# Daaohame/RAHT-3DGS-codec

Hardware: AMD Instinct MI355X
Metric: M-Gaussians/s fwd+inv RAHT, 59-ch SH3 3DGS (higher is better)
Workload: dtype f32 (xyz columns: f64); 1 GPU; cfg3: 2999072 Gaussians (3000000 draws/GPU, J=12, 59 channels), fwd RAHT + quantize/reorder + dequantize/un-reorder + inv RAHT (quantization fused into the transform kernels); the 3 xyz columns carried in float64 inside the same launches (raht_fwd_quant_mixed / raht_dequant_inv_mixed): the reference's integers on every column; rows_per_gpu=2999072, channels=59, depth_J=12, engine=tile, quantize=True, parallelism=1 GPU, world=1

## Files before the change

### include/raht.h

```cpp
#ifndef RAHT_H
#define RAHT_H

#include <stdint.h>

#ifdef __cplusplus
extern "C" {
#endif

#define RAHT_VERSION 300

enum raht_status {
    RAHT_OK = 0,
    RAHT_ERR_INVALID = -1,
    RAHT_ERR_UNSORTED = -2,
    RAHT_ERR_BOUNDS = -3,
    RAHT_ERR_HIP = -4,
    RAHT_ERR_NOMEM = -5,
    RAHT_ERR_UNSUPPORTED = -6
};

enum raht_dtype { RAHT_F32 = 0, RAHT_F64 = 1, RAHT_I32 = 2, RAHT_I64 = 3 };

enum raht_engine { RAHT_ENGINE_TILE = 0, RAHT_ENGINE_LEVEL = 1 };

typedef struct raht_plan raht_plan;
typedef void *raht_stream_t;

const char *raht_last_error(void);
int raht_version(void);

int raht_plan_create(const void *V, int v_dtype, int64_t N, const double minV[3], double width,
                     int depth, raht_stream_t stream, raht_plan **out);

int raht_plan_create_from_keys(const uint64_t *keys_sorted, int64_t N, int nbits,
                               const int64_t *leaf_weights, raht_stream_t stream, raht_plan **out);
int raht_plan_create_from_keys_borrowed(const uint64_t *keys_sorted, int64_t N, int nbits,
                                        const int64_t *leaf_weights, raht_stream_t stream, raht_plan **out);

int raht_plan_set_top_level(raht_plan *plan, int top_level, raht_stream_t stream);
int raht_plan_roots(const raht_plan *plan, int64_t *n_roots, int64_t *rows_dev, raht_stream_t stream);
int raht_plan_set_root_buffer(raht_plan *plan, void *buf_dev);
int raht_plan_set_root_buffer_wide(raht_plan *plan, double *buf_dev);

int raht_plan_set_row_map(raht_plan *plan, const int64_t *map_dev, int64_t n_matrix_rows, raht_stream_t stream);

int raht_plan_destroy(raht_plan *plan);
int64_t raht_plan_size(const raht_plan *plan);
int raht_plan_nbits(const raht_plan *plan);

int raht_plan_set_engine(raht_plan *plan, int engine, int tile_rows);
int raht_plan_set_tail_tile(raht_plan *plan, int tail_rows, int tail_channels, int final_rows);
int raht_plan_set_max_stages(raht_plan *plan, int max_stages);

int raht_release_cached_memory(void);
int raht_set_cached_memory_limit(int64_t bytes);

int raht_plan_levels(const raht_plan *plan);
int raht_plan_export_level(const raht_plan *plan, int level, int64_t *list, uint8_t *flags,
                           int64_t *weights, int64_t *n);
int raht_plan_order(const raht_plan *plan, int64_t *order_dev, raht_stream_t stream);
int raht_plan_arrays(const raht_plan *plan, const uint64_t **keys, const uint8_t **lvl,
                     const int32_t **wl, const int32_t **wr);
int raht_plan_copy_array(const raht_plan *plan, int which, void *dst_dev, raht_stream_t stream);
int raht_plan_stage_stats(raht_plan *plan, int elem_size, int D, int *n_stages, int64_t *rows_per_stage,
                          int max_stages, int *tile_rows);

int raht_fwd(const raht_plan *plan, const float *C, int64_t ldc, int D, float *T, int64_t ldt,
             float *w, raht_stream_t stream);
int raht_fwd_f64(const raht_plan *plan, const double *C, int64_t ldc, int D, double *T, int64_t ldt,
                 double *w, raht_stream_t stream);

int raht_inv(const raht_plan *plan, const float *T, int64_t ldt, int D, float *C, int64_t ldc,
             raht_stream_t stream);
int raht_inv_f64(const raht_plan *plan, const double *T, int64_t ldt, int D, double *C, int64_t ldc,
                 raht_stream_t stream);

int raht_fwd_quant(const raht_plan *plan, const float *C, int64_t ldc, int D, const float *steps,
                   int n_steps, int32_t *Q, int64_t ldq, raht_stream_t stream);
int raht_dequant_inv(const raht_plan *plan, const int32_t *Q, int64_t ldq, int D, const float *steps,
                     int n_steps, float *C, int64_t ldc, raht_stream_t stream);

int raht_fwd_quant_multi(const raht_plan *plan, const float *C, int64_t ldc, int D, const float *steps, int k,
                         int32_t *const *Q, int64_t ldq, raht_stream_t stream);

int raht_dequant_inv_sqdiff(const raht_plan *plan, const int32_t *Q, int64_t ldq, int D, const float *steps, int n_steps,
                            const float *C_ref, int64_t ld_ref, float *C_rec, int64_t ldc, double *sqdiff, raht_stream_t stream);

int raht_fwd_quant_f64(const raht_plan *plan, const double *C, int64_t ldc, int D, const double *steps,
                       int n_steps, int32_t *Q, int64_t ldq, raht_stream_t stream);
int raht_dequant_inv_f64(const raht_plan *plan, const int32_t *Q, int64_t ldq, int D, const double *steps,
                         int n_steps, double *C, int64_t ldc, raht_stream_t stream);

int raht_fwd_quant_mixed(const raht_plan *plan, const float *C, int64_t ldc, int D, const double *steps, int n_steps,
                         int n_wide, int32_t *Q, int64_t ldq, raht_stream_t stream);
int raht_dequant_inv_mixed(const raht_plan *plan, const int32_t *Q, int64_t ldq, int D, const double *steps, int n_steps,
                           int n_wide, float *C, int64_t ldc, raht_stream_t stream);
int raht_fwd_quant_mixed_multi(const raht_plan *plan, const float *C, int64_t ldc, int D, const double *steps, int k,
                               int n_wide, int32_t *const *Q, int64_t ldq, raht_stream_t stream);
int raht_dequant_inv_mixed_sqdiff(const raht_plan *plan, const int32_t *Q, int64_t ldq, int D, const double *steps, int n_steps,
                                  int n_wide, const float *C_ref, int64_t ld_ref, float *C_rec, int64_t ldc, double *sqdiff,
                                  raht_stream_t stream);
int raht_plan_mixed_stats(raht_plan *plan, int D, int n_wide, int *tile_rows, int *n_stages, int64_t *rows_per_stage,
                          int max_stages);

int raht_fwd_batch(int n, raht_plan *const *plans, const float *const *C, const int64_t *ldc, int D,
                   float *const *T, const int64_t *ldt, raht_stream_t stream);
int raht_inv_batch(int n, raht_plan *const *plans, const float *const *T, const int64_t *ldt, int D,
                   float *const *C, const int64_t *ldc, raht_stream_t stream);
int raht_fwd_quant_batch(int n, raht_plan *const *plans, const float *const *C, const int64_t *ldc, int D,
                         const float *steps, int n_steps, int32_t *const *Q, const int64_t *ldq, raht_stream_t stream);
int raht_dequant_inv_batch(int n, raht_plan *const *plans, const int32_t *const *Q, const int64_t *ldq, int D,
                           const float *steps, int n_steps, float *const *C, const int64_t *ldc, raht_stream_t stream);

int raht_fwd_quant_mixed_batch(int n, raht_plan *const *plans, const float *const *C, const int64_t *ldc, int D,
                               const double *steps, int n_steps, int n_wide,
                               int32_t *const *Q, const int64_t *ldq, raht_stream_t stream);
int raht_dequant_inv_mixed_batch(int n, raht_plan *const *plans, const int32_t *const *Q, const int64_t *ldq, int D,
                                 const double *steps, int n_steps, int n_wide,
                                 float *const *C, const int64_t *ldc, raht_stream_t stream);
int raht_mixed_batch_stats(int n, raht_plan *const *plans, int D, int n_wide, int inverse,
                           int *tile_launches, int *top_launches, int *single_scene_calls);

int raht_plan_prepare(raht_plan *plan, int elem_size, int D, raht_stream_t stream);

int raht_plan_set_concurrent_directions(raht_plan *plan, int on);

int raht_plan_set_stage0_events(raht_plan *plan, void *ev_before, void *ev_after);

int raht_debug_run_stage(const raht_plan *plan, int inverse, int stage, const float *mat, int64_t ld_mat,
                         int D, float *mat2, int64_t ld_mat2, int32_t *Q, int64_t ldq, float step,
                         int ablate, raht_stream_t stream);

int raht_quant_reorder(const raht_plan *plan, const float *T, int64_t ldt, int D, const float *steps,
                       int n_steps, int32_t *Q, int64_t ldq, raht_stream_t stream);
int raht_dequant_unreorder(const raht_plan *plan, const int32_t *Q, int64_t ldq, int D,
                           const float *steps, int n_steps, float *T, int64_t ldt,
                           raht_stream_t stream);
int raht_quant_reorder_f64(const raht_plan *plan, const double *T, int64_t ldt, int D, const double *steps,
                           int n_steps, int32_t *Q, int64_t ldq, raht_stream_t stream);
int raht_dequant_unreorder_f64(const raht_plan *plan, const int32_t *Q, int64_t ldq, int D,
                               const double *steps, int n_steps, double *T, int64_t ldt,
                               raht_stream_t stream);

int raht_voxelize(const float *PC, int64_t ldpc, int64_t N, int d, const float *vmin_in,
                  double width_in, int J, uint64_t *keys_sorted, int64_t *sort_idx,
                  int64_t *voxel_indices, float *PCvox, int64_t *Vvox, int64_t *n_vox,
                  float vmin_out[3], double *width_out, double *voxel_size_out,
                  raht_stream_t stream);

int raht_voxelize_all(const float *PC, int64_t ldpc, int64_t N, int d, const float *vmin_in, double width_in,
                      int J, uint64_t *keys_sorted, int64_t *sort_idx, int64_t *voxel_indices, float *PCvox,
                      int64_t *Vvox, float *PCsorted, float *DeltaPC, int64_t *n_vox, float vmin_out[3],
                      double *width_out, double *voxel_size_out, raht_stream_t stream);

int raht_voxelize_plan(const float *PC, int64_t ldpc, int64_t N, int d, const float *vmin_in, double width_in,
                       int J, uint64_t *voxel_keys, int64_t *voxel_indices, float *PCvox, int64_t *n_vox,
                       float vmin_out[3], double *width_out, double *voxel_size_out, raht_stream_t stream,
                       raht_plan **plan);

int raht_voxelize_residuals(const float *PC, int64_t ldpc, int64_t N, int d, const uint64_t *keys_sorted,
                            const int64_t *sort_idx, const float *PCvox, const float vmin[3], double voxel_size,
                            float *PCsorted, float *DeltaPC, raht_stream_t stream);

int raht_voxel_keys(const float *PC, int64_t ldpc, int64_t N, const float vmin[3], double width, int J,
                    uint64_t *keys, raht_stream_t stream);

int raht_morton(const int64_t *V, int64_t N, int J, uint64_t *keys, raht_stream_t stream);

int raht_sort_keys(const uint64_t *keys_in, int64_t N, int nbits, uint64_t *keys_out,
                   int64_t *idx_out, raht_stream_t stream);
int64_t raht_sort_fallbacks(void);

int raht_merge_clusters(const int32_t *cluster_indices, const int32_t *cluster_offsets, int64_t num_clusters,
                        const float *means, const float *quats, const float *scales, const float *opacities,
                        const float *colors, int color_dim, int weight_by_opacity, float *merged_means,
                        float *merged_quats, float *merged_scales, float *merged_opacities,
                        float *merged_colors, raht_stream_t stream);

int raht_voxelize_merge(const float *G, int64_t ldg, int64_t N, int color_dim, int weight_by_opacity, const float *vmin_in,
                        double width_in, int J, uint64_t *keys_sorted, int64_t *sort_idx, int64_t *voxel_indices, float *Gvox,
                        float *merged_means, int64_t *n_vox, float vmin_out[3], double *width_out, double *voxel_size_out,
                        raht_stream_t stream);

int raht_quant_rows(const float *X, int64_t ldx, int64_t n, int D, const float *steps, int n_steps,
                    const int64_t *pos, int32_t *Q, int64_t ldq, raht_stream_t stream);
int raht_dequant_rows(const int32_t *Q, int64_t ldq, const int64_t *pos, int64_t n, int D, const float *steps,
                      int n_steps, float *X, int64_t ldx, raht_stream_t stream);
int raht_quant_rows_f64(const double *X, int64_t ldx, int64_t n, int D, const double *steps, int n_steps,
                        const int64_t *pos, int32_t *Q, int64_t ldq, raht_stream_t stream);
int raht_dequant_rows_f64(const int32_t *Q, int64_t ldq, const int64_t *pos, int64_t n, int D, const double *steps,
                          int n_steps, double *X, int64_t ldx, raht_stream_t stream);

int raht_rows_gather(const void *src, int64_t ld_src, const int64_t *pos, int64_t n, int D, int elem_size, void *dst,
                     int64_t ld_dst, raht_stream_t stream);
int raht_rows_scatter(const void *src, int64_t ld_src, const int64_t *pos, int64_t n, int D, int elem_size, void *dst,
                      int64_t ld_dst, raht_stream_t stream);

int64_t raht_rlgr_bound(int64_t n);
int raht_rlgr_encode(const int32_t *seq, int64_t n, int64_t stride, int flag_signed, uint8_t *out,
                     int64_t cap, int64_t *nbytes);
int raht_rlgr_decode(const uint8_t *buf, int64_t nbytes, int64_t n, int flag_signed, int32_t *seq,
                     int64_t stride);
int raht_rlgr_encode_channels(const int32_t *Q, int64_t N, int D, int64_t sym_stride, int64_t chan_stride,
                              int flag_signed, uint8_t *out, int64_t cap_per_channel, int64_t *nbytes,
                              int nthreads);
int raht_rlgr_decode_channels(const uint8_t *bufs, int64_t cap_per_channel, const int64_t *nbytes,
                              int64_t N, int D, int flag_signed, int32_t *Q, int64_t sym_stride,
                              int64_t chan_stride, int nthreads);
int raht_transpose_i32(const int32_t *in, int64_t ld_in, int64_t rows, int64_t cols, int32_t *out,
                       int64_t ld_out, raht_stream_t stream);
int raht_xchg_bytes(int world, int64_t slot_bytes, int64_t *total);
int raht_xchg_alloc(int world, int64_t slot_bytes, void **base, void *handle64);
int raht_xchg_open(const void *handle64, void **base);
int raht_xchg_close(void *base);
int raht_xchg_free(void *base);
int raht_xchg_gather(const void *send, int64_t slot_bytes, void *const *peers, int rank, int world, uint32_t seq,
                     raht_stream_t stream);
int raht_xchg_buffer(void *base, int world, int64_t slot_bytes, uint32_t seq, void **buf);
int raht_xchg_status(void *base, int world, int64_t slot_bytes, raht_stream_t stream, int *status);

int raht_rlgr_seg_encode(const int32_t *Q, int64_t N, int D, int64_t chan_stride, int seg_len, int flag_signed,
                         uint32_t *seg_bytes, uint32_t *seg_off, uint8_t *out, int64_t cap, int64_t *total_bytes,
                         raht_stream_t stream);
int raht_rlgr_seg_decode(const uint8_t *in, int64_t in_bytes, const uint32_t *seg_off, const uint32_t *seg_bytes, int64_t N,
                         int D, int seg_len, int flag_signed, int32_t *Q, int64_t chan_stride, uint32_t *bad_dev,
                         raht_stream_t stream);

int raht_rlgr_seg_encode_strided(const int32_t *Q, int64_t N, int D, int64_t sym_stride, int64_t chan_stride, int seg_len,
                                 int flag_signed, uint32_t *seg_bytes, uint32_t *seg_off, uint8_t *out, int64_t cap,
                                 int64_t *total_bytes, raht_stream_t stream);
int raht_rlgr_seg_decode_strided(const uint8_t *in, int64_t in_bytes, const uint32_t *seg_off, const uint32_t *seg_bytes, int64_t N,
                                 int D, int seg_len, int flag_signed, int32_t *Q, int64_t sym_stride, int64_t chan_stride,
                                 uint32_t *bad_dev, raht_stream_t stream);

int raht_rlgr_seg_offsets_width(int64_t N, int D, int seg_len);
int raht_rlgr_seg_encode64(const int32_t *Q, int64_t N, int D, int64_t sym_stride, int64_t chan_stride, int seg_len,
                           int flag_signed, uint32_t *seg_bytes, uint64_t *seg_off, uint8_t *out, int64_t cap,
                           int64_t *total_bytes, raht_stream_t stream);
int raht_rlgr_seg_decode64(const uint8_t *in, int64_t in_bytes, const uint64_t *seg_off, const uint32_t *seg_bytes, int64_t N,
                           int D, int seg_len, int flag_signed, int32_t *Q, int64_t sym_stride, int64_t chan_stride,
                           uint32_t *bad_dev, raht_stream_t stream);

#define RAHT_RLGR_BATCH_MAX 12
int raht_rlgr_seg_encode_batch(int k, const int32_t *const *Q, int64_t N, int D, int64_t sym_stride, int64_t chan_stride, int seg_len,
                               int flag_signed, uint32_t *const *seg_bytes, uint32_t *const *seg_off, uint8_t *const *out,
                               const int64_t *cap, int64_t *total_bytes, raht_stream_t stream);
int raht_rlgr_seg_decode_batch(int k, const uint8_t *const *in, const int64_t *in_bytes, const uint32_t *const *seg_off,
                               const uint32_t *const *seg_bytes, int64_t N, int D, int seg_len, int flag_signed, int32_t *const *Q,
                               int64_t sym_stride, int64_t chan_stride, uint32_t *bad_dev, raht_stream_t stream);
int raht_rlgr_seg_decode_batch_check(int k, const uint8_t *const *in, const int64_t *in_bytes, const uint32_t *const *seg_off,
                                     const uint32_t *const *seg_bytes, int64_t N, int D, int seg_len, int flag_signed,
                                     int32_t *const *Q, const int32_t *const *expect, int64_t sym_stride, int64_t chan_stride,
                                     uint32_t *bad_dev, raht_stream_t stream);

int raht_rlgr_seg_encode_batch64(int k, const int32_t *const *Q, int64_t N, int D, int64_t sym_stride, int64_t chan_stride,
                                 int seg_len, int flag_signed, uint32_t *const *seg_bytes, uint64_t *const *seg_off,
// ... 80 lines not shown
```

### raht-3dgs-codec_amd/_lib.py

```python
import contextlib
import ctypes as C
import os
import subprocess

_PKG = os.path.dirname(os.path.abspath(__file__))
_CSRC = os.path.join(_PKG, "csrc")
SO_PATH = os.path.join(_PKG, "libraht_hip.so")

RAHT_OK = 0
ERRORS = {-1: "RAHT_ERR_INVALID", -2: "RAHT_ERR_UNSORTED", -3: "RAHT_ERR_BOUNDS", -4: "RAHT_ERR_HIP",
          -5: "RAHT_ERR_NOMEM", -6: "RAHT_ERR_UNSUPPORTED"}
RAHT_F32, RAHT_F64, RAHT_I32, RAHT_I64 = 0, 1, 2, 3
ENGINE_TILE, ENGINE_LEVEL = 0, 1

EXPORTS = [
    "raht_last_error", "raht_version", "raht_plan_create", "raht_plan_create_from_keys", "raht_plan_create_from_keys_borrowed",
    "raht_plan_destroy", "raht_plan_set_top_level", "raht_plan_roots", "raht_plan_set_root_buffer", "raht_plan_set_root_buffer_wide", "raht_plan_size", "raht_plan_nbits", "raht_plan_set_engine", "raht_plan_set_tail_tile", "raht_release_cached_memory", "raht_set_cached_memory_limit", "raht_quant_rows", "raht_dequant_rows", "raht_quant_rows_f64", "raht_dequant_rows_f64",
    "raht_plan_levels", "raht_plan_export_level", "raht_plan_order", "raht_plan_arrays",
    "raht_plan_copy_array", "raht_plan_stage_stats", "raht_fwd", "raht_fwd_f64", "raht_inv", "raht_inv_f64", "raht_debug_run_stage", "raht_plan_set_stage0_events", "raht_fwd_quant", "raht_dequant_inv", "raht_plan_prepare",
    "raht_quant_reorder", "raht_dequant_unreorder", "raht_voxelize", "raht_voxelize_all", "raht_voxelize_plan", "raht_morton", "raht_sort_keys",
    "raht_voxel_keys", "raht_sort_fallbacks", "raht_voxelize_residuals", "raht_plan_set_row_map", "raht_rows_gather", "raht_rows_scatter",
    "raht_plan_set_max_stages", "raht_plan_set_concurrent_directions", "raht_quant_reorder_f64", "raht_dequant_unreorder_f64", "raht_fwd_quant_f64", "raht_dequant_inv_f64",
    "raht_fwd_quant_mixed", "raht_dequant_inv_mixed", "raht_dequant_inv_sqdiff", "raht_fwd_quant_multi", "raht_plan_mixed_stats",
    "raht_fwd_quant_mixed_multi", "raht_dequant_inv_mixed_sqdiff",
    "raht_fwd_batch", "raht_inv_batch", "raht_fwd_quant_batch", "raht_dequant_inv_batch",
    "raht_fwd_quant_mixed_batch", "raht_dequant_inv_mixed_batch", "raht_mixed_batch_stats",
    "raht_rlgr_bound", "raht_rlgr_encode", "raht_rlgr_decode", "raht_rlgr_encode_channels", "raht_rlgr_decode_channels", "raht_transpose_i32", "raht_i32_equal", "raht_sqdiff_columns", "raht_merge_clusters", "raht_voxelize_merge", "raht_rlgr_seg_encode", "raht_rlgr_seg_decode", "raht_rlgr_seg_encode_strided", "raht_rlgr_seg_decode_strided", "raht_rlgr_seg_encode_batch", "raht_rlgr_seg_decode_batch", "raht_rlgr_seg_decode_batch_check", "raht_rlgr_seg_offsets_width", "raht_rlgr_seg_encode64", "raht_rlgr_seg_decode64", "raht_rlgr_seg_encode_batch64", "raht_rlgr_seg_decode_batch64", "raht_rlgr_seg_encode_ragged", "raht_rlgr_seg_decode_ragged", "raht_debug_rlgr_decode_out", "raht_debug_rlgr_encode_out", "raht_rlgr_seg_rate", "raht_debug_height_stages_per_launch", "raht_debug_live_blocks", "raht_debug_cached_blocks", "raht_debug_sort_form", "raht_debug_motion_tile",
    "raht_xchg_bytes", "raht_xchg_alloc", "raht_xchg_open", "raht_xchg_close", "raht_xchg_free", "raht_xchg_gather", "raht_xchg_buffer", "raht_xchg_status",
    "raht_octree_counts", "raht_octree_encode", "raht_octree_decode", "raht_octree_symbols", "raht_octree_bytes", "raht_demorton",
    "raht_octree_encode_inter", "raht_octree_decode_inter", "raht_octree_bytes_used",
    "raht_region_layout", "raht_region_cells", "raht_region_assemble",
    "raht_region_layout_set", "raht_region_assemble_set", "raht_region_needs",
    "raht_predict", "raht_motion_search", "raht_predict_mc",
]


class RahtError(RuntimeError):
    def __init__(self, code, msg):
        super().__init__(f"{ERRORS.get(code, code)}: {msg}")
        self.code = code


def build(verbose=False):
    r = subprocess.run(["make", "-C", _CSRC, "-j4"], capture_output=True, text=True)
    if verbose or r.returncode != 0:
        print(r.stdout)
        print(r.stderr)
    if r.returncode != 0:
        raise RuntimeError("building libraht_hip.so failed")
    return SO_PATH


_lib = None


def lib():
    global _lib
    if _lib is not None:
        return _lib
    if not os.path.exists(SO_PATH):
        raise RuntimeError(
            f"raht-3dgs-codec_amd: HIP library {SO_PATH} is missing. Build it with "
            f"`python -c 'import __graft_entry__ as g; g.build()'` (or `make -C {_CSRC}`). "
            "There is no CPU fallback for the RAHT hot path.")
    try:
        import torch
    except Exception:
        pass
    L = C.CDLL(SO_PATH)
    vp, i64, i32, dbl = C.c_void_p, C.c_int64, C.c_int, C.c_double
    L.raht_last_error.restype = C.c_char_p
    L.raht_plan_create.argtypes = [vp, i32, i64, C.POINTER(dbl), dbl, i32, vp, C.POINTER(vp)]
    L.raht_plan_create_from_keys.argtypes = [vp, i64, i32, vp, vp, C.POINTER(vp)]
    L.raht_plan_create_from_keys_borrowed.argtypes = [vp, i64, i32, vp, vp, C.POINTER(vp)]
    L.raht_plan_destroy.argtypes = [vp]
    L.raht_plan_set_top_level.argtypes = [vp, i32, vp]
    L.raht_plan_roots.argtypes = [vp, C.POINTER(i64), vp, vp]
    L.raht_plan_set_root_buffer.argtypes = [vp, vp]
    L.raht_plan_set_root_buffer_wide.argtypes = [vp, vp]
    L.raht_plan_size.argtypes = [vp]
    L.raht_plan_size.restype = i64
    L.raht_plan_nbits.argtypes = [vp]
    L.raht_plan_set_engine.argtypes = [vp, i32, i32]
    L.raht_plan_set_tail_tile.argtypes = [vp, i32, i32, i32]
    L.raht_plan_levels.argtypes = [vp]
    L.raht_plan_export_level.argtypes = [vp, i32, vp, vp, vp, C.POINTER(i64)]
    L.raht_plan_order.argtypes = [vp, vp, vp]
    L.raht_plan_arrays.argtypes = [vp, C.POINTER(vp), C.POINTER(vp), C.POINTER(vp), C.POINTER(vp)]
    L.raht_plan_copy_array.argtypes = [vp, i32, vp, vp]
    L.raht_plan_stage_stats.argtypes = [vp, i32, i32, C.POINTER(i32), C.POINTER(i64), i32, C.POINTER(i32)]
    for f in (L.raht_fwd, L.raht_fwd_f64):
        f.argtypes = [vp, vp, i64, i32, vp, i64, vp, vp]
    for f in (L.raht_inv, L.raht_inv_f64):
        f.argtypes = [vp, vp, i64, i32, vp, i64, vp]
    L.raht_plan_set_stage0_events.argtypes = [vp, vp, vp]
    L.raht_debug_run_stage.argtypes = [vp, i32, i32, vp, i64, i32, vp, i64, vp, i64, C.c_float, i32, vp]
    L.raht_fwd_quant.argtypes = [vp, vp, i64, i32, C.POINTER(C.c_float), i32, vp, i64, vp]
    L.raht_dequant_inv.argtypes = [vp, vp, i64, i32, C.POINTER(C.c_float), i32, vp, i64, vp]
    L.raht_plan_prepare.argtypes = [vp, i32, i32, vp]
    L.raht_fwd_quant_mixed.argtypes = [vp, vp, i64, i32, C.POINTER(dbl), i32, i32, vp, i64, vp]
    L.raht_dequant_inv_mixed.argtypes = [vp, vp, i64, i32, C.POINTER(dbl), i32, i32, vp, i64, vp]
    L.raht_dequant_inv_sqdiff.argtypes = [vp, vp, i64, i32, C.POINTER(C.c_float), i32, vp, i64, vp, i64, vp, vp]
    L.raht_fwd_quant_multi.argtypes = [vp, vp, i64, i32, C.POINTER(C.c_float), i32, C.POINTER(vp), i64, vp]
    L.raht_fwd_quant_mixed_multi.argtypes = [vp, vp, i64, i32, C.POINTER(dbl), i32, i32, C.POINTER(vp), i64, vp]
    L.raht_dequant_inv_mixed_sqdiff.argtypes = [vp, vp, i64, i32, C.POINTER(dbl), i32, i32, vp, i64, vp, i64, vp, vp]
    L.raht_plan_mixed_stats.argtypes = [vp, i32, i32, C.POINTER(i32), C.POINTER(i32), C.POINTER(i64), i32]
    pp, pi64 = C.POINTER(vp), C.POINTER(i64)
    L.raht_fwd_batch.argtypes = [i32, pp, pp, pi64, i32, pp, pi64, vp]
    L.raht_inv_batch.argtypes = [i32, pp, pp, pi64, i32, pp, pi64, vp]
    L.raht_fwd_quant_batch.argtypes = [i32, pp, pp, pi64, i32, C.POINTER(C.c_float), i32, pp, pi64, vp]
    L.raht_dequant_inv_batch.argtypes = [i32, pp, pp, pi64, i32, C.POINTER(C.c_float), i32, pp, pi64, vp]
    L.raht_fwd_quant_mixed_batch.argtypes = [i32, pp, pp, pi64, i32, C.POINTER(dbl), i32, i32, pp, pi64, vp]
    L.raht_dequant_inv_mixed_batch.argtypes = [i32, pp, pp, pi64, i32, C.POINTER(dbl), i32, i32, pp, pi64, vp]
    L.raht_mixed_batch_stats.argtypes = [i32, pp, i32, i32, i32, C.POINTER(i32), C.POINTER(i32), C.POINTER(i32)]
    L.raht_plan_set_max_stages.argtypes = [vp, i32]
    L.raht_plan_set_concurrent_directions.argtypes = [vp, i32]
    L.raht_plan_set_row_map.argtypes = [vp, vp, i64, vp]
    for f in (L.raht_rows_gather, L.raht_rows_scatter):
        f.argtypes = [vp, i64, vp, i64, i32, i32, vp, i64, vp]
    for f in (L.raht_quant_reorder_f64, L.raht_dequant_unreorder_f64, L.raht_fwd_quant_f64, L.raht_dequant_inv_f64):
        f.argtypes = [vp, vp, i64, i32, C.POINTER(dbl), i32, vp, i64, vp]
    L.raht_quant_reorder.argtypes = [vp, vp, i64, i32, C.POINTER(C.c_float), i32, vp, i64, vp]
    L.raht_dequant_unreorder.argtypes = [vp, vp, i64, i32, C.POINTER(C.c_float), i32, vp, i64, vp]
    L.raht_quant_rows.argtypes = [vp, i64, i64, i32, C.POINTER(C.c_float), i32, vp, vp, i64, vp]
    L.raht_dequant_rows.argtypes = [vp, i64, vp, i64, i32, C.POINTER(C.c_float), i32, vp, i64, vp]
    L.raht_quant_rows_f64.argtypes = [vp, i64, i64, i32, C.POINTER(dbl), i32, vp, vp, i64, vp]
    L.raht_dequant_rows_f64.argtypes = [vp, i64, vp, i64, i32, C.POINTER(dbl), i32, vp, i64, vp]
    L.raht_voxelize.argtypes = [vp, i64, i64, i32, C.POINTER(C.c_float), dbl, i32, vp, vp, vp, vp, vp,
                                C.POINTER(i64), C.POINTER(C.c_float), C.POINTER(dbl), C.POINTER(dbl), vp]
    L.raht_sqdiff_columns.argtypes = [vp, i64, vp, i64, i64, i32, i32, vp, vp]
    L.raht_voxelize_all.argtypes = [vp, i64, i64, i32, C.POINTER(C.c_float), dbl, i32, vp, vp, vp, vp, vp, vp, vp,
                                    C.POINTER(i64), C.POINTER(C.c_float), C.POINTER(dbl), C.POINTER(dbl), vp]
    L.raht_voxelize_plan.argtypes = [vp, i64, i64, i32, C.POINTER(C.c_float), dbl, i32, vp, vp, vp, C.POINTER(i64),
                                     C.POINTER(C.c_float), C.POINTER(dbl), C.POINTER(dbl), vp, C.POINTER(vp)]
    L.raht_voxelize_merge.argtypes = [vp, i64, i64, i32, i32, C.POINTER(C.c_float), dbl, i32, vp, vp, vp, vp, vp, C.POINTER(i64),
                                      C.POINTER(C.c_float), C.POINTER(dbl), C.POINTER(dbl), vp]
    L.raht_morton.argtypes = [vp, i64, i32, vp, vp]
    L.raht_voxel_keys.argtypes = [vp, i64, i64, C.POINTER(C.c_float), dbl, i32, vp, vp]
    L.raht_voxelize_residuals.argtypes = [vp, i64, i64, i32, vp, vp, vp, C.POINTER(C.c_float), dbl, vp, vp, vp]
    L.raht_sort_keys.argtypes = [vp, i64, i32, vp, vp, vp]
    L.raht_sort_fallbacks.argtypes = []
    L.raht_sort_fallbacks.restype = i64
    L.raht_rlgr_bound.argtypes = [i64]
    L.raht_rlgr_bound.restype = i64
    L.raht_rlgr_encode.argtypes = [vp, i64, i64, i32, vp, i64, C.POINTER(i64)]
    L.raht_rlgr_decode.argtypes = [vp, i64, i64, i32, vp, i64]
    L.raht_rlgr_encode_channels.argtypes = [vp, i64, i32, i64, i64, i32, vp, i64, vp, i32]
    L.raht_rlgr_decode_channels.argtypes = [vp, i64, vp, i64, i32, i32, vp, i64, i64, i32]
    L.raht_merge_clusters.argtypes = [vp, vp, i64, vp, vp, vp, vp, vp, i32, i32, vp, vp, vp, vp, vp, vp]
    L.raht_transpose_i32.argtypes = [vp, i64, i64, i64, vp, i64, vp]
    L.raht_i32_equal.argtypes = [vp, vp, i64, i32, C.POINTER(i64)]
    L.raht_rlgr_seg_encode.argtypes = [vp, i64, i32, i64, i32, i32, vp, vp, vp, i64, C.POINTER(i64), vp]
    L.raht_rlgr_seg_decode.argtypes = [vp, i64, vp, vp, i64, i32, i32, i32, vp, i64, vp, vp]
    L.raht_rlgr_seg_encode_strided.argtypes = [vp, i64, i32, i64, i64, i32, i32, vp, vp, vp, i64, C.POINTER(i64), vp]
    L.raht_rlgr_seg_decode_strided.argtypes = [vp, i64, vp, vp, i64, i32, i32, i32, vp, i64, i64, vp, vp]
    L.raht_debug_rlgr_decode_out.argtypes = [i32]
    L.raht_debug_rlgr_encode_out.argtypes = [i32]
    L.raht_debug_height_stages_per_launch.argtypes = [i32]
    L.raht_debug_live_blocks.argtypes = []
    L.raht_debug_live_blocks.restype = i64
    L.raht_debug_cached_blocks.argtypes = []
    L.raht_debug_cached_blocks.restype = i64
    L.raht_set_cached_memory_limit.argtypes = [i64]
    L.raht_debug_sort_form.argtypes = [i32, i32, i64]
    L.raht_debug_motion_tile.argtypes = [i32]
    L.raht_rlgr_seg_encode_batch.argtypes = [i32, C.POINTER(vp), i64, i32, i64, i64, i32, i32, C.POINTER(vp), C.POINTER(vp), C.POINTER(vp), C.POINTER(i64), C.POINTER(i64), vp]
    L.raht_rlgr_seg_decode_batch.argtypes = [i32, C.POINTER(vp), C.POINTER(i64), C.POINTER(vp), C.POINTER(vp), i64, i32, i32, i32, C.POINTER(vp), i64, i64, vp, vp]
    L.raht_rlgr_seg_decode_batch_check.argtypes = [i32, C.POINTER(vp), C.POINTER(i64), C.POINTER(vp), C.POINTER(vp), i64, i32, i32, i32, C.POINTER(vp), C.POINTER(vp), i64, i64, vp, vp]
    L.raht_rlgr_seg_offsets_width.argtypes = [i64, i32, i32]
    L.raht_rlgr_seg_encode64.argtypes = L.raht_rlgr_seg_encode_strided.argtypes
    L.raht_rlgr_seg_decode64.argtypes = L.raht_rlgr_seg_decode_strided.argtypes
    L.raht_rlgr_seg_encode_batch64.argtypes = L.raht_rlgr_seg_encode_batch.argtypes
    L.raht_rlgr_seg_decode_batch64.argtypes = L.raht_rlgr_seg_decode_batch_check.argtypes
    L.raht_rlgr_seg_encode_ragged.argtypes = [i32, C.POINTER(vp), C.POINTER(i64), i32, C.POINTER(i64), C.POINTER(i64), i32, i32, C.POINTER(vp), C.POINTER(vp), C.POINTER(vp), C.POINTER(i64), C.POINTER(i64), vp]
    L.raht_rlgr_seg_decode_ragged.argtypes = [i32, C.POINTER(vp), C.POINTER(i64), C.POINTER(vp), C.POINTER(vp), C.POINTER(i64), i32, i32, i32, C.POINTER(vp), C.POINTER(vp), C.POINTER(i64), C.POINTER(i64), vp, vp]
    L.raht_rlgr_seg_rate.argtypes = [vp, i32, i64, i64, i32, vp, i32, i32, i32, i32, vp, vp, vp]
    L.raht_xchg_bytes.argtypes = [i32, i64, C.POINTER(i64)]
    L.raht_xchg_alloc.argtypes = [i32, i64, C.POINTER(vp), vp]
    L.raht_xchg_open.argtypes = [vp, C.POINTER(vp)]
    L.raht_xchg_close.argtypes = [vp]
    L.raht_xchg_free.argtypes = [vp]
    L.raht_xchg_gather.argtypes = [vp, i64, C.POINTER(vp), i32, i32, C.c_uint32, vp]
    L.raht_xchg_buffer.argtypes = [vp, i32, i64, C.c_uint32, C.POINTER(vp)]
    L.raht_xchg_status.argtypes = [vp, i32, i64, vp, C.POINTER(i32)]
    L.raht_octree_counts.argtypes = [vp, i64, i32, C.POINTER(i64), vp]
    L.raht_octree_encode.argtypes = [vp, i64, i32, C.POINTER(i64), vp, vp]
    L.raht_octree_decode.argtypes = [vp, C.POINTER(i64), i32, vp, vp, vp]
    L.raht_octree_symbols.argtypes = [vp, i64, vp, vp, vp]
    L.raht_octree_bytes.argtypes = [vp, i64, vp, vp, vp, vp]
    L.raht_demorton.argtypes = [vp, i64, i32, vp, vp]
    L.raht_octree_encode_inter.argtypes = [vp, i64, i32, C.POINTER(i64), vp, i64, vp, vp]
    L.raht_octree_decode_inter.argtypes = [vp, C.POINTER(i64), i32, vp, i64, vp, vp, vp]
    L.raht_octree_bytes_used.argtypes = [vp, i64, vp, i32, vp, vp, vp]
    L.raht_region_layout.argtypes = [vp, i64, i32, i64, i64, vp, vp]
    L.raht_region_cells.argtypes = [vp, i64, i32, i32, i64, vp, vp, vp]
    L.raht_region_assemble.argtypes = [vp, i64, i64, vp, i64, i64, i32, C.POINTER(i64), i32, vp]
    L.raht_region_layout_set.argtypes = [vp, i64, i32, vp, i32, vp, vp]
    L.raht_region_assemble_set.argtypes = [vp, i64, i64, vp, i64, i64, i32, vp, C.POINTER(i64), i32, vp]
    L.raht_region_needs.argtypes = [vp, i64, i32, i32, i32, vp, i64, vp, i32, vp, i64, C.POINTER(i64), vp]
    L.raht_predict.argtypes = [vp, i64, vp, i64, i32, vp, i64, vp, i64, i32, i32, vp, i64, vp, vp]
    L.raht_motion_search.argtypes = [vp, i64, i32, i32, vp, i64, vp, i64, i32, vp, i64, vp, i64, i32, vp, vp, i32, vp, vp, vp, vp]
    L.raht_predict_mc.argtypes = [vp, i64, i32, i32, vp, i64, vp, vp, i64, i32, vp, i64, vp, i64, i32, i32, vp, i64, vp, vp]
    _lib = L
    return L


def check(rc):
    if rc != RAHT_OK:
        raise RahtError(rc, lib().raht_last_error().decode("utf-8", "replace"))


@contextlib.contextmanager
def sort_form(onesweep=1, rounds=0, fail_tile=-1):
    prev = lib().raht_debug_sort_form(onesweep, rounds, fail_tile)
    check(min(prev, 0))
    try:
        yield
    finally:
        lib().raht_debug_sort_form(prev & 1, (prev >> 1) & 31, (prev >> 6) - 1)
```

### raht-3dgs-codec_amd/csrc/raht_common.h

```cpp
#pragma once

#include <hip/hip_runtime.h>
#include <stdint.h>

#include <cstdarg>
#include <cstdio>
#include <deque>
#include <exception>
#include <functional>
#include <new>
#include <type_traits>
#include <utility>
#include <vector>

#include "raht.h"

#define RAHT_WAVE 64
#define RAHT_MAX_LEVELS 64

namespace raht {

void set_error(const char *fmt, ...);

#define RAHT_HIP_CHECK(expr)                                                              \
// ... 45 lines not shown
    return RAHT_OK;
}

constexpr int RAHT_MAX_DEVICES = 64;
static inline int current_device()
{
    int d = 0;
    if (hipGetDevice(&d) != hipSuccess || d < 0 || d >= RAHT_MAX_DEVICES) d = 0;
    return d;
}
class DeviceGuard {
public:
    explicit DeviceGuard(int device) : prev_(current_device()), dev_(device)
    {
        if (prev_ != dev_) (void)hipSetDevice(dev_);
    }
    ~DeviceGuard() { if (prev_ != dev_) (void)hipSetDevice(prev_); }
    DeviceGuard(const DeviceGuard &) = delete;
    DeviceGuard &operator=(const DeviceGuard &) = delete;
private:
    int prev_, dev_;
};
struct PerDeviceOnce {
    bool done[RAHT_MAX_DEVICES] = {};
    bool first(int device) { if (done[device]) return false; done[device] = true; return true; }
};

class Scratch {
public:
    Scratch(size_t bytes, hipStream_t stream);
    ~Scratch();
    Scratch(const Scratch &) = delete;
    Scratch &operator=(const Scratch &) = delete;
    void *ptr() const { return p_; }
    template <typename T> T *as() const { return (T *)p_; }
    bool ok() const { return p_ != nullptr; }
private:
    void *p_ = nullptr;
    int slot_ = -1;
};

hipError_t dev_malloc(void **p, size_t bytes);
template <typename T> inline hipError_t dev_malloc(T **p, size_t bytes) { return dev_malloc((void **)p, bytes); }
void dev_free(void *p);

template <typename T>
class DevBuf {
public:
    DevBuf() = default;
    DevBuf(DevBuf &&o) noexcept : p_(o.p_), owned_(o.owned_) { o.p_ = nullptr; }
    DevBuf &operator=(DevBuf &&o) noexcept { if (this != &o) { reset(); p_ = o.p_; owned_ = o.owned_; o.p_ = nullptr; } return *this; }
    ~DevBuf() { reset(); }
    hipError_t alloc(size_t count)
    {
        reset();
        owned_ = true;
        return dev_malloc((void **)&p_, count * sizeof(typename std::conditional<std::is_void<T>::value, char, T>::type));
    }
    void borrow(T *p) { reset(); p_ = p; owned_ = false; }
    T *get() const { return p_; }
    operator T *() const { return p_; }
    void reset() { if (p_ && owned_) dev_free(p_); p_ = nullptr; }
    T *release() { T *q = p_; p_ = nullptr; return q; }
private:
    T *p_ = nullptr;
    bool owned_ = true;
};
struct OwnedEvent {
    hipEvent_t ev = nullptr;
    OwnedEvent() = default;
    OwnedEvent(OwnedEvent &&o) noexcept : ev(o.ev) { o.ev = nullptr; }
    OwnedEvent &operator=(OwnedEvent &&o) noexcept { std::swap(ev, o.ev); return *this; }
    ~OwnedEvent() { if (ev) (void)hipEventDestroy(ev); }
    operator hipEvent_t() const { return ev; }
};

int read_back_u32(uint32_t *dst_a, const uint32_t *dev_a, int na, uint32_t *dst_b, const uint32_t *dev_b, int nb,
                  hipStream_t s, const std::function<void()> &behind = std::function<void()>());

int exclusive_scan_u32(const uint32_t *in, uint32_t *out, int64_t n, uint32_t *total, hipStream_t s);
int exclusive_scan_u32_u64(const uint32_t *in, uint64_t *out, int64_t n, uint64_t *total, hipStream_t s);

struct VoxGrid;
int sort_keys_u32idx(const uint64_t *keys_in, int64_t N, int nbits, uint64_t *keys_out, uint32_t *idx_out, hipStream_t s,
                     uint32_t *sort_err = nullptr, int64_t *idx64_out = nullptr, const VoxGrid *grid = nullptr, bool onesweep = true);
void note_sort_fallback();
int vox_keys(const VoxGrid &grid, int64_t N, uint64_t *keys, hipStream_t s);
int bucket_sort_u8(const uint8_t *bucket, uint32_t *perm_out, int64_t n, int bits,
                   uint32_t *bucket_off, hipStream_t s);

int compact_u32(const uint32_t *in, const uint32_t *flag, uint32_t *out, int64_t n,
                int64_t *count_host, hipStream_t s, const uint32_t *extra_dev = nullptr, uint32_t *extra_host = nullptr);

int run_starts_u64(const uint64_t *keys_sorted, int64_t n, uint32_t *starts, int64_t *starts64, uint64_t *run_keys,
                   uint32_t *count_dev, hipStream_t s);

#ifdef RAHT_PHASE_CLOCKS
constexpr int PL_CLK_BLOCKS = 4096, PL_CLK_SLOTS = 12;
static __device__ unsigned long long g_phase_clk_plan[3][PL_CLK_BLOCKS][PL_CLK_SLOTS];
#define PL_STAMP(which, blk, k) do { if (threadIdx.x == 0 && (blk) < PL_CLK_BLOCKS) g_phase_clk_plan[which][blk][k] = __builtin_readcyclecounter(); } while (0)
#define PL_NOTE_LEVELS(blk, n) do { if (threadIdx.x == 0 && (blk) < PL_CLK_BLOCKS) g_phase_clk_plan[1][blk][PL_CLK_SLOTS - 1] = (unsigned long long)(n); } while (0)
#define PL_SLOT_DECL int pl_slot = 0
#define PL_STAMP_NEXT() do { if (pl_slot < 8) { PL_STAMP(2, 0, pl_slot); ++pl_slot; } } while (0)
int read_phase_clocks_sched(unsigned long long *dst, int which, int n_blocks);
#else
#define PL_STAMP(which, blk, k) do { } while (0)
#define PL_NOTE_LEVELS(blk, n) do { } while (0)
#define PL_SLOT_DECL do { } while (0)
#define PL_STAMP_NEXT() do { } while (0)
#endif

constexpr int RAHT_TOP_MAX_ROWS = 8192;

struct Stage {
    int64_t n_entries = 0;
    int64_t n_tiles = 0;
    DevBuf<uint32_t> rows;
    DevBuf<uint32_t> surv_off;
    DevBuf<void> ws;
    size_t ws_inv_off = 0;
    int tile_rows = 0;
    DevBuf<int32_t> e_wl, e_wr;
    DevBuf<uint8_t> e_lvl;
    DevBuf<uint32_t> e_pos;
    DevBuf<uint8_t> e_ht;
    bool is_top = false;
    uint32_t n_merges = 0;
    DevBuf<uint32_t> t_pj;
    DevBuf<float> t_ab32;
    DevBuf<double> t_ab64;
    DevBuf<uint32_t> t_root;
    uint32_t t_loff[65] = {0};
    uint32_t t_lev_host[2 * 64] = {0};
    DevBuf<uint32_t> t_lev;
    int t_nlev = 0;
    int t_nbig = 0;
    uint32_t t_small_start = 0;
    DevBuf<uint32_t> prog;
    uint32_t prog_stride = 0;
    uint32_t prog_ab = 0;
    bool prog_compact = false;
};

struct Schedule {
    int tile_rows = 0;
    int tail_rows = 0;
    int final_rows = 0;
    bool valid = false;
    std::vector<Stage> stages;
    size_t ws_row_bytes = 0;
    bool ws_split = false;
    OwnedEvent ready;
    hipStream_t ready_on = nullptr;
};
static_assert(!std::is_copy_constructible<Stage>::value && !std::is_copy_constructible<Schedule>::value, "stages and schedules own device memory: moved, never copied");

}

struct raht_plan {
    int device = 0;
    int64_t N = 0;
    int nbits = 0;
    int max_level = -1;
    raht::DevBuf<uint64_t> keys;
    raht::DevBuf<uint8_t> lvl;
    raht::DevBuf<int32_t> wl, wr;
    raht::DevBuf<int64_t> wsum;
    raht::DevBuf<uint32_t> order;
    raht::DevBuf<uint32_t> inv_order;
    raht::DevBuf<uint32_t> level_rows;
    uint32_t level_off[RAHT_MAX_LEVELS + 1];
    int top_level = 64;
    int64_t n_roots = 1;
    raht::DevBuf<uint32_t> root_rows;
    void *root_buf = nullptr;
    double *root_buf_w = nullptr;
    raht::DevBuf<uint32_t> row_map;
    int64_t map_rows = 0;
    int engine = RAHT_ENGINE_TILE;
    int tile_rows_override = 0;
    int tail_rows_override = 0;
    int tail_chunk_override = 0;
    int final_rows_override = 0;
    const uint32_t *pend_dev = nullptr; uint32_t *pend_host = nullptr; int pend_n = 0;
    hipEvent_t ev_before = nullptr, ev_after = nullptr;
    int max_stages = 24;
    bool split_ws = false;
    std::deque<raht::Schedule> schedules;
    std::vector<uint8_t> lvl_host;
};

namespace raht {
int check_plan_device(const raht_plan *plan, const char *what);
__device__ __forceinline__ void pair_weights(int64_t i, int l, int r, const int64_t *wsum, double &w0, double &w1)
{
    if (wsum) {
        w0 = (double)(wsum[i] - wsum[i - l]);
        w1 = (double)(wsum[i + r] - wsum[i]);
    } else {
        w0 = (double)l;
        w1 = (double)r;
    }
}

int ensure_level_rows(raht_plan *plan, hipStream_t s);
int get_schedule(raht_plan *plan, int tile_rows, int tail_rows, int final_rows, hipStream_t s, Schedule **out);
void pick_tail_geometry(const raht_plan *plan, int elem_size, int D, int stage0_rows, int *tail_rows, int *tail_chunk,
                        int *final_rows);
int build_tile_programs(raht_plan *plan, Schedule *sc, hipStream_t s);
int ensure_workspace(Schedule *sc, size_t row_bytes, bool split = false);
static inline void *stage_ws(const Stage &st, bool inverse) { return st.ws ? (void *)((char *)st.ws.get() + (inverse ? st.ws_inv_off : 0)) : nullptr; }
void free_schedule(Schedule &sc);
struct StageArrays { const uint32_t *rows; const int32_t *wl, *wr; const uint8_t *lvl; const uint32_t *pos; uint8_t *ht; };
static inline StageArrays stage_arrays(const raht_plan *p, const Stage &st)
{
    if (st.rows) return {st.rows, st.e_wl, st.e_wr, st.e_lvl, st.e_pos, st.e_ht};
    return {nullptr, p->wl, p->wr, p->lvl, p->inv_order, st.e_ht};
}
int pick_tile_rows(const raht_plan *plan, int elem_size, int chunk_channels);
int pick_chunk_channels(int elem_size, int D);

size_t tile_lds_bytes(int R, int elem_size, int Dc, bool ident, bool qm);
int launch_sq_final(const double *part, int64_t n_tiles, int D, int ncv, double *out, hipStream_t s);
}
```

### raht-3dgs-codec_amd/csrc/schedule.hip

```cpp
#include "raht_common.h"

#include <algorithm>
#include <atomic>

namespace raht {

__global__ void compact_scatter_kernel(const uint32_t *in, const uint32_t *flag, const uint32_t *pos, uint32_t *out, int64_t n);

__global__ void stage_survivor_kernel(const uint32_t *__restrict__ rows, int64_t n, int R, int64_t N,
                                      const int32_t *__restrict__ wl, const int32_t *__restrict__ wr,
                                      const uint8_t *__restrict__ lvl, int top_level,
                                      uint32_t *__restrict__ survivor)
{
    const int64_t j = (int64_t)blockIdx.x * blockDim.x + threadIdx.x;
    if (j >= n) return;
    const int64_t r = rows ? rows[j] : j;
    const int64_t t = j / R;
    const int64_t j0 = t * R, j1 = j0 + R;
    const int64_t start = rows ? rows[j0] : j0;
    const int64_t end = (j1 < n) ? (rows ? (int64_t)rows[j1] : j1) : N;
    const bool merged = (r > 0) && ((int)lvl[r] < top_level) && (r - wl[r] >= start) && (r + wr[r] <= end);
    survivor[j] = merged ? 0u : 1u;
}

static int fit_chunk_channels(int elem_size, int D, int max_dc)
{
    const int vn = 16 / elem_size;
    const int hi = std::max(std::min(max_dc, 64), vn);
    if (D <= hi) return D;
    for (int Dc = hi; Dc >= vn; --Dc) {
        const int r = D % Dc;
        if (r == 0 || r >= vn) return Dc;
    }
    for (int Dc = hi + 1; Dc <= 64; ++Dc) {
        const int r = D % Dc;
        if (r == 0 || r >= vn) return Dc;
    }
    return std::min(D, 64);
}

int pick_chunk_channels(int elem_size, int D)
{
    return fit_chunk_channels(elem_size, D, 64);
}

size_t tile_lds_bytes(int R, int elem_size, int Dc, bool ident, bool qm)
{
    const int vn = 16 / elem_size;
    const size_t Dp = (size_t)((Dc + vn - 1) / vn) * vn;
    size_t data = (size_t)R * Dp * elem_size;
    size_t meta = (size_t)R * ((elem_size == 4 ? 16 : 24) + (ident ? 0 : 4) + (qm ? 4 : 0) + 1);
    size_t surv = ((size_t)R * 2 + 15) & ~(size_t)15;
    return data + ((meta + 15) & ~(size_t)15) + 1024 + surv + (size_t)12 * Dp * elem_size;
}

int pick_tile_rows(const raht_plan *plan, int elem_size, int Dc)
{
    if (plan->tile_rows_override > 0) return plan->tile_rows_override;
    const size_t budget = (size_t)42 * 1280;
    for (int R = 512; R >= 64; R -= 8)
        if (tile_lds_bytes(R, elem_size, Dc, true, true) <= budget) return R;
    return 0;
}

void pick_tail_geometry(const raht_plan *plan, int elem_size, int D, int stage0_rows, int *tail_rows, int *tail_chunk,
                        int *final_rows)
{
    int Dc = std::min(D, 64), R = stage0_rows;
    if (D > 64) Dc = pick_chunk_channels(elem_size, D);
    if (plan->tail_chunk_override > 0) Dc = fit_chunk_channels(elem_size, D, std::min(plan->tail_chunk_override, std::min(D, 64)));
    if (plan->tail_rows_override > 0) {
        R = plan->tail_rows_override;
        while (R > 64 && tile_lds_bytes(R, elem_size, Dc, false, true) > (size_t)128 * 1280) R -= 64;
    } else {
        while (R > 64 && tile_lds_bytes(R, elem_size, Dc, false, true) > (size_t)42 * 1280) R -= 8;
    }
    *tail_rows = R;
    *tail_chunk = Dc;
    int Rf = 1536;
    if (plan->final_rows_override > 0) Rf = std::min(plan->final_rows_override, RAHT_TOP_MAX_ROWS);
    *final_rows = Rf;
}

void free_schedule(Schedule &sc)
{
    if (!sc.stages.empty()) (void)hipDeviceSynchronize();
    sc.stages.clear();
    sc.ready = OwnedEvent();
}

int ensure_workspace(Schedule *sc, size_t row_bytes, bool split)
{
    if (row_bytes <= sc->ws_row_bytes && split == sc->ws_split) return RAHT_OK;
    row_bytes = std::max(row_bytes, sc->ws_row_bytes);
    for (size_t k = 1; k < sc->stages.size(); ++k) {
        Stage &st = sc->stages[k];
        if (st.ws) { (void)hipDeviceSynchronize(); st.ws.reset(); }
        const size_t one = (row_bytes * (size_t)st.n_entries + 255) & ~(size_t)255;
        if (st.ws.alloc(split ? 2 * one : one) != hipSuccess) {
            set_error("workspace allocation failed (%zu bytes)", split ? 2 * one : one);
            sc->ws_row_bytes = 0;
            return RAHT_ERR_NOMEM;
        }
        st.ws_inv_off = split ? one : 0;
    }
    sc->ws_row_bytes = row_bytes;
    sc->ws_split = split;
    return RAHT_OK;
}

__global__ void tile_start_kernel(const uint32_t *__restrict__ pos, int64_t n, int R, int64_t n_tiles,
                                  uint32_t total, uint32_t *__restrict__ surv_off)
{
    const int64_t t = (int64_t)blockIdx.x * blockDim.x + threadIdx.x;
    if (t > n_tiles) return;
    surv_off[t] = (t < n_tiles) ? pos[t * R] : total;
    (void)n;
}

__global__ void gather_meta_kernel(const uint32_t *__restrict__ rows, int64_t n, const int32_t *__restrict__ wl,
                                   const int32_t *__restrict__ wr, const uint8_t *__restrict__ lvl,
                                   const uint32_t *__restrict__ inv_order, int32_t *__restrict__ e_wl,
                                   int32_t *__restrict__ e_wr, uint8_t *__restrict__ e_lvl, uint32_t *__restrict__ e_pos)
{
    const int64_t j = (int64_t)blockIdx.x * blockDim.x + threadIdx.x;
    if (j >= n) return;
    const uint32_t r = rows[j];
    e_wl[j] = wl[r]; e_wr[j] = wr[r]; e_lvl[j] = lvl[r]; e_pos[j] = inv_order[r];
}

constexpr int HT_MAX_ROWS = 1024, HT_MAX_STAGES = 8;
struct HeightStage {
    const uint32_t *rows; const int32_t *wl, *wr; const uint8_t *lvl; uint8_t *ht;
    int64_t n; int R; uint32_t first_tile;
    const uint32_t *n_dev, *kind_dev; uint32_t kind_tile;
};
struct HeightArgs { HeightStage st[HT_MAX_STAGES]; int n_stages; uint32_t n_tiles; int64_t N; int top_level; };

template <int SPL>
__global__ __launch_bounds__(64) void tile_heights_kernel(const HeightArgs H)
{
    extern __shared__ __align__(16) unsigned char ht_smem[];
    int k = 0;
#pragma unroll
    for (int q = 1; q < HT_MAX_STAGES; ++q) k += (q < H.n_stages && blockIdx.x >= H.st[q].first_tile) ? 1 : 0;
    PL_STAMP(1, blockIdx.x, 0);
    const HeightStage &S = H.st[k];
    const int R = S.R;
    const int lane = threadIdx.x;
    const int64_t e0 = (int64_t)(blockIdx.x - S.first_tile) * R;
    if (S.kind_dev && *S.kind_dev != S.kind_tile) return;
    const int64_t Sn = S.n_dev ? (int64_t)*S.n_dev : S.n;
    if (e0 >= Sn) return;
    const uint32_t *__restrict__ rows = S.rows;
    const int nt = (int)min((int64_t)R, Sn - e0);
    uint8_t *s_cur = ht_smem;
    uint32_t *s_row = (uint32_t *)(ht_smem + ((R + 15) & ~15));
    const int64_t start_row = rows ? (int64_t)rows[e0] : e0;
    const int64_t end_row = (e0 + R < Sn) ? (rows ? (int64_t)rows[e0 + R] : e0 + R) : H.N;
    int lv[SPL], part[SPL];
    int32_t wlv[SPL], wrv[SPL];
    int64_t r[SPL];
#pragma unroll
    for (int s = 0; s < SPL; ++s) {
        const int j = lane + s * 64;
        lv[s] = 255; wlv[s] = 0; wrv[s] = 0; r[s] = 0;
        if (j < nt) {
            r[s] = rows ? (int64_t)rows[e0 + j] : e0 + j;
            lv[s] = (int)S.lvl[e0 + j]; wlv[s] = S.wl[e0 + j]; wrv[s] = S.wr[e0 + j];
        }
    }
    if (rows) {
#pragma unroll
        for (int s = 0; s < SPL; ++s) { const int j = lane + s * 64; if (j < nt) s_row[j] = (uint32_t)r[s]; }
    }
#pragma unroll
    for (int s = 0; s < SPL; ++s) { const int j = lane + s * 64; if (j < nt) s_cur[j] = 0; }
    __syncthreads();
    PL_STAMP(1, blockIdx.x, 1);
    uint64_t mask = 0;
#pragma unroll
    for (int s = 0; s < SPL; ++s) {
        const int j = lane + s * 64;
        const bool merged = (j < nt) && (r[s] > 0) && (lv[s] < H.top_level) && (r[s] - wlv[s] >= start_row) && (r[s] + wrv[s] <= end_row);
        part[s] = 0;
        if (merged) {
            if (!rows) part[s] = j - wlv[s];
            else {
                const uint32_t want = (uint32_t)(r[s] - wlv[s]);
                int lo = 0, hi = j - 1;
                while (lo < hi) { const int mid = (lo + hi) >> 1; if (s_row[mid] < want) lo = mid + 1; else hi = mid; }
                part[s] = lo;
            }
            mask |= (uint64_t)1 << lv[s];
        } else {
            lv[s] = 255;
        }
    }
#pragma unroll
    for (int d = 32; d >= 1; d >>= 1) {
        const uint32_t lo = (uint32_t)__shfl_xor((int)(uint32_t)mask, d, 64), hi = (uint32_t)__shfl_xor((int)(uint32_t)(mask >> 32), d, 64);
        mask |= (uint64_t)lo | ((uint64_t)hi << 32);
    }
    int ht[SPL];
#pragma unroll
    for (int s = 0; s < SPL; ++s) ht[s] = 0;
    PL_STAMP(1, blockIdx.x, 2);
    PL_NOTE_LEVELS(blockIdx.x, __popcll(mask));
    mask = (uint64_t)(uint32_t)__builtin_amdgcn_readfirstlane((int)(uint32_t)mask) |
           ((uint64_t)(uint32_t)__builtin_amdgcn_readfirstlane((int)(uint32_t)(mask >> 32)) << 32);
    while (mask) {
        const int l = __ffsll((unsigned long long)mask) - 1;
        mask &= mask - 1;
        int h[SPL];
#pragma unroll
        for (int s = 0; s < SPL; ++s) {
            h[s] = 0;
            if (lv[s] == l) h[s] = 1 + max((int)s_cur[part[s]], (int)s_cur[lane + s * 64]);
        }
#pragma unroll
        for (int s = 0; s < SPL; ++s)
            if (lv[s] == l) { ht[s] = h[s]; s_cur[part[s]] = (uint8_t)h[s]; }
        __syncthreads();
    }
    PL_STAMP(1, blockIdx.x, 3);
#pragma unroll
    for (int s = 0; s < SPL; ++s) { const int j = lane + s * 64; if (j < nt) S.ht[e0 + j] = (uint8_t)ht[s]; }
    PL_STAMP(1, blockIdx.x, 4);
}

template <typename F>
static void by_lane_slots(int R, F &&f)
{
    const int spl = (R + 63) / 64;
    if (spl <= 3) f(std::integral_constant<int, 3>{});
    else if (spl <= 4) f(std::integral_constant<int, 4>{});
    else if (spl <= 8) f(std::integral_constant<int, 8>{});
    else f(std::integral_constant<int, 16>{});
}

// ... 24 lines not shown
        for (int q = H.n_stages; q < HT_MAX_STAGES; ++q) H.st[q] = H.st[0];
        launch_heights_kernel(H, maxR, any_rows, s);
        RAHT_HIP_CHECK(hipGetLastError());
        reset();
        return RAHT_OK;
    };
    reset();
    const int group = g_height_group.load();
    for (size_t k = 0; k < sc.stages.size(); ++k) {
        Stage &st = sc.stages[k];
        if (st.is_top || st.n_entries < 1) continue;
        if (st.tile_rows > HT_MAX_ROWS) { set_error("tile heights: %d rows per tile not supported", st.tile_rows); return RAHT_ERR_UNSUPPORTED; }
        if (!st.e_ht) RAHT_HIP_CHECK(st.e_ht.alloc((size_t)st.n_entries));
        HeightStage &h = H.st[H.n_stages++];
        h = height_stage(stage_arrays(plan, st), st.tile_rows, H.n_tiles);
        h.n = st.n_entries;
        H.n_tiles += (uint32_t)st.n_tiles;
        maxR = std::max(maxR, st.tile_rows);
        any_rows = any_rows || st.rows != nullptr;
        if (H.n_stages == group) RAHT_RET(flush());
    }
    return flush();
}

struct ProgStage {
    const uint32_t *rows; const int32_t *wl, *wr; const uint8_t *lvl, *ht; const uint32_t *pos;
    uint32_t *prog; int64_t n; int R; uint32_t stride, ab; int compact;
};

template <int SPL>
__global__ __launch_bounds__(64) void tile_program_kernel(const ProgStage S, int64_t N, int top_level, const int64_t *__restrict__ wsum)
{
    extern __shared__ __align__(16) unsigned char pg_smem[];
    __shared__ uint32_t s_hist[64], s_cur[64];
    uint32_t *s_row = (uint32_t *)pg_smem;
    const int R = S.R;
    const int lane = threadIdx.x;
    const int64_t e0 = (int64_t)blockIdx.x * R;
    if (e0 >= S.n) return;
    const uint32_t *__restrict__ rows = S.rows;
    const int nt = (int)min((int64_t)R, S.n - e0);
    const int64_t start_row = rows ? (int64_t)rows[e0] : e0;
    const int64_t end_row = (e0 + R < S.n) ? (rows ? (int64_t)rows[e0 + R] : e0 + R) : N;
    uint32_t *pg = S.prog + (size_t)blockIdx.x * S.stride;
    uint32_t *rw = pg + 32, *rec = pg + 32 + R;
    double *ab = (double *)(pg + S.ab);
    int lv[SPL], ht[SPL];
    int32_t wlv[SPL], wrv[SPL];
    uint32_t pos[SPL];
    int64_t r[SPL];
#pragma unroll
    for (int s = 0; s < SPL; ++s) {
        const int j = lane + s * 64;
        lv[s] = 255; wlv[s] = 0; wrv[s] = 0; r[s] = 0; ht[s] = 0; pos[s] = 0;
        if (j < nt) {
            r[s] = rows ? (int64_t)rows[e0 + j] : e0 + j;
            lv[s] = (int)S.lvl[e0 + j]; wlv[s] = S.wl[e0 + j]; wrv[s] = S.wr[e0 + j];
            ht[s] = S.ht[e0 + j] & 63; pos[s] = S.pos[e0 + j];
        }
    }
    s_hist[lane] = 0;
    if (rows) {
#pragma unroll
        for (int s = 0; s < SPL; ++s) { const int j = lane + s * 64; if (j < nt) s_row[j] = (uint32_t)r[s]; }
    }
    __syncthreads();
    bool merged[SPL];
    int part[SPL];
#pragma unroll
    for (int s = 0; s < SPL; ++s) {
        const int j = lane + s * 64;
        merged[s] = (j < nt) && (r[s] > 0) && (lv[s] < top_level) && (r[s] - wlv[s] >= start_row) && (r[s] + wrv[s] <= end_row);
        part[s] = 0;
        if (merged[s]) {
            if (!rows) part[s] = j - wlv[s];
            else {
                const uint32_t want = (uint32_t)(r[s] - wlv[s]);
                int lo = 0, hi = j - 1;
                while (lo < hi) { const int mid = (lo + hi) >> 1; if (s_row[mid] < want) lo = mid + 1; else hi = mid; }
                part[s] = lo;
            }
            atomicAdd(&s_hist[ht[s]], 1u);
        }
        if (j < nt) rw[j] = pos[s] | (merged[s] ? 0x80000000u : 0u);
    }
    __syncthreads();
    const uint32_t c = s_hist[lane];
    uint32_t inc = c;
#pragma unroll
    for (int d = 1; d < 64; d <<= 1) {
        const uint32_t t = __shfl_up(inc, d, 64);
        if (lane >= d) inc += t;
    }
    ((uint16_t *)pg)[lane] = (uint16_t)inc;
    s_cur[lane] = inc - c;
    const uint32_t n_merged = (uint32_t)__shfl((int)inc, 63, 64);
    __syncthreads();
    const uint64_t lt = (lane == 0) ? 0ull : (~0ull >> (64 - lane));
    uint32_t n_surv = 0;
#pragma unroll
    for (int s = 0; s < SPL; ++s) {
        const int j = lane + s * 64;
        const bool surv = j < nt && !merged[s];
        const uint64_t bal = __ballot(surv);
        if (surv) rec[n_merged + n_surv + (uint32_t)__popcll(bal & lt)] = (uint32_t)j;
        n_surv += (uint32_t)__popcll(bal);
        if (merged[s]) {
            const uint32_t k = atomicAdd(&s_cur[ht[s]], 1u);
            if (S.compact) {
                rec[k] = (uint32_t)j | ((uint32_t)wlv[s] << 10) | ((uint32_t)wrv[s] << 20);
            } else {
                double w0, w1;
                pair_weights(r[s], wlv[s], wrv[s], wsum, w0, w1);
                const double den = w0 + w1;
                rec[k] = (uint32_t)part[s] | ((uint32_t)j << 16);
                ab[2 * k] = sqrt(w0 / den);
                ab[2 * k + 1] = sqrt(w1 / den);
            }
        }
    }
}

int build_tile_programs(raht_plan *plan, Schedule *sc, hipStream_t s)
{
    bool built = false;
    for (auto &st : sc->stages) {
        if (st.is_top || st.n_entries < 1 || st.prog) continue;
        const int R = st.tile_rows;
        if (R > HT_MAX_ROWS || !st.e_ht) { set_error("tile programs: %d rows per tile not supported", R); return RAHT_ERR_UNSUPPORTED; }
        ProgStage P;
        const StageArrays a = stage_arrays(plan, st);
        P.rows = a.rows; P.wl = a.wl; P.wr = a.wr; P.lvl = a.lvl; P.pos = a.pos; P.ht = a.ht;
        P.n = st.n_entries; P.R = R;
        P.compact = (st.rows == nullptr && plan->wsum == nullptr) ? 1 : 0;
        P.ab = (uint32_t)(32 + 2 * R + 3) & ~3u;
        P.stride = P.compact ? P.ab : P.ab + 4 * (uint32_t)R;
        if (!P.wl || !P.wr || !P.lvl || !P.pos) { set_error("tile programs: missing plan arrays"); return RAHT_ERR_INVALID; }
        RAHT_HIP_CHECK(st.prog.alloc((size_t)P.stride * (size_t)st.n_tiles));
        P.prog = st.prog;
        const size_t lds = st.rows ? (size_t)R * 4 : 0;
        const unsigned grid = (unsigned)st.n_tiles;
        by_lane_slots(R, [&](auto spl) {
            hipLaunchKernelGGL(tile_program_kernel<decltype(spl)::value>, dim3(grid), dim3(64), lds, s, P, plan->N, plan->top_level, plan->wsum);
        });
        RAHT_HIP_CHECK(hipGetLastError());
        st.prog_stride = P.stride; st.prog_ab = P.ab; st.prog_compact = P.compact != 0;
        built = true;
    }
    if (built) {
        if (!sc->ready) RAHT_HIP_CHECK(hipEventCreateWithFlags(&sc->ready.ev, hipEventDisableTiming));
        RAHT_HIP_CHECK(hipEventRecord(sc->ready, s));
        sc->ready_on = s;
    }
    return RAHT_OK;
}

__global__ void top_resolve_kernel(const uint32_t *__restrict__ rows, int64_t n, const int32_t *__restrict__ wl,
                                   const int32_t *__restrict__ wr, const uint8_t *__restrict__ lvl,
                                   const int64_t *__restrict__ wsum, int top_level, uint32_t *__restrict__ pj,
                                   double *__restrict__ ab, uint8_t *__restrict__ bucket, uint32_t *__restrict__ is_root)
{
    const int64_t e = (int64_t)blockIdx.x * blockDim.x + threadIdx.x;
    if (e >= n) return;
    const int64_t r = rows ? (int64_t)rows[e] : e;
    const int l = (int)lvl[r];
    const bool merged = (r > 0) && (l < top_level);
    is_root[e] = merged ? 0u : 1u;
    bucket[e] = merged ? (uint8_t)l : (uint8_t)63;
    uint32_t rec = 0;
    double a = 0.0, b = 0.0;
    if (merged) {
        const int64_t want = r - wl[r];
        int64_t p = want;
        if (rows) {
            int64_t lo = 0, hi = e - 1;
            while (lo < hi) {
                const int64_t mid = (lo + hi) >> 1;
                if ((int64_t)rows[mid] < want) lo = mid + 1; else hi = mid;
            }
            p = lo;
        }
        double w0, w1;
        pair_weights(r, wl[r], wr[r], wsum, w0, w1);
        const double den = w0 + w1;
        a = sqrt(w0 / den);
        b = sqrt(w1 / den);
        rec = (uint32_t)p | ((uint32_t)e << 16);
    }
    pj[e] = rec; ab[2 * e] = a; ab[2 * e + 1] = b;
}

__global__ void top_gather_kernel(const uint32_t *__restrict__ perm, uint32_t n_merges, const uint32_t *__restrict__ pj,
                                  const double *__restrict__ ab, uint32_t *__restrict__ t_pj,
                                  float *__restrict__ t_ab32, double *__restrict__ t_ab64)
{
    const uint32_t k = blockIdx.x * blockDim.x + threadIdx.x;
    if (k >= n_merges) return;
    const uint32_t e = perm[k];
    t_pj[k] = pj[e];
    const double a = ab[2 * e], b = ab[2 * e + 1];
    t_ab64[2 * k] = a; t_ab64[2 * k + 1] = b;
    t_ab32[2 * k] = (float)a; t_ab32[2 * k + 1] = (float)b;
}

__global__ void top_root_rank_kernel(const uint32_t *__restrict__ is_root, const uint32_t *__restrict__ pos, int64_t n,
                                     uint32_t *__restrict__ t_root)
{
    const int64_t e = (int64_t)blockIdx.x * blockDim.x + threadIdx.x;
    if (e < n) t_root[e] = is_root[e] ? pos[e] : 0xffffffffu;
}

static hipError_t gather_stage_meta(const raht_plan *plan, Stage &st, hipStream_t s)
{
    const size_t n = (size_t)st.n_entries;
    hipError_t e = hipSuccess;
    if ((e = st.e_wl.alloc(n)) != hipSuccess || (e = st.e_wr.alloc(n)) != hipSuccess || (e = st.e_lvl.alloc(n)) != hipSuccess ||
        (e = st.e_pos.alloc(n)) != hipSuccess) return e;
    hipLaunchKernelGGL(gather_meta_kernel, dim3((unsigned)ceil_div((int64_t)n, 256)), dim3(256), 0, s, st.rows, (int64_t)n, plan->wl,
                       plan->wr, plan->lvl, plan->inv_order, st.e_wl, st.e_wr, st.e_lvl, st.e_pos);
    return hipSuccess;
}

static int build_top_stage(raht_plan *plan, int64_t n, hipStream_t s, Stage &st)
{
    st.is_top = true;
    st.n_entries = n;
    st.n_tiles = 1;
    st.tile_rows = (int)n;
    const uint32_t *rows = st.rows;
    const unsigned gb = (unsigned)ceil_div(n, 256);
    if (rows) RAHT_HIP_CHECK(gather_stage_meta(plan, st, s));
    Scratch buf(sizeof(double) * 2 * (size_t)n + sizeof(uint32_t) * (4 * (size_t)n + 66) + (size_t)n, s);
    if (!buf.ok()) return RAHT_ERR_NOMEM;
    double *ab = buf.as<double>();
    uint32_t *pj = (uint32_t *)(ab + 2 * n), *is_root = pj + n, *pos = is_root + n, *perm = pos + n, *boff = perm + n,
             *total = boff + 65;
    uint8_t *bucket = (uint8_t *)(total + 1);
    hipLaunchKernelGGL(top_resolve_kernel, dim3(gb), dim3(256), 0, s, rows, n, plan->wl, plan->wr, plan->lvl, plan->wsum,
                       plan->top_level, pj, ab, bucket, is_root);
    RAHT_RET(exclusive_scan_u32(is_root, pos, n, total, s));
    RAHT_HIP_CHECK(st.t_root.alloc((size_t)n));
    hipLaunchKernelGGL(top_root_rank_kernel, dim3(gb), dim3(256), 0, s, is_root, pos, n, st.t_root);
    RAHT_RET(bucket_sort_u8(bucket, perm, n, 6, boff, s));
    RAHT_RET(read_back_u32(st.t_loff, boff, 65, nullptr, nullptr, 0, s));
    st.n_merges = st.t_loff[63];
    {
        uint32_t *lev = st.t_lev_host;
        int nlev = 0;
        for (int l = 0; l < 63; ++l)
            if (st.t_loff[l + 1] > st.t_loff[l]) { lev[2 * nlev] = st.t_loff[l]; lev[2 * nlev + 1] = st.t_loff[l + 1]; ++nlev; }
        int nbig = nlev;
        while (nbig > 0 && lev[2 * (nbig - 1) + 1] - lev[2 * (nbig - 1)] <= 64) --nbig;
        const size_t lds_budget = 160 * 1024 - 1024;
        while (nbig < nlev && (size_t)n * 16 + (size_t)(st.n_merges - lev[2 * nbig]) * 20 > lds_budget) ++nbig;
        st.t_nlev = nlev; st.t_nbig = nbig;
        st.t_small_start = (nbig < nlev) ? lev[2 * nbig] : st.n_merges;
        RAHT_HIP_CHECK(st.t_lev.alloc(2 * 64));
        RAHT_HIP_CHECK(hipMemcpyAsync(st.t_lev, lev, sizeof(uint32_t) * 2 * (size_t)std::max(nlev, 1), hipMemcpyHostToDevice, s));
    }
    const size_t nm = std::max<size_t>(st.n_merges, 1);
    RAHT_HIP_CHECK(st.t_pj.alloc(nm));
    RAHT_HIP_CHECK(st.t_ab32.alloc(2 * nm));
    RAHT_HIP_CHECK(st.t_ab64.alloc(2 * nm));
    if (st.n_merges)
        hipLaunchKernelGGL(top_gather_kernel, dim3((unsigned)ceil_div(st.n_merges, 256)), dim3(256), 0, s, perm, st.n_merges,
                           pj, ab, st.t_pj, st.t_ab32, st.t_ab64);
    return RAHT_OK;
}

constexpr int SB_THREADS = 256, SB_ITEMS = 8, SB_BLOCK = SB_THREADS * SB_ITEMS;
constexpr int SCHED_SPEC_MAX = 8;
enum { SK_NONE = 0, SK_TILE = 1, SK_TOP = 2 };

struct SchedState {
    uint32_t n[SCHED_SPEC_MAX + 2];
    uint32_t kind[SCHED_SPEC_MAX + 2];
    uint32_t finished;
    uint32_t last_stage, last_is_top;
    uint32_t trouble;
    uint32_t top[4];
};
constexpr int SCHED_STATE_WORDS = sizeof(SchedState) / 4;

__device__ __forceinline__ uint32_t block_sum_256(uint32_t v, uint32_t *red )
{
#pragma unroll
    for (int d = 32; d >= 1; d >>= 1) v += __shfl_xor(v, d, 64);
    if ((threadIdx.x & 63) == 0) red[threadIdx.x >> 6] = v;
    __syncthreads();
    const uint32_t t = red[0] + red[1] + red[2] + red[3];
    __syncthreads();
    return t;
}

__device__ __forceinline__ void sched_state_init(SchedState *S, uint32_t n0, uint32_t kind0)
{
    uint32_t *w = (uint32_t *)S;
    for (int i = threadIdx.x; i < SCHED_STATE_WORDS; i += blockDim.x) w[i] = 0;
    __syncthreads();
    if (threadIdx.x == 0) { S->n[0] = n0; S->kind[0] = kind0; }
}

__global__ __launch_bounds__(SB_THREADS) void sched_count_kernel(SchedState *__restrict__ S, int k, const uint32_t *__restrict__ rows,
                                                                 const int32_t *__restrict__ wl, const int32_t *__restrict__ wr,
                                                                 const uint8_t *__restrict__ lvl, int R, int64_t N, int top_level,
                                                                 uint8_t *__restrict__ flags, uint32_t *__restrict__ blk_cnt, int64_t n_first)
// ... 583 lines not shown
```

### raht-3dgs-codec_amd/csrc/transform_mx.hip

```cpp
#include "raht_common.h"
#include "raht_device.h"
#include "tile_engine.h"
#include "tile_host.h"

#include <algorithm>
#include <cstdlib>
#include <string>
#include <type_traits>
#include <vector>

namespace raht {

#ifdef RAHT_PHASE_CLOCKS
constexpr int MX_CLK_TILES = 4096, MX_CLK_SLOTS = 12;
__device__ unsigned long long g_phase_clk_mx[MX_CLK_TILES][MX_CLK_SLOTS];
#define MX_STAMP(k) do { if (IDENT && threadIdx.x == 0 && tile_id < MX_CLK_TILES) g_phase_clk_mx[tile_id][k] = __builtin_readcyclecounter(); } while (0)
#else
#define MX_STAMP(k) do { } while (0)
#endif

constexpr int MX_MAX_WIDE = 4;
constexpr int MX_THREADS = 512;
constexpr int MX_TOP_THREADS = 1024;
constexpr int MX_TOP_SLOTS = RAHT_TOP_MAX_ROWS / MX_TOP_THREADS;

struct StepTableMX {
    StepTable f;
    double w[MX_MAX_WIDE];
};

static size_t tile_lds_bytes_mx(int R, int NF, int nwide)
{
    const size_t data = (size_t)R * NF * 16 + (((size_t)R * nwide * 8 + 15) & ~(size_t)15);
    const size_t meta = (size_t)R * (16 + 4 + 4);
    const size_t surv = ((size_t)R * 2 + 15) & ~(size_t)15;
    return data + meta + surv;
}

struct MxPtrs {
    const double *in_w;
    double *out_w;
    double *wsn_w;
    double *root_w;
    const uint32_t *prog;
    uint32_t prog_stride, prog_ab;
    int prog_compact;
};

struct MxMultiQ {
    int k;
    uint32_t fast_div;
    double step[MULTI_Q_MAX];
    int32_t *Q[MULTI_Q_MAX];
};

template <bool INV, bool IDENT, int SLOTS, bool ROOTS, bool MULTI = false, bool SQ = false>
__device__ __forceinline__ void tile_body_mx(const TileArgs<float> &A, const MxPtrs &P, const StepTableMX &ST, const int64_t tile_id,
                                             const MxMultiQ *MQ = nullptr)
{
    extern __shared__ __align__(16) unsigned char smem[];
    typedef RegChunk<float> V16;
    typedef RegChunk<double> W16;
    typedef RegChunk<int32_t> I16;
    const int R = A.R;
    const int tid0 = threadIdx.x;
    const int nthreads = blockDim.x, nwv = nthreads >> 6;
    const int nwide = A.nwide;
    const int lgw = nwide > 2 ? 2 : nwide - 1;
    const int Df = A.D;
    const int Fp = A.Dp, NF = Fp >> 2;
    const int lg = A.lg, lr = 6 - A.lg;
    const uint32_t NFm = ((1u << 20) + (uint32_t)NF - 1) / (uint32_t)NF;
    auto sync_lds = [&]() { asm volatile("s_waitcnt lgkmcnt(0)\n\ts_barrier" ::: "memory"); };
    auto wait_landed = [&]() { asm volatile("s_waitcnt vmcnt(0)" ::: "memory"); };

    size_t off = 0;
    float *ftile = (float *)smem; off += (size_t)R * Fp * 4;
    double *wd = (double *)(smem + off); off += ((size_t)R * nwide * 8 + 15) & ~(size_t)15;
    W16 *rec_ab = (W16 *)(smem + off); off += (size_t)R * 16;
    uint32_t *rec_pj = (uint32_t *)(smem + off); off += (size_t)R * 4;
    int32_t *sdst = (int32_t *)(smem + off); off += (size_t)R * 4;
    uint16_t *ssurv = (uint16_t *)(smem + off);

    auto lane_geom = [&](int tid, int &lane, int &wid, int &g, int &c4, int &fl, int &sp, int &goff, bool &head) {
        lane = tid & 63;
        wid = __builtin_amdgcn_readfirstlane(tid >> 6);
        g = lane >> lg;
        c4 = lane & ((1 << lg) - 1);
        fl = min(c4, NF - 1);
        head = c4 == 0;
        sp = fl;
        goff = min(fl * 4, Df - 4);
    };
    float my_step[4], my_rcp[4], tab_step[4];
    auto fetch_steps = [&](int place) {
        const int g0 = ST.f.n == 1 ? 0 : min(place * 4, Df - 4);
#pragma unroll
        for (int i = 0; i < 4; ++i) tab_step[i] = ST.f.v[g0 + i];
    };
    auto use_steps = [&]() {
#pragma unroll
        for (int i = 0; i < 4; ++i) {
            my_step[i] = ST.f.n == 1 ? ST.f.v[0] : tab_step[i];
            my_rcp[i] = refined_rcp(my_step[i]);
        }
    };

    int tid = tid0;
    asm volatile("" : "+v"(tid));
    int lane, wid, g, c4, fl, sp, goff; bool head;
    lane_geom(tid, lane, wid, g, c4, fl, sp, goff, head);
    const int64_t e0 = tile_id * R;
    const int nt = (int)min((int64_t)R, A.n_entries - e0);
    MX_STAMP(0);
    if constexpr (!MULTI) fetch_steps(fl);

    const uint32_t *pg = P.prog + (uint64_t)tile_id * P.prog_stride;
    const int end_v = ((const uint16_t *)pg)[lane];
    const int endm_v = lane ? ((const uint16_t *)pg)[lane - 1] : 0;
    uint32_t surv_raw = A.surv_off ? A.surv_off[tile_id + (tid0 & 1)] : 0u;
    uint32_t m_rw[SLOTS], m_rec[SLOTS];
    W16 m_ab[SLOTS];
#pragma unroll
    for (int s = 0; s < SLOTS; ++s) {
        const int j = tid0 + s * nthreads;
        m_rw[s] = 0; m_rec[s] = 0; m_ab[s].v[0] = 0.0; m_ab[s].v[1] = 0.0;
        if (j < nt) {
            m_rw[s] = pg[32 + j];
            m_rec[s] = pg[32 + R + j];
            if (!P.prog_compact) m_ab[s] = ((const W16 *)(pg + P.prog_ab))[j];
        }
    }
    auto early_loads_landed = [&]() {
        asm volatile("" : "+v"(surv_raw));
        if constexpr (!MULTI) asm volatile("" : "+v"(tab_step[0]), "+v"(tab_step[1]), "+v"(tab_step[2]), "+v"(tab_step[3]));
    };
    auto fin_of = [&](uint32_t rw) { return (rw >> 31) != 0 || (A.last_stage && !ROOTS); };
    auto write_dst = [&]() {
#pragma unroll
        for (int s = 0; s < SLOTS; ++s) {
            const int j = tid0 + s * nthreads;
            if (j < nt) sdst[j] = (int32_t)((m_rw[s] & 0x7fffffffu) | (fin_of(m_rw[s]) ? 0x80000000u : 0u));
        }
    };
    auto write_survivors = [&](uint32_t n_merged) {
#pragma unroll
        for (int s = 0; s < SLOTS; ++s) {
            const uint32_t k = (uint32_t)(tid0 + s * nthreads);
            if (k >= n_merged && k < (uint32_t)nt) ssurv[k - n_merged] = (uint16_t)m_rec[s];
        }
    };
    auto write_records = [&](uint32_t n_merged) {
#pragma unroll
        for (int s = 0; s < SLOTS; ++s) {
            const uint32_t k = (uint32_t)(tid0 + s * nthreads);
            if (k < n_merged) {
                uint32_t pj = m_rec[s];
                W16 ab = m_ab[s];
                if (P.prog_compact) {
                    const uint32_t j = pj & 1023u, l = (pj >> 10) & 1023u, r = (pj >> 20) & 1023u;
                    const double w0 = (double)(int)l, w1 = (double)(int)r;
                    const double den = w0 + w1;
                    ab.v[0] = sqrt(w0 / den);
                    ab.v[1] = sqrt(w1 / den);
                    pj = (j - l) | (j << 16);
                }
                rec_ab[k] = ab;
                rec_pj[k] = pj;
            }
        }
    };

    auto load_linear = [&](const float *dst, int chunks, const float *src) {
        const uint32_t lds0 = (uint32_t)(uintptr_t)(__attribute__((address_space(3))) const void *)dst;
        for (int it = wid; (it << 6) < chunks; it += nwv) {
            const int c = (it << 6) + lane;
            if (c < chunks) glds16<0>(src + (uint32_t)c * 4u, lds0 + ((uint32_t)it << 10));
        }
    };
    auto load_caller_rows = [&](int rows, auto src) {
        const uint32_t lds0 = (uint32_t)(uintptr_t)(__attribute__((address_space(3))) const void *)ftile;
        const int total = rows * NF;
        for (int it = wid; (it << 6) < total; it += nwv) {
            const int c = (it << 6) + lane;
            const int jr = (int)(((uint32_t)c * NFm) >> 20), ch = c - jr * NF;
            if (c < total) { const void *a = src(jr, (uint32_t)min(ch * 4, Df - 4)); if (a) glds16<1>(a, lds0 + ((uint32_t)it << 10)); }
        }
    };
    auto widen_row = [&](int j) {
        double *row = wd + __mul24(j, nwide);
        const V16 raw = *(const V16 *)(ftile + __mul24(j, Fp));
        double d[4];
#pragma unroll
        for (int i = 0; i < 4; ++i) d[i] = i < nwide ? (double)raw.v[i] : 0.0;
#pragma unroll
        for (int i = 0; i < 4; ++i) if (i < nwide) row[i] = d[i];
    };

    if constexpr (!INV) {
        if constexpr (IDENT) {
            const uint32_t ldc = (uint32_t)A.ld_in;
            const float *src = A.in + e0 * (int64_t)ldc;
            load_caller_rows(nt, [&](int jr, uint32_t go) { return row_at(src, (uint32_t)jr, ldc, go); });
        } else {
            load_linear(ftile, nt * NF, A.in + e0 * (int64_t)Fp);
            load_linear((const float *)wd, (nt * nwide + 1) >> 1, (const float *)(P.in_w + e0 * (int64_t)nwide));
        }
        MX_STAMP(9);
        const uint32_t n_merged = (uint32_t)__builtin_amdgcn_readlane(end_v, 63);
        write_dst();
        write_survivors(n_merged);
        write_records(n_merged);
        MX_STAMP(1);
        wait_landed();
        early_loads_landed();
        sync_lds();
        MX_STAMP(2);
        if constexpr (IDENT) {
#pragma unroll
            for (int s = 0; s < SLOTS; ++s) {
                const int j = tid + s * nthreads;
                if (j < nt) widen_row(j);
            }
            sync_lds();
        }
        MX_STAMP(3);
        MX_STAMP(4);
    } else {
        const uint32_t n_merged = (uint32_t)__builtin_amdgcn_readlane(end_v, 63);
        write_dst();
        write_survivors(n_merged);
        MX_STAMP(1);
        sync_lds();
        MX_STAMP(2);
        load_caller_rows(nt, [&](int jr, uint32_t go) -> const void * {
            const uint32_t d = (uint32_t)sdst[jr];
            return (d >> 31) ? (const void *)row_far((const int32_t *)A.Q, d & 0x7fffffffu, (uint32_t)A.ldq, go) : nullptr; });
        write_records(n_merged);
        const uint32_t surv_base = (uint32_t)__builtin_amdgcn_readlane((int)surv_raw, 0);
        const uint32_t surv_cnt = (uint32_t)__builtin_amdgcn_readlane((int)surv_raw, 1) - surv_base;
        if (!A.last_stage) {
            if (c4 < NF) for (uint32_t it = wid; (it << lr) < surv_cnt; it += nwv) {
                const uint32_t qc = min((it << lr) + g, surv_cnt - 1);
                const V16 x = ld_chunk<float>(row_at((const float *)A.wsn + (int64_t)surv_base * Fp, qc, (uint32_t)Fp, (uint32_t)(fl * 4)));
                *(V16 *)&ftile[__mul24((int)ssurv[qc], Fp) + fl * 4] = x;
            }
            for (uint32_t c = (uint32_t)tid; c < surv_cnt * (uint32_t)nwide; c += (uint32_t)nthreads) {
                const uint32_t qc = c / (uint32_t)nwide, i = c - qc * (uint32_t)nwide;
                wd[__mul24((int)ssurv[qc], nwide) + i] = P.wsn_w[(int64_t)surv_base * nwide + c];
            }
        } else if (ROOTS) {
            if (c4 < NF) for (uint32_t it = wid; (it << lr) < surv_cnt; it += nwv) {
                const uint32_t qc = min((it << lr) + g, surv_cnt - 1);
                const V16 x = ld_chunk<float>(A.root_buf + (int64_t)(surv_base + qc) * Df + goff);
                *(V16 *)&ftile[__mul24((int)ssurv[qc], Fp) + fl * 4] = x;
            }
            for (uint32_t c = (uint32_t)tid; c < surv_cnt * (uint32_t)nwide; c += (uint32_t)nthreads) {
                const uint32_t qc = c / (uint32_t)nwide, i = c - qc * (uint32_t)nwide;
                wd[__mul24((int)ssurv[qc], nwide) + i] = P.root_w[(int64_t)surv_base * nwide + c];
            }
        }
        MX_STAMP(3);
        wait_landed();
        early_loads_landed();
        sync_lds();
        MX_STAMP(4);
        use_steps();
#pragma unroll
        for (int s = 0; s < SLOTS; ++s) {
            const int j = tid0 + s * nthreads;
            if (j < nt && fin_of(m_rw[s])) {
                double *row = wd + __mul24(j, nwide);
                const I16 raw = *(const I16 *)(ftile + __mul24(j, Fp));
#pragma unroll
                for (int i = 0; i < 4; ++i) if (i < nwide) row[i] = (double)raw.v[i] * ST.w[i];
            }
        }
        if (A.last_stage && !ROOTS) {
            const uint32_t n_fin = (uint32_t)nt - n_merged;
            if (c4 < NF) for (uint32_t it = wid; (it << lr) < n_fin; it += nwv) {
                const uint32_t qc = (it << lr) + g;
                if (qc < n_fin) {
                    V16 *pr = (V16 *)&ftile[__mul24((int)ssurv[qc], Fp) + fl * 4];
                    const I16 raw = *(const I16 *)pr;
                    V16 x;
#pragma unroll
                    for (int i = 0; i < 4; ++i)
                        x.v[i] = (head && i < nwide) ? __int_as_float(raw.v[i]) : (float)raw.v[i] * my_step[i];
                    *pr = x;
                }
            }
        }
        sync_lds();
    }
    MX_STAMP(5);
    {
        const uint32_t stride = (uint32_t)(nwv << lr);
        const uint32_t gw = (uint32_t)lane >> lgw, cw = (uint32_t)min(lane & ((1 << lgw) - 1), nwide - 1);
        const uint32_t bw = 64u >> lgw;
        const uint32_t cf = (uint32_t)fl * 4u;
        bool chained = false;
        const int loff_v = endm_v, hist_v = end_v - endm_v;
        uint64_t mask = __ballot(hist_v > 0);
        while (mask) {
            const int l = INV ? (63 - __clzll((long long)mask)) : (__ffsll((long long)mask) - 1);
            mask &= ~(1ull << l);
            const uint32_t base = (uint32_t)__builtin_amdgcn_readlane(loff_v, l), cnt = (uint32_t)__builtin_amdgcn_readlane(hist_v, l);
            auto apply_f = [&](auto UC, uint32_t mb) {
                constexpr int U = decltype(UC)::value;
                W16 ab[U];
                uint32_t pj[U];
#pragma unroll
                for (int u = 0; u < U; ++u) { const uint32_t m = base + min(mb + u * stride + g, cnt - 1); pj[u] = rec_pj[m]; ab[u] = rec_ab[m]; }
                uint32_t ip[U], ij[U];
                V16 x0[U], x1[U];
#pragma unroll
                for (int u = 0; u < U; ++u) { ip[u] = __umul24(pj[u] & 0xffffu, (uint32_t)Fp) + cf; ij[u] = __umul24(pj[u] >> 16, (uint32_t)Fp) + cf; }
#pragma unroll
                for (int u = 0; u < U; ++u) { x0[u] = *(const V16 *)&ftile[ip[u]]; x1[u] = *(const V16 *)&ftile[ij[u]]; }
                if constexpr (INV) {
#pragma unroll
                    for (int u = 0; u < U; ++u) {
#pragma unroll
                        for (int i = 0; i < 4; ++i) x1[u].v[i] = (float)__float_as_int(x1[u].v[i]) * my_step[i];
                    }
                }
#pragma unroll
                for (int u = 0; u < U; ++u) {
                    const float ca = (float)ab[u].v[0], cb = (float)ab[u].v[1];
                    V16 lo, hi;
#pragma unroll
                    for (int i = 0; i < 4; ++i) {
                        if (!INV) {
                            lo.v[i] = ca * x0[u].v[i] + cb * x1[u].v[i];
                            hi.v[i] = ca * x1[u].v[i] - cb * x0[u].v[i];
                        } else {
                            lo.v[i] = ca * x0[u].v[i] - cb * x1[u].v[i];
                            hi.v[i] = cb * x0[u].v[i] + ca * x1[u].v[i];
                        }
                    }
                    if (u == 0 || mb + u * stride < cnt) { *(V16 *)&ftile[ip[u]] = lo; *(V16 *)&ftile[ij[u]] = hi; }
                }
            };
            auto pass_f = [&](auto UC) {
                constexpr int U = decltype(UC)::value;
                for (uint32_t mb = (uint32_t)(wid << lr); mb < cnt; mb += stride * U) apply_f(UC, mb);
            };
            auto apply_w = [&](uint32_t m0) {
                const uint32_t m = base + min(m0 + gw, cnt - 1);
                const uint32_t pj = rec_pj[m];
                const W16 ab = rec_ab[m];
                const uint32_t ip = __umul24(pj & 0xffffu, (uint32_t)nwide) + cw, ij = __umul24(pj >> 16, (uint32_t)nwide) + cw;
                const double d0 = wd[ip], d1 = wd[ij];
                const double ca = ab.v[0], cb = ab.v[1];
                double lo, hi;
                if (!INV) {
                    lo = ca * d0 + cb * d1;
                    hi = ca * d1 - cb * d0;
                } else {
                    lo = ca * d0 - cb * d1;
                    hi = cb * d0 + ca * d1;
                }
                wd[ip] = lo; wd[ij] = hi;
            };
            if (cnt <= (1u << lr)) {
                if (wid == 0) pass_f(std::integral_constant<int, 1>());
                else if (wid == 1) { for (uint32_t m0 = 0; m0 < cnt; m0 += bw) apply_w(m0); }
                chained = true;
            } else {
                if (chained) { __syncthreads(); chained = false; }
                if (cnt <= stride) pass_f(std::integral_constant<int, 1>());
                else pass_f(std::integral_constant<int, TILE_ROUND_U>());
                for (uint32_t m0 = (uint32_t)(nwv - 1 - wid) * bw; m0 < cnt; m0 += (uint32_t)nwv * bw) apply_w(m0);
                __syncthreads();
            }
        }
        if (chained) __syncthreads();
    }

    MX_STAMP(6);
    {
        int tid5 = tid0;
        asm volatile("" : "+v"(tid5));
        lane_geom(tid5, lane, wid, g, c4, fl, sp, goff, head);
    }
    const bool rowlane = c4 < NF;
    if constexpr (INV) {
        if constexpr (IDENT) {
            float *base = A.out + e0 * A.ld_out;
            double acc[4] = {0.0, 0.0, 0.0, 0.0};
            const float *rbase = SQ ? A.ref + e0 * A.ld_ref : nullptr;
            if (rowlane) for (int it = wid; (it << lr) < nt; it += 2 * nwv) {
                int j[2]; V16 x[2]; double w[2][4] = {};
                V16 c[2];
                if constexpr (SQ) {
#pragma unroll
                    for (int u = 0; u < 2; ++u)
                        c[u] = ld_chunk<float, true>(row_at(rbase, (uint32_t)min(((it + u * nwv) << lr) + g, nt - 1), (uint32_t)A.ld_ref, (uint32_t)goff));
                }
#pragma unroll
                for (int u = 0; u < 2; ++u) {
                    j[u] = min(((it + u * nwv) << lr) + g, nt - 1);
                    x[u] = *(const V16 *)&ftile[__mul24(j[u], Fp) + sp * 4];
                }
                if (head) {
#pragma unroll
                    for (int u = 0; u < 2; ++u) {
#pragma unroll
                        for (int i = 0; i < 4; ++i) w[u][i] = wd[__mul24(j[u], nwide) + min(i, nwide - 1)];
                    }
                }
                asm volatile("" : "+v"(w[0][0]), "+v"(w[0][1]), "+v"(w[0][2]), "+v"(w[0][3]), "+v"(w[1][0]), "+v"(w[1][1]), "+v"(w[1][2]), "+v"(w[1][3]));
#pragma unroll
                for (int u = 0; u < 2; ++u) {
#pragma unroll
                    for (int i = 0; i < 4; ++i) { const float f = (float)w[u][i]; x[u].v[i] = (head && i < nwide) ? f : x[u].v[i]; }
                    asm volatile("" : "+v"(x[u].v[0]), "+v"(x[u].v[1]), "+v"(x[u].v[2]), "+v"(x[u].v[3]));
                    if constexpr (SQ) {
                        if (u == 0 || ((it + nwv) << lr) < nt) {
                            if (A.out) st_chunk<float, true>(row_at(base, (uint32_t)j[u], (uint32_t)A.ld_out, (uint32_t)goff), x[u]);
                            if (((it + u * nwv) << lr) + g < nt) {
#pragma unroll
                                for (int i = 0; i < 4; ++i) { const float d = x[u].v[i] - c[u].v[i]; acc[i] += (double)d * (double)d; }
                            }
                        }
                    } else if (u == 0 || ((it + nwv) << lr) < nt) {
                        st_chunk<float, true>(row_at(base, (uint32_t)j[u], (uint32_t)A.ld_out, (uint32_t)goff), x[u]);
                    }
                }
            }
            if constexpr (SQ) {
#pragma unroll
                for (int i = 0; i < 4; ++i) {
                    for (int sh = 1 << lg; sh < 64; sh <<= 1) acc[i] += __shfl_xor(acc[i], sh, 64);
                }
                __syncthreads();
                double *sacc = (double *)smem;
                if (g == 0 && rowlane) {
#pragma unroll
                    for (int i = 0; i < 4; ++i) sacc[(wid * NF + c4) * 4 + i] = acc[i];
                }
                __syncthreads();
                if (tid0 < NF * 4) {
                    double t = 0.0;
                    for (int w = 0; w < nwv; ++w) t += sacc[w * NF * 4 + tid0];
                    A.sq_part[tile_id * (NF * 4) + tid0] = t;
                }
            }
        } else {
            float *bf = A.out + e0 * (int64_t)Fp;
            double *bw_ = P.out_w + e0 * (int64_t)nwide;
            for (int c = tid; c < nt * NF; c += nthreads) st_chunk<float>(bf + c * 4, *(const V16 *)&ftile[c * 4]);
            for (int c = tid; c < nt * nwide; c += nthreads) bw_[c] = wd[c];
        }
    } else {
        if (!A.last_stage || ROOTS) {
            const uint32_t surv_base = (uint32_t)__builtin_amdgcn_readlane((int)surv_raw, 0);
            const uint32_t surv_cnt = (uint32_t)__builtin_amdgcn_readlane((int)surv_raw, 1) - surv_base;
            constexpr bool to_roots = ROOTS;
            float *bf = to_roots ? A.root_buf + (int64_t)surv_base * Df : A.wsn + (int64_t)surv_base * Fp;
            double *bw_ = (to_roots ? P.root_w : P.wsn_w) + (int64_t)surv_base * nwide;
            const uint32_t ldb = (uint32_t)(to_roots ? Df : Fp), cb = (uint32_t)(to_roots ? goff : fl * 4);
            if (c4 < NF) for (uint32_t it = wid; (it << lr) < surv_cnt; it += nwv) {
                const uint32_t q = min((it << lr) + g, surv_cnt - 1);
                const V16 x = *(const V16 *)&ftile[__mul24((int)ssurv[q], Fp) + fl * 4];
                st_chunk<float>(row_at(bf, q, ldb, cb), x);
            }
            for (uint32_t c = (uint32_t)tid; c < surv_cnt * (uint32_t)nwide; c += (uint32_t)nthreads) {
                const uint32_t q = c / (uint32_t)nwide, i = c - q * (uint32_t)nwide;
                bw_[c] = wd[__mul24((int)ssurv[q], nwide) + i];
            }
        }
        if constexpr (MULTI) {
            int32_t *qa = (int32_t *)rec_ab;
            auto store_step = [&](auto fast_div, int32_t *Qd) {
                if (rowlane) for (int it = wid; (it << lr) < nt; it += 2 * nwv) {
                    int jc[2]; V16 x[2]; I16 qi[2] = {}; uint32_t dv[2];
#pragma unroll
                    for (int u = 0; u < 2; ++u) {
                        jc[u] = min(((it + u * nwv) << lr) + g, nt - 1);
                        x[u] = *(const V16 *)&ftile[__mul24(jc[u], Fp) + sp * 4];
                        dv[u] = (uint32_t)sdst[jc[u]];
                    }
                    if (head) {
#pragma unroll
                        for (int u = 0; u < 2; ++u) {
#pragma unroll
                            for (int i = 0; i < 4; ++i) qi[u].v[i] = qa[__mul24(jc[u], nwide) + min(i, nwide - 1)];
                        }
                    }
                    asm volatile("" : "+v"(x[0].v[0]), "+v"(x[1].v[0]), "+v"(qi[0].v[0]), "+v"(qi[0].v[1]), "+v"(qi[0].v[2]), "+v"(qi[0].v[3]),
                                 "+v"(qi[1].v[0]), "+v"(qi[1].v[1]), "+v"(qi[1].v[2]), "+v"(qi[1].v[3]));
#pragma unroll
                    for (int u = 0; u < 2; ++u) {
                        I16 qv;
#pragma unroll
                        for (int i = 0; i < 4; ++i) {
                            const int32_t q = quantize_one(x[u].v[i], my_step[i], my_rcp[i], decltype(fast_div)::value);
                            qv.v[i] = (head && i < nwide) ? qi[u].v[i] : q;
                        }
                        asm volatile("" : "+v"(qv.v[0]), "+v"(qv.v[1]), "+v"(qv.v[2]), "+v"(qv.v[3]));
                        if ((dv[u] >> 31) && (u == 0 || ((it + nwv) << lr) < nt))
                            st_chunk<int32_t, true>(row_far(Qd, dv[u] & 0x7fffffffu, (uint32_t)A.ldq, (uint32_t)goff), qv);
                    }
                }
            };
            for (int kk = 0; kk < MQ->k; ++kk) {
                const double sw = MQ->step[kk];
#pragma unroll
                for (int s = 0; s < SLOTS; ++s) {
                    const int j = tid0 + s * nthreads;
                    if (j < nt && ((uint32_t)sdst[j] >> 31)) {
                        const double *row = &wd[__mul24(j, nwide)];
                        int32_t *qrow = &qa[__mul24(j, nwide)];
#pragma unroll
                        for (int i = 0; i < 4; ++i) if (i < nwide) qrow[i] = quantize_one_f64(row[i], sw);
                    }
                }
                sync_lds();
                const float sf = (float)sw, rf = refined_rcp(sf);
#pragma unroll
                for (int i = 0; i < 4; ++i) { my_step[i] = sf; my_rcp[i] = rf; }
                if ((MQ->fast_div >> kk) & 1u) store_step(std::true_type(), MQ->Q[kk]);
                else store_step(std::false_type(), MQ->Q[kk]);
                sync_lds();
            }
        } else {
            MX_STAMP(10);
#pragma unroll
            for (int s = 0; s < SLOTS; ++s) {
                const int j = tid0 + s * nthreads;
                if (j < nt && ((uint32_t)sdst[j] >> 31)) {
                    double *row = &wd[__mul24(j, nwide)];
                    double d[4] = {0.0, 0.0, 0.0, 0.0};
#pragma unroll
                    for (int i = 0; i < 4; ++i) if (i < nwide) d[i] = row[i];
                    asm volatile("" ::: "memory");
                    int32_t *qrow = (int32_t *)row;
#pragma unroll
                    for (int i = 0; i < 4; ++i) if (i < nwide) qrow[i] = quantize_one_f64(d[i], ST.w[i]);
                }
            }
            sync_lds();
            MX_STAMP(7);
            use_steps();
#ifdef RAHT_PHASE_CLOCKS
            asm volatile("" :: "v"(my_step[0]), "v"(my_rcp[3]));
#endif
            MX_STAMP(11);
            auto store_final = [&](auto fast_div) {
                if (rowlane) for (int it = wid; (it << lr) < nt; it += 2 * nwv) {
                    int jc[2]; V16 x[2]; I16 qi[2] = {}; uint32_t dv[2];
#pragma unroll
                    for (int u = 0; u < 2; ++u) {
                        jc[u] = min(((it + u * nwv) << lr) + g, nt - 1);
                        x[u] = *(const V16 *)&ftile[__mul24(jc[u], Fp) + sp * 4];
                        dv[u] = (uint32_t)sdst[jc[u]];
                    }
                    if (head) {
#pragma unroll
                        for (int u = 0; u < 2; ++u) {
                            const int32_t *qrow = (const int32_t *)&wd[__mul24(jc[u], nwide)];
#pragma unroll
                            for (int i = 0; i < 4; ++i) qi[u].v[i] = qrow[min(i, nwide - 1)];
                        }
                    }
                    asm volatile("" : "+v"(x[0].v[0]), "+v"(x[1].v[0]), "+v"(qi[0].v[0]), "+v"(qi[0].v[1]), "+v"(qi[0].v[2]), "+v"(qi[0].v[3]),
                                 "+v"(qi[1].v[0]), "+v"(qi[1].v[1]), "+v"(qi[1].v[2]), "+v"(qi[1].v[3]));
#pragma unroll
                    for (int u = 0; u < 2; ++u) {
                        I16 qv;
#pragma unroll
                        for (int i = 0; i < 4; ++i) {
                            const int32_t q = quantize_one(x[u].v[i], my_step[i], my_rcp[i], decltype(fast_div)::value);
                            qv.v[i] = (head && i < nwide) ? qi[u].v[i] : q;
                        }
                        asm volatile("" : "+v"(qv.v[0]), "+v"(qv.v[1]), "+v"(qv.v[2]), "+v"(qv.v[3]));
                        if ((dv[u] >> 31) && (u == 0 || ((it + nwv) << lr) < nt))
                            st_chunk<int32_t, true>(row_far(A.Q, dv[u] & 0x7fffffffu, (uint32_t)A.ldq, (uint32_t)goff), qv);
                    }
                }
            };
            if (ST.f.fast_div) store_final(std::true_type()); else store_final(std::false_type());
        }
    }
    MX_STAMP(8);
}

template <bool INV, bool IDENT, int SLOTS>
__global__ __launch_bounds__(MX_THREADS, 6) void tile_kernel_mx(const TileArgs<float> A, const MxPtrs P, const StepTableMX ST)
{
    tile_body_mx<INV, IDENT, SLOTS, false>(A, P, ST, (int64_t)blockIdx.x);
}
template <bool INV, bool IDENT, int SLOTS>
__global__ __launch_bounds__(MX_THREADS, 6) void tile_kernel_mx_roots(const TileArgs<float> A, const MxPtrs P, const StepTableMX ST)
{
    tile_body_mx<INV, IDENT, SLOTS, true>(A, P, ST, (int64_t)blockIdx.x);
}
template <bool IDENT, int SLOTS>
__global__ __launch_bounds__(MX_THREADS, 6) void tile_kernel_mx_multi(const TileArgs<float> A, const MxPtrs P, const StepTableMX ST, const MxMultiQ M)
{
    tile_body_mx<false, IDENT, SLOTS, false, true, false>(A, P, ST, (int64_t)blockIdx.x, &M);
}
template <int SLOTS>
__global__ __launch_bounds__(MX_THREADS, 6) void tile_kernel_mx_sq(const TileArgs<float> A, const MxPtrs P, const StepTableMX ST)
{
    tile_body_mx<true, true, SLOTS, false, false, true>(A, P, ST, (int64_t)blockIdx.x);
}

struct TileBatchMX {
    TileArgs<float> a[BATCH_MAX];
    MxPtrs p[BATCH_MAX];
    uint32_t first_tile[BATCH_MAX + 1];
    int n;
};
static_assert(sizeof(TileBatchMX) + sizeof(StepTableMX) <= 4096, "tile_kernel_mx_batch: arguments exceed the 4 KB kernarg segment");

template <bool INV, bool IDENT, int SLOTS>
__global__ __launch_bounds__(MX_THREADS, 6) void tile_kernel_mx_batch(const TileBatchMX B, const StepTableMX ST)
{
    int s = 0;
#pragma unroll
    for (int q = 1; q < BATCH_MAX; ++q) s += (q < B.n && blockIdx.x >= B.first_tile[q]) ? 1 : 0;
    tile_body_mx<INV, IDENT, SLOTS, false>(B.a[s], B.p[s], ST, (int64_t)(blockIdx.x - B.first_tile[s]));
}

struct TopArgsMX {
    const float *in_rows;  int64_t ld_in;
    const float *in_img; const double *in_img_w;
    float *out_rows;       int64_t ld_out;
    float *out_img; double *out_img_w;
    int32_t *Q;            int64_t ldq;
    const uint32_t *e_pos;
    const uint32_t *pj;
    const float *ab32;  const double *ab64;
    int n, n_merges, D, nwide, Fp;
    const uint32_t *lev;
    int nlev, nbig;
    uint32_t small_start;
    const uint32_t *root_rank;
    float *root_f; double *root_w;
};

template <bool WIDE, bool INV, bool ROOTS, bool MULTI = false>
__device__ __forceinline__ void top_body_mx(const TopArgsMX &A, const StepTableMX &ST, const int chunk, const MxMultiQ *MQ = nullptr)
{
    typedef typename std::conditional<WIDE, double, float>::type T;
    constexpr int VN = WIDE ? 2 : 4;
    typedef RegChunk<T> V16;
    extern __shared__ __align__(16) unsigned char smem[];
    V16 *tile = (V16 *)smem;
    __shared__ uint32_t s_lev[2 * 64];
    const int tid = threadIdx.x;
    const int nwide = A.nwide;
    const int goff = WIDE ? 2 * chunk : min(chunk * 4, A.D - 4);
    const int ioff = chunk * 4;
    const int n = A.n, nm = A.n_merges;
    if (tid < 2 * A.nlev) s_lev[tid] = A.lev[tid];
    const T *ab = WIDE ? (const T *)A.ab64 : (const T *)A.ab32;
    const int n_small = nm - (int)A.small_start;
    uint32_t *s_pj = (uint32_t *)(smem + (size_t)n * 16);
    T *s_ab = (T *)(s_pj + ((n_small + 3) & ~3));
    for (int i = tid; i < n_small; i += MX_TOP_THREADS) {
        s_pj[i] = A.pj[A.small_start + i];
        s_ab[2 * i] = ab[2 * (A.small_start + i)];
        s_ab[2 * i + 1] = ab[2 * (A.small_start + i) + 1];
    }
    T my_step[VN];
    float my_rcp[VN];
    bool live[VN];
#pragma unroll
    for (int i = 0; i < VN; ++i) {
        if constexpr (WIDE) { live[i] = goff + i < nwide; my_step[i] = live[i] ? ST.w[goff + i] : 1.0; my_rcp[i] = 1.0f; }
        else { live[i] = !(chunk == 0 && i < nwide); my_step[i] = ST.f.v[ST.f.n == 1 ? 0 : goff + i]; my_rcp[i] = refined_rcp(my_step[i]); }
    }
    uint32_t pj[MX_TOP_SLOTS];
    T ra[MX_TOP_SLOTS], rb[MX_TOP_SLOTS];
#pragma unroll
    for (int k = 0; k < MX_TOP_SLOTS; ++k) {
        const int idx = min(k * MX_TOP_THREADS + tid, max(nm - 1, 0));
        pj[k] = A.pj[idx]; ra[k] = ab[2 * idx]; rb[k] = ab[2 * idx + 1];
    }
    uint32_t m_dst[MX_TOP_SLOTS], m_rr[MX_TOP_SLOTS];
#pragma unroll
    for (int k = 0; k < MX_TOP_SLOTS; ++k) {
        m_dst[k] = A.e_pos[min(k * MX_TOP_THREADS + tid, n - 1)];
        m_rr[k] = ROOTS ? A.root_rank[min(k * MX_TOP_THREADS + tid, n - 1)] : 0xffffffffu;
    }
#pragma unroll
    for (int k = 0; k < MX_TOP_SLOTS; ++k) {
        const int e = k * MX_TOP_THREADS + tid;
        if (e >= n) continue;
        V16 v;
        if constexpr (!INV) {
            if (A.in_img) {
                if constexpr (WIDE) {
#pragma unroll
                    for (int i = 0; i < VN; ++i) v.v[i] = live[i] ? A.in_img_w[(int64_t)e * nwide + goff + i] : 0.0;
                } else {
                    v = *(const V16 *)(A.in_img + (int64_t)e * A.Fp + ioff);
                }
            } else if constexpr (WIDE) {
#pragma unroll
                for (int i = 0; i < VN; ++i) v.v[i] = live[i] ? (double)A.in_rows[(int64_t)e * A.ld_in + goff + i] : 0.0;
            } else {
                v = ld_chunk<float>(A.in_rows + (int64_t)e * A.ld_in + goff);
            }
        } else if (m_rr[k] != 0xffffffffu) {
            if constexpr (WIDE) {
#pragma unroll
                for (int i = 0; i < VN; ++i) v.v[i] = live[i] ? A.root_w[(int64_t)m_rr[k] * nwide + goff + i] : 0.0;
            } else {
                v = ld_chunk<float>(A.root_f + (int64_t)m_rr[k] * A.D + goff);
            }
        } else {
            const int32_t *q = A.Q + (int64_t)m_dst[k] * A.ldq + goff;
            if constexpr (WIDE) {
#pragma unroll
                for (int i = 0; i < VN; ++i) v.v[i] = live[i] ? (double)q[i] * my_step[i] : 0.0;
            } else {
                const RegChunk<int32_t> raw = ld_chunk<int32_t>(q);
#pragma unroll
                for (int i = 0; i < VN; ++i) v.v[i] = (float)raw.v[i] * my_step[i];
            }
        }
        tile[e] = v;
    }
    __syncthreads();

    auto butterfly = [&](uint32_t rec, T a, T b) {
        const uint32_t ip = rec & 0xffffu, ij = rec >> 16;
        const V16 x0 = tile[ip], x1 = tile[ij];
        V16 vlo, vhi;
#pragma unroll
        for (int i = 0; i < VN; ++i) {
            if (!INV) {
                vlo.v[i] = a * x0.v[i] + b * x1.v[i];
                vhi.v[i] = a * x1.v[i] - b * x0.v[i];
            } else {
                vlo.v[i] = a * x0.v[i] - b * x1.v[i];
                vhi.v[i] = b * x0.v[i] + a * x1.v[i];
            }
        }
        tile[ip] = vlo; tile[ij] = vhi;
    };
    auto big_levels = [&]() {
#pragma unroll 1
        for (int q = 0; q < A.nbig; ++q) {
            const int li = INV ? A.nbig - 1 - q : q;
            const uint32_t lo = s_lev[2 * li], hi = s_lev[2 * li + 1];
#pragma unroll
            for (int k = 0; k < MX_TOP_SLOTS; ++k) {
                const uint32_t idx = (uint32_t)(k * MX_TOP_THREADS + tid);
                if ((uint32_t)(k * MX_TOP_THREADS) < hi && (uint32_t)((k + 1) * MX_TOP_THREADS) > lo && idx >= lo && idx < hi)
                    butterfly(pj[k], ra[k], rb[k]);
            }
            __syncthreads();
        }
    };
    auto small_levels = [&]() {
        if (tid < 64) {
#pragma unroll 1
            for (int q = A.nbig; q < A.nlev; ++q) {
                const int li = INV ? A.nlev - 1 - (q - A.nbig) : q;
                const uint32_t lo = s_lev[2 * li], hi = s_lev[2 * li + 1];
                const uint32_t i = lo - A.small_start + (uint32_t)tid;
                if (lo + (uint32_t)tid < hi) butterfly(s_pj[i], s_ab[2 * i], s_ab[2 * i + 1]);
            }
        }
        __syncthreads();
    };
    if (!INV) { big_levels(); small_levels(); }
    else { small_levels(); big_levels(); }

#pragma unroll
    for (int k = 0; k < MX_TOP_SLOTS; ++k) {
        const int e = k * MX_TOP_THREADS + tid;
        if (e >= n) continue;
        const V16 v = tile[e];
        if constexpr (INV) {
            if (A.out_img) {
                if constexpr (WIDE) {
#pragma unroll
                    for (int i = 0; i < VN; ++i) if (live[i]) A.out_img_w[(int64_t)e * nwide + goff + i] = v.v[i];
                } else {
                    *(V16 *)(A.out_img + (int64_t)e * A.Fp + ioff) = v;
                }
            } else if constexpr (WIDE) {
#pragma unroll
                for (int i = 0; i < VN; ++i) if (live[i]) A.out_rows[(int64_t)e * A.ld_out + goff + i] = (float)v.v[i];
            } else if (chunk == 0) {
#pragma unroll
                for (int i = 0; i < VN; ++i) if (live[i]) A.out_rows[(int64_t)e * A.ld_out + goff + i] = v.v[i];
            } else {
                st_chunk<float>(A.out_rows + (int64_t)e * A.ld_out + goff, v);
            }
        } else if (m_rr[k] != 0xffffffffu) {
            if constexpr (WIDE) {
#pragma unroll
                for (int i = 0; i < VN; ++i) if (live[i]) A.root_w[(int64_t)m_rr[k] * nwide + goff + i] = v.v[i];
            } else {
                st_chunk<float>(A.root_f + (int64_t)m_rr[k] * A.D + goff, v);
            }
        } else if constexpr (MULTI) {
            for (int kk = 0; kk < MQ->k; ++kk) {
                int32_t *q = MQ->Q[kk] + (int64_t)m_dst[k] * A.ldq + goff;
                if constexpr (WIDE) {
#pragma unroll
                    for (int i = 0; i < VN; ++i) if (live[i]) q[i] = quantize_one_f64(v.v[i], MQ->step[kk]);
                } else {
                    const float sf = (float)MQ->step[kk], rf = refined_rcp(sf);
                    const int fd = (int)((MQ->fast_div >> kk) & 1u);
                    RegChunk<int32_t> qv;
#pragma unroll
                    for (int i = 0; i < VN; ++i) qv.v[i] = quantize_one(v.v[i], sf, rf, fd);
                    if (chunk == 0) {
#pragma unroll
                        for (int i = 0; i < VN; ++i) if (live[i]) q[i] = qv.v[i];
                    } else {
                        st_chunk<int32_t>(q, qv);
                    }
                }
            }
        } else {
            int32_t *q = A.Q + (int64_t)m_dst[k] * A.ldq + goff;
            if constexpr (WIDE) {
#pragma unroll
                for (int i = 0; i < VN; ++i) if (live[i]) q[i] = quantize_one_f64(v.v[i], my_step[i]);
            } else {
                RegChunk<int32_t> qv;
#pragma unroll
                for (int i = 0; i < VN; ++i) qv.v[i] = quantize_one(v.v[i], my_step[i], my_rcp[i], ST.f.fast_div);
                if (chunk == 0) {
#pragma unroll
                    for (int i = 0; i < VN; ++i) if (live[i]) q[i] = qv.v[i];
                } else {
                    st_chunk<int32_t>(q, qv);
                }
            }
        }
    }
}

template <bool INV>
__global__ __launch_bounds__(MX_TOP_THREADS) void top_kernel_mx(const TopArgsMX A, const StepTableMX ST)
{
    const int NW2 = (A.nwide + 1) >> 1;
    if ((int)blockIdx.x < NW2) top_body_mx<true, INV, false>(A, ST, (int)blockIdx.x);
    else top_body_mx<false, INV, false>(A, ST, (int)blockIdx.x - NW2);
}
template <bool INV>
__global__ __launch_bounds__(MX_TOP_THREADS) void top_kernel_mx_roots(const TopArgsMX A, const StepTableMX ST)
{
    const int NW2 = (A.nwide + 1) >> 1;
    if ((int)blockIdx.x < NW2) top_body_mx<true, INV, true>(A, ST, (int)blockIdx.x);
    else top_body_mx<false, INV, true>(A, ST, (int)blockIdx.x - NW2);
}

struct TopBatchMX { TopArgsMX a[BATCH_MAX]; };
static_assert(sizeof(TopBatchMX) + sizeof(StepTableMX) <= 4096, "top_kernel_mx_batch: arguments exceed the 4 KB kernarg segment");

template <bool INV>
__global__ __launch_bounds__(MX_TOP_THREADS) void top_kernel_mx_batch(const TopBatchMX B, const StepTableMX ST)
{
    const TopArgsMX &A = B.a[blockIdx.y];
    const int NW2 = (A.nwide + 1) >> 1;
    if ((int)blockIdx.x < NW2) top_body_mx<true, INV, false>(A, ST, (int)blockIdx.x);
    else top_body_mx<false, INV, false>(A, ST, (int)blockIdx.x - NW2);
}

__global__ __launch_bounds__(MX_TOP_THREADS) void top_kernel_mx_multi(const TopArgsMX A, const StepTableMX ST, const MxMultiQ M)
{
    const int NW2 = (A.nwide + 1) >> 1;
    if ((int)blockIdx.x < NW2) top_body_mx<true, false, false, true>(A, ST, (int)blockIdx.x, &M);
    else top_body_mx<false, false, false, true>(A, ST, (int)blockIdx.x - NW2, &M);
}

__global__ void mx_cols_to_f64_kernel(const float *__restrict__ C, int64_t ldc, int64_t N, int nwide, double *__restrict__ W)
{
    const int64_t e = (int64_t)blockIdx.x * blockDim.x + threadIdx.x;
    if (e >= N * nwide) return;
    const int64_t i = e / nwide;
    W[e] = (double)C[i * ldc + (e - i * nwide)];
}
__global__ void mx_cols_from_f64_kernel(const double *__restrict__ W, int64_t N, int nwide, float *__restrict__ C, int64_t ldc)
{
    const int64_t e = (int64_t)blockIdx.x * blockDim.x + threadIdx.x;
    if (e >= N * nwide) return;
    const int64_t i = e / nwide;
    C[i * ldc + (e - i * nwide)] = (float)W[e];
}

struct MxGeom {
    int nwide = 0, NCp = 0, Dp = 0, lg = 0;
    int R0 = 0, R1 = 0, Rf = 0;
};
// ... 104 lines not shown
        L.n_tiles = 0;
        return RAHT_OK;
    }
    TileArgs<float> &A = L.A;
    A.rows = st.rows; A.surv_off = st.surv_off; A.n_entries = st.n_entries; A.N = p->N; A.R = st.tile_rows;
    A.D = D; A.Dc = D; A.Dp = g.Dp; A.lg = g.lg; A.nwide = g.nwide;
    A.last_stage = (k == K - 1) ? 1 : 0;
    A.wsum = p->wsum;
    const StageArrays a = stage_arrays(p, st);
    A.lvl = a.lvl; A.wl = a.wl; A.wr = a.wr; A.inv_order = a.pos; A.ht = a.ht;
    A.Q = io.Q; A.ldq = io.ldq;
    A.top_level = p->top_level; A.root_buf = A.last_stage ? (float *)p->root_buf : nullptr; A.dbg = 0; A.ref = nullptr; A.ld_ref = 0; A.sq_part = nullptr;
    A.ld_ws = g.Dp; A.wsn = ws_n;
    A.fin = nullptr; A.ld_fin = 0;
    if (!INV) { A.in = (k == 0) ? io.C_in : ws_k; A.ld_in = (k == 0) ? io.ldc : g.Dp; A.out = nullptr; A.ld_out = 0; }
    else { A.in = nullptr; A.ld_in = 0; A.out = (k == 0) ? io.C_out : ws_k; A.ld_out = (k == 0) ? io.ldc : g.Dp; }
    {
        const char *bad = nullptr;
        if (!A.lvl || !A.wl || !A.wr || !A.ht) bad = "plan arrays";
        else if (!A.last_stage && (!A.wsn || !A.surv_off)) bad = "survivor workspace of a non-final stage";
        else if (!A.Q || !A.inv_order) bad = "Q / inv_order";
        else if (!INV && !A.in) bad = "forward input";
        else if (INV && !A.out && !(k == 0 && io.sq_part)) bad = "inverse output";
        else if (k == 0 && io.sq_part && (!INV || !io.ref || A.root_buf || (int64_t)st.tile_rows * io.ld_ref * 4 >= ((int64_t)1 << 31))) bad = "sqdiff reference rows";
        else if (!INV && io.multi && A.root_buf) bad = "multi-step write-back without root buffers";
        else if ((st.rows == nullptr) != (k == 0)) bad = "stage order";
        else if (st.tile_rows < 1 || st.tile_rows > TILE_MAX_SLOTS * MX_THREADS ||
                 (int64_t)st.tile_rows * std::max<int64_t>(io.ldc, g.Dp) * 4 >= ((int64_t)1 << 31)) bad = "tile geometry (32-bit row offsets)";
        if (bad) { set_error("mixed tile stage %d (%s): missing %s", k, INV ? "inverse" : "forward", bad); return RAHT_ERR_INVALID; }
    }
    MxPtrs &P = L.P;
    P.in_w = (!INV && k >= 1) ? ws_k_w : nullptr;
    P.out_w = (INV && k >= 1) ? ws_k_w : nullptr;
    P.wsn_w = ws_n_w;
    P.root_w = A.last_stage ? p->root_buf_w : nullptr;
    P.prog = st.prog; P.prog_stride = st.prog_stride; P.prog_ab = st.prog_ab; P.prog_compact = st.prog_compact ? 1 : 0;
    if (!P.prog) { set_error("mixed tile stage %d: missing tile programs", k); return RAHT_ERR_INVALID; }
    L.lds = tile_lds_bytes_mx(st.tile_rows, g.Dp / 4, g.nwide);
    L.n_tiles = (unsigned)st.n_tiles;
    if (INV && k == 0 && io.sq_part) {
        A.out = io.C_out; A.ld_out = io.C_out ? io.ldc : 0;
        A.ref = io.ref; A.ld_ref = io.ld_ref; A.sq_part = io.sq_part;
    }
    return RAHT_OK;
}

template <bool INV>
static int launch_prepared_mx(const raht_plan *p, int k, const MxIO &io, const MxStageLaunch &L, const MxGeom &g,
                              const StepTableMX &stp, hipStream_t s)
{
    auto launch = [&]() -> int {
        if (L.is_top) {
            const dim3 grid((unsigned)g.NCp), block(MX_TOP_THREADS);
            if constexpr (!INV) { if (io.multi) return launch_lds<top_kernel_mx_multi>(grid, block, L.lds, TOP_LDS_LIMIT, s, L.T, stp, *io.multi); }
            if (L.T.root_f) return launch_lds<top_kernel_mx_roots<INV>>(grid, block, L.lds, TOP_LDS_LIMIT, s, L.T, stp);
            return launch_lds<top_kernel_mx<INV>>(grid, block, L.lds, TOP_LDS_LIMIT, s, L.T, stp);
        }
        if constexpr (!INV) { if (io.multi) return launch_tile_mx<false, false, MX_MULTI>(k == 0, L.A, L.P, stp, io.multi, L.n_tiles, L.lds, s); }
        if constexpr (INV) { if (k == 0 && io.sq_part) return launch_tile_mx<true, false, MX_SQ>(true, L.A, L.P, stp, nullptr, L.n_tiles, L.lds, s); }
        return L.A.root_buf ? launch_tile_mx<INV, true, MX_PLAIN>(k == 0, L.A, L.P, stp, nullptr, L.n_tiles, L.lds, s)
                            : launch_tile_mx<INV, false, MX_PLAIN>(k == 0, L.A, L.P, stp, nullptr, L.n_tiles, L.lds, s);
    };
    if (!(k == 0 && p->ev_before)) return launch();
    RAHT_HIP_CHECK(hipEventRecord(p->ev_before, s));
    const int rc = launch();
    RAHT_HIP_CHECK(hipEventRecord(p->ev_after, s));
    return rc;
}

template <bool INV>
static int launch_stage_mx(const raht_plan *p, const Schedule &sc, int k, const MxIO &io, int D, const MxGeom &g,
                           const StepTableMX &stp, hipStream_t s)
{
    MxStageLaunch L;
    RAHT_RET((prepare_stage_mx<INV>(p, sc, k, io, D, g, L)));
    return launch_prepared_mx<INV>(p, k, io, L, g, stp, s);
}

static int mx_check_args(const raht_plan *p, const void *a, const void *b, int D, int64_t lda, int64_t ldb, const double *steps,
                         int n_steps, int n_wide, const char *what)
{
    if (!p || !a || !b || D < 1 || lda < D || ldb < D) { set_error("%s: bad argument", what); return RAHT_ERR_INVALID; }
    RAHT_RET(check_plan_device(p, what));
    if (n_wide < 1 || n_wide > MX_MAX_WIDE || n_wide > D) { set_error("%s: n_wide must be 1..%d (and <= D)", what, MX_MAX_WIDE); return RAHT_ERR_INVALID; }
    RAHT_RET(check_quant_steps(what, steps, n_steps, D, true));
    if (p->row_map) { set_error("%s: not available for row-mapped plans", what); return RAHT_ERR_UNSUPPORTED; }
    if ((p->root_buf == nullptr) != (p->root_buf_w == nullptr)) {
        set_error("%s: set both root buffers (raht_plan_set_root_buffer and raht_plan_set_root_buffer_wide) or neither", what);
        return RAHT_ERR_UNSUPPORTED;
    }
    if (p->top_level < 64 && !p->root_buf) {
        set_error("%s: a truncated plan needs both root buffers (raht_plan_set_root_buffer, raht_plan_set_root_buffer_wide)", what);
        return RAHT_ERR_UNSUPPORTED;
    }
    return RAHT_OK;
}

template <typename F>
static int with_wide_roots(raht_plan *p, F &&call)
{
    void *const saved = p->root_buf;
    if (saved) p->root_buf = p->root_buf_w;
    const int rc = call();
    p->root_buf = saved;
    return rc;
}

static int mx_setup(raht_plan *p, int D, int n_wide, int64_t max_ld, hipStream_t s, Schedule **sc_out, MxGeom &g)
{
    *sc_out = nullptr;
    if (p->engine == RAHT_ENGINE_LEVEL || max_ld > ((int64_t)1 << 18)) return RAHT_OK;
    if (!mx_geometry(p, D, n_wide, g)) return RAHT_OK;
    Schedule *sc = nullptr;
    RAHT_RET(get_schedule(p, g.R0, g.R1, g.Rf, s, &sc));
    if (!sc->valid) return RAHT_OK;
    RAHT_RET(build_tile_programs(p, sc, s));
    RAHT_RET(ensure_workspace(sc, (size_t)g.Dp * 4 + (size_t)g.nwide * 8 + 8, p->split_ws));
    *sc_out = sc;
    return RAHT_OK;
}

static int fwd_quant_mixed_impl(const raht_plan *cp, const float *C, int64_t ldc, int D, const double *steps, int n_steps, int n_wide,
                                int32_t *Q, int64_t ldq, raht_stream_t stream)
{
    raht_plan *p = const_cast<raht_plan *>(cp);
    hipStream_t s = (hipStream_t)stream;
    RAHT_RET(mx_check_args(p, C, Q, D, ldc, ldq, steps, n_steps, n_wide, "raht_fwd_quant_mixed"));
    Schedule *sc = nullptr;
    MxGeom g;
    RAHT_RET(mx_setup(p, D, n_wide, std::max(ldc, ldq), s, &sc, g));
    if (!sc) {
        float f[MAX_STEP_CH];
        for (int c = 0; c < n_steps; ++c) f[c] = (float)steps[c];
        RAHT_RET(raht_fwd_quant(p, C, ldc, D, f, n_steps, Q, ldq, stream));
        Scratch tmp(sizeof(double) * 2 * (size_t)p->N * (size_t)n_wide, s);
        if (!tmp.ok()) return RAHT_ERR_NOMEM;
        double *W = tmp.as<double>(), *TW = W + (size_t)p->N * n_wide;
        hipLaunchKernelGGL(mx_cols_to_f64_kernel, dim3((unsigned)ceil_div(p->N * n_wide, 256)), dim3(256), 0, s, C, ldc, p->N, n_wide, W);
        RAHT_HIP_CHECK(hipGetLastError());
        RAHT_RET(with_wide_roots(p, [&]() { return raht_fwd_f64(p, W, n_wide, n_wide, TW, n_wide, nullptr, stream); }));
        double ws[MX_MAX_WIDE];
        for (int i = 0; i < n_wide; ++i) ws[i] = steps[n_steps == 1 ? 0 : i];
        return raht_quant_reorder_f64(p, TW, n_wide, n_wide, ws, n_wide, Q, ldq, stream);
    }
    StepTableMX stp;
    fill_steps_mx(stp, steps, n_steps, n_wide);
    MxIO io;
    io.C_in = C; io.ldc = ldc; io.Q = Q; io.ldq = ldq;
    const int K = (int)sc->stages.size();
    for (int k = 0; k < K; ++k) RAHT_RET((launch_stage_mx<false>(p, *sc, k, io, D, g, stp, s)));
    return RAHT_OK;
}

static int dequant_inv_mixed_impl(const raht_plan *cp, const int32_t *Q, int64_t ldq, int D, const double *steps, int n_steps, int n_wide,
                                  float *C, int64_t ldc, raht_stream_t stream)
{
    raht_plan *p = const_cast<raht_plan *>(cp);
    hipStream_t s = (hipStream_t)stream;
    RAHT_RET(mx_check_args(p, Q, C, D, ldq, ldc, steps, n_steps, n_wide, "raht_dequant_inv_mixed"));
    Schedule *sc = nullptr;
    MxGeom g;
    RAHT_RET(mx_setup(p, D, n_wide, std::max(ldc, ldq), s, &sc, g));
    if (!sc) {
        float f[MAX_STEP_CH];
        for (int c = 0; c < n_steps; ++c) f[c] = (float)steps[c];
        RAHT_RET(raht_dequant_inv(p, Q, ldq, D, f, n_steps, C, ldc, stream));
        Scratch tmp(sizeof(double) * 2 * (size_t)p->N * (size_t)n_wide, s);
        if (!tmp.ok()) return RAHT_ERR_NOMEM;
        double *W = tmp.as<double>(), *TW = W + (size_t)p->N * n_wide;
        double ws[MX_MAX_WIDE];
        for (int i = 0; i < n_wide; ++i) ws[i] = steps[n_steps == 1 ? 0 : i];
        RAHT_RET(raht_dequant_unreorder_f64(p, Q, ldq, n_wide, ws, n_wide, TW, n_wide, stream));
        RAHT_RET(with_wide_roots(p, [&]() { return raht_inv_f64(p, TW, n_wide, n_wide, W, n_wide, stream); }));
        hipLaunchKernelGGL(mx_cols_from_f64_kernel, dim3((unsigned)ceil_div(p->N * n_wide, 256)), dim3(256), 0, s, W, p->N, n_wide, C, ldc);
        RAHT_HIP_CHECK(hipGetLastError());
        return RAHT_OK;
    }
    StepTableMX stp;
    fill_steps_mx(stp, steps, n_steps, n_wide);
    MxIO io;
    io.C_out = C; io.ldc = ldc; io.Q = const_cast<int32_t *>(Q); io.ldq = ldq;
    const int K = (int)sc->stages.size();
    for (int k = K - 1; k >= 0; --k) RAHT_RET((launch_stage_mx<true>(p, *sc, k, io, D, g, stp, s)));
    return RAHT_OK;
}

static int fwd_quant_mixed_multi_impl(const raht_plan *cp, const float *C, int64_t ldc, int D, const double *steps, int k, int n_wide,
                                      int32_t *const *Q, int64_t ldq, raht_stream_t stream)
{
    const char *what = "raht_fwd_quant_mixed_multi";
    raht_plan *p = const_cast<raht_plan *>(cp);
    hipStream_t s = (hipStream_t)stream;
    if (!p || !C || !Q || !steps || k < 1) { set_error("%s: bad argument (plan, C, Q, steps must be set, k >= 1)", what); return RAHT_ERR_INVALID; }
    for (int i = 0; i < k; ++i) {
        if (!Q[i]) { set_error("%s: Q[%d] is NULL", what, i); return RAHT_ERR_INVALID; }
        for (int j = 0; j < i; ++j) if (Q[j] == Q[i]) { set_error("%s: Q[%d] and Q[%d] are the same matrix", what, j, i); return RAHT_ERR_INVALID; }
    }
    for (int i = 0; i < k; ++i) RAHT_RET(mx_check_args(p, C, Q[i], D, ldc, ldq, &steps[i], 1, n_wide, what));
    Schedule *sc = nullptr;
    MxGeom g;
    if (!p->root_buf) RAHT_RET(mx_setup(p, D, n_wide, std::max(ldc, ldq), s, &sc, g));
    if (!sc) {
        for (int i = 0; i < k; ++i) RAHT_RET(fwd_quant_mixed_impl(p, C, ldc, D, &steps[i], 1, n_wide, Q[i], ldq, stream));
        return RAHT_OK;
    }
    const int K = (int)sc->stages.size();
    for (int k0 = 0; k0 < k; k0 += MULTI_Q_MAX) {
        MxMultiQ M;
        M.k = std::min(MULTI_Q_MAX, k - k0);
        M.fast_div = 0;
        for (int i = 0; i < MULTI_Q_MAX; ++i) {
            M.step[i] = steps[k0 + std::min(i, M.k - 1)];
            M.Q[i] = Q[k0 + std::min(i, M.k - 1)];
            const float f = (float)M.step[i];
            if (f >= 0x1p-100f && f <= 0x1p100f) M.fast_div |= 1u << i;
        }
        StepTableMX stp;
        fill_steps_mx(stp, &steps[k0], 1, n_wide);
        MxIO io;
        io.C_in = C; io.ldc = ldc; io.Q = M.Q[0]; io.ldq = ldq; io.multi = &M;
        for (int kk = 0; kk < K; ++kk) RAHT_RET((launch_stage_mx<false>(p, *sc, kk, io, D, g, stp, s)));
    }
    return RAHT_OK;
}

static int dequant_inv_mixed_sqdiff_impl(const raht_plan *cp, const int32_t *Q, int64_t ldq, int D, const double *steps, int n_steps,
                                         int n_wide, const float *Cref, int64_t ldref, float *Crec, int64_t ldc, double *sq,
                                         raht_stream_t stream)
{
    const char *what = "raht_dequant_inv_mixed_sqdiff";
    raht_plan *p = const_cast<raht_plan *>(cp);
    hipStream_t s = (hipStream_t)stream;
    if (!p || !Q || !Cref || !sq || D < 1 || ldref < D || (Crec && ldc < D)) { set_error("%s: bad argument (plan, Q, C_ref, sqdiff must be set)", what); return RAHT_ERR_INVALID; }
    RAHT_RET(mx_check_args(p, Q, Cref, D, ldq, ldref, steps, n_steps, n_wide, what));
    Schedule *sc = nullptr;
    MxGeom g;
    if (!p->root_buf) RAHT_RET(mx_setup(p, D, n_wide, std::max(std::max(ldq, ldref), Crec ? ldc : (int64_t)D), s, &sc, g));
    if (!sc || sc->stages.size() < 2 || sc->stages[0].is_top) {
        Scratch tmp(Crec ? 16 : sizeof(float) * (size_t)p->N * (size_t)D, s);
        if (!tmp.ok()) return RAHT_ERR_NOMEM;
        float *out = Crec ? Crec : tmp.as<float>();
        const int64_t ldo = Crec ? ldc : D;
        RAHT_RET(dequant_inv_mixed_impl(p, Q, ldq, D, steps, n_steps, n_wide, out, ldo, stream));
        return raht_sqdiff_columns(Cref, ldref, out, ldo, p->N, D, RAHT_F32, sq, stream);
    }
    const int ncv = g.Dp;
    const Stage &st0 = sc->stages[0];
    Scratch part(sizeof(double) * (size_t)st0.n_tiles * (size_t)ncv, s);
    if (!part.ok()) return RAHT_ERR_NOMEM;
    if ((size_t)(MX_THREADS / 64) * (size_t)ncv * 8 > tile_lds_bytes_mx(st0.tile_rows, g.Dp / 4, g.nwide)) {
        set_error("%s: unexpected stage-0 geometry", what);
        return RAHT_ERR_INVALID;
    }
    StepTableMX stp;
    fill_steps_mx(stp, steps, n_steps, n_wide);
    MxIO io;
    io.C_out = Crec; io.ldc = Crec ? ldc : 0; io.Q = const_cast<int32_t *>(Q); io.ldq = ldq;
    io.ref = Cref; io.ld_ref = ldref; io.sq_part = part.as<double>();
    const int K = (int)sc->stages.size();
    for (int k = K - 1; k >= 0; --k) RAHT_RET((launch_stage_mx<true>(p, *sc, k, io, D, g, stp, s)));
    return launch_sq_final(part.as<double>(), (int64_t)st0.n_tiles, D, ncv, sq, s);
}

struct MxScene {
    raht_plan *p = nullptr;
    Schedule *sc = nullptr;
    MxGeom g;
    MxIO io;
};

static bool mx_batchable(const raht_plan *p, const Schedule *sc)
{
    return sc && !p->root_buf && !p->root_buf_w && p->top_level >= 64 && !p->ev_before;
}

struct MxShape {
    bool ident; int slots; size_t lds; int nwide, NCp, Dp, lg;
    bool operator==(const MxShape &o) const
    { return ident == o.ident && slots == o.slots && lds == o.lds && nwide == o.nwide && NCp == o.NCp && Dp == o.Dp && lg == o.lg; }
};
static MxShape mx_tile_shape(const Stage &st, int k, const MxGeom &g)
{
    return MxShape{k == 0, st.tile_rows <= MX_THREADS ? 1 : 2, tile_lds_bytes_mx(st.tile_rows, g.Dp / 4, g.nwide), g.nwide, g.NCp, g.Dp, g.lg};
}

template <bool INV, typename FS, typename FT, typename FP>
static int group_mx_scenes(int n, const MxScene *scn, BatchCounts &cnt, FS &&single, FT &&tile, FP &&top)
{
    return group_batch_rounds<INV>(n, [&](int i) { return scn[i].sc ? (int)scn[i].sc->stages.size() : 0; },
                                   [&](int i, int k) { return scn[i].sc->stages[(size_t)k].is_top; },
                                   [&](int i, int j, int k) { return mx_tile_shape(scn[i].sc->stages[(size_t)k], k, scn[i].g) == mx_tile_shape(scn[j].sc->stages[(size_t)k], k, scn[j].g); },
                                   [&](int i, int j, int) { return scn[i].g.NCp == scn[j].g.NCp && scn[i].g.Dp == scn[j].g.Dp; },
                                   cnt, single, tile, top);
}

template <bool INV>
static int launch_tile_batch_mx(int m, const MxStageLaunch *const *Ls, bool ident, const StepTableMX &stp, hipStream_t s)
{
    TileBatchMX B;
    B.n = m;
    uint32_t tot = 0;
    for (int i = 0; i < BATCH_MAX; ++i) {
        B.a[i] = Ls[i < m ? i : 0]->A;
        B.p[i] = Ls[i < m ? i : 0]->P;
        B.first_tile[i] = tot;
        if (i < m) tot += Ls[i]->n_tiles;
    }
    B.first_tile[BATCH_MAX] = tot;
    return by_ident_slots(ident, Ls[0]->A.R <= MX_THREADS, [&](auto id, auto slots) -> int {
        return launch_lds<tile_kernel_mx_batch<INV, decltype(id)::value, decltype(slots)::value>>(dim3(tot), dim3(MX_THREADS), Ls[0]->lds, TILE_LDS_LIMIT, s, B, stp);
    });
}

template <bool INV>
static int launch_top_batch_mx(int m, const MxStageLaunch *const *Ls, int NCp, const StepTableMX &stp, hipStream_t s)
{
    TopBatchMX B;
    size_t lds = 0;
    for (int i = 0; i < BATCH_MAX; ++i) B.a[i] = Ls[i < m ? i : 0]->T;
    for (int i = 0; i < m; ++i) lds = std::max(lds, Ls[i]->lds);
    return launch_lds<top_kernel_mx_batch<INV>>(dim3((unsigned)NCp, (unsigned)m), dim3(MX_TOP_THREADS), lds, TOP_LDS_LIMIT, s, B, stp);
}

static int mx_batch_check_args(const char *what, int n, raht_plan *const *plans, const void *const *a, const int64_t *lda,
                               const void *const *b, const int64_t *ldb, int D, const double *steps, int n_steps, int n_wide)
{
    if (n < 1 || !plans || !a || !lda || !b || !ldb || D < 1) { set_error("%s: bad argument (n >= 1, D >= 1, the arrays of plans, matrices and strides must be set)", what); return RAHT_ERR_INVALID; }
    if (n_wide < 1 || n_wide > MX_MAX_WIDE || n_wide > D) { set_error("%s: n_wide must be 1..%d (and <= D)", what, MX_MAX_WIDE); return RAHT_ERR_INVALID; }
    RAHT_RET(check_quant_steps(what, steps, n_steps, D, true));
    RAHT_RET(check_batch_plans(what, n, plans));
    for (int i = 0; i < n; ++i)
        if (!a[i] || !b[i] || lda[i] < D || ldb[i] < D) { set_error("%s: bad matrix argument (scene %d: NULL pointer or row stride < D)", what, i); return RAHT_ERR_INVALID; }
    return RAHT_OK;
}

static int mx_batch_check_plan(const char *what, int i, const raht_plan *p, const void *a, const void *b, int D, int64_t lda, int64_t ldb,
// ... 31 lines not shown
        const MxScene &S = scn[(size_t)i];
        if (!S.sc) continue;
        for (int k = 0; k < (int)S.sc->stages.size(); ++k) {
            const int rc = prepare_stage_mx<INV>(S.p, *S.sc, k, S.io, D, S.g, prep[first[(size_t)i] + (size_t)k]);
            if (rc != RAHT_OK) {
                const std::string msg = raht_last_error();
                set_error("%s: %s (scene %d)", what, msg.c_str(), i);
                return rc;
            }
        }
    }
    StepTableMX stp;
    fill_steps_mx(stp, steps, n_steps, n_wide);
    auto stage_of = [&](int i, int k) -> const MxStageLaunch & { return prep[first[(size_t)i] + (size_t)k]; };
    auto single = [&](int i) -> int {
        const MxIO &io = scn[(size_t)i].io;
        if constexpr (INV) return dequant_inv_mixed_impl(scn[(size_t)i].p, io.Q, io.ldq, D, steps, n_steps, n_wide, io.C_out, io.ldc, (raht_stream_t)s);
        else return fwd_quant_mixed_impl(scn[(size_t)i].p, io.C_in, io.ldc, D, steps, n_steps, n_wide, io.Q, io.ldq, (raht_stream_t)s);
    };
    auto tile = [&](int m, const int *idx, int k) -> int {
        if (m == 1) return launch_prepared_mx<INV>(scn[(size_t)idx[0]].p, k, scn[(size_t)idx[0]].io, stage_of(idx[0], k), scn[(size_t)idx[0]].g, stp, s);
        const MxStageLaunch *Ls[BATCH_MAX];
        for (int q = 0; q < m; ++q) Ls[q] = &stage_of(idx[q], k);
        return launch_tile_batch_mx<INV>(m, Ls, k == 0, stp, s);
    };
    auto top = [&](int m, const int *idx, int k) -> int {
        if (m == 1) return launch_prepared_mx<INV>(scn[(size_t)idx[0]].p, k, scn[(size_t)idx[0]].io, stage_of(idx[0], k), scn[(size_t)idx[0]].g, stp, s);
        const MxStageLaunch *Ls[BATCH_MAX];
        for (int q = 0; q < m; ++q) Ls[q] = &stage_of(idx[q], k);
        return launch_top_batch_mx<INV>(m, Ls, scn[(size_t)idx[0]].g.NCp, stp, s);
    };
    BatchCounts cnt;
    return group_mx_scenes<INV>(n, scn.data(), cnt, single, tile, top);
}

static int mixed_batch_stats_impl(int n, raht_plan *const *plans, int D, int n_wide, int inverse, int *tile_launches, int *top_launches,
                                  int *single_scene_calls)
{
    const char *what = "raht_mixed_batch_stats";
    if (n < 1 || !plans || !tile_launches || !top_launches || !single_scene_calls || D < 1 || n_wide < 1 || n_wide > MX_MAX_WIDE || n_wide > D) {
        set_error("%s: bad argument", what);
        return RAHT_ERR_INVALID;
    }
    RAHT_RET(check_batch_plans(what, n, plans));
    std::vector<MxScene> scn((size_t)n);
    for (int i = 0; i < n; ++i) {
        MxScene &S = scn[(size_t)i];
        S.p = plans[i];
        RAHT_RET(check_plan_device(S.p, what));
        if (S.p->row_map) { set_error("%s: not available for row-mapped plans (scene %d)", what, i); return RAHT_ERR_UNSUPPORTED; }
        Schedule *sc = nullptr;
        RAHT_RET(mx_setup(S.p, D, n_wide, D, nullptr, &sc, S.g));
        S.sc = mx_batchable(S.p, sc) ? sc : nullptr;
    }
    BatchCounts cnt;
    auto none1 = [](int) { return (int)RAHT_OK; };
    auto none3 = [](int, const int *, int) { return (int)RAHT_OK; };
    if (inverse) RAHT_RET((group_mx_scenes<true>(n, scn.data(), cnt, none1, none3, none3)));
    else RAHT_RET((group_mx_scenes<false>(n, scn.data(), cnt, none1, none3, none3)));
    *tile_launches = cnt.tile; *top_launches = cnt.top; *single_scene_calls = cnt.single;
    return RAHT_OK;
}

}

using namespace raht;

extern "C" {

int raht_fwd_quant_mixed(const raht_plan *plan, const float *C, int64_t ldc, int D, const double *steps, int n_steps, int n_wide,
                         int32_t *Q, int64_t ldq, raht_stream_t stream)
{
    return guarded("raht_fwd_quant_mixed", [&]() { return fwd_quant_mixed_impl(plan, C, ldc, D, steps, n_steps, n_wide, Q, ldq, stream); });
}

int raht_dequant_inv_mixed(const raht_plan *plan, const int32_t *Q, int64_t ldq, int D, const double *steps, int n_steps, int n_wide,
                           float *C, int64_t ldc, raht_stream_t stream)
{
    return guarded("raht_dequant_inv_mixed", [&]() { return dequant_inv_mixed_impl(plan, Q, ldq, D, steps, n_steps, n_wide, C, ldc, stream); });
}

int raht_fwd_quant_mixed_multi(const raht_plan *plan, const float *C, int64_t ldc, int D, const double *steps, int k, int n_wide,
                               int32_t *const *Q, int64_t ldq, raht_stream_t stream)
{
    return guarded("raht_fwd_quant_mixed_multi", [&]() { return fwd_quant_mixed_multi_impl(plan, C, ldc, D, steps, k, n_wide, Q, ldq, stream); });
}

int raht_dequant_inv_mixed_sqdiff(const raht_plan *plan, const int32_t *Q, int64_t ldq, int D, const double *steps, int n_steps,
                                  int n_wide, const float *C_ref, int64_t ld_ref, float *C_rec, int64_t ldc, double *sqdiff,
                                  raht_stream_t stream)
{
    return guarded("raht_dequant_inv_mixed_sqdiff", [&]() {
        return dequant_inv_mixed_sqdiff_impl(plan, Q, ldq, D, steps, n_steps, n_wide, C_ref, ld_ref, C_rec, ldc, sqdiff, stream); });
}

int raht_fwd_quant_mixed_batch(int n, raht_plan *const *plans, const float *const *C, const int64_t *ldc, int D,
                               const double *steps, int n_steps, int n_wide, int32_t *const *Q, const int64_t *ldq, raht_stream_t stream)
{
    const char *what = "raht_fwd_quant_mixed_batch";
    return guarded(what, [&]() -> int {
        RAHT_RET(mx_batch_check_args(what, n, plans, (const void *const *)C, ldc, (const void *const *)Q, ldq, D, steps, n_steps, n_wide));
        std::vector<MxIO> ios((size_t)n);
        for (int i = 0; i < n; ++i) { MxIO &io = ios[(size_t)i]; io.C_in = C[i]; io.ldc = ldc[i]; io.Q = Q[i]; io.ldq = ldq[i]; }
        return run_batch_mx<false>(what, n, plans, ios.data(), D, steps, n_steps, n_wide, (hipStream_t)stream);
    });
}

int raht_dequant_inv_mixed_batch(int n, raht_plan *const *plans, const int32_t *const *Q, const int64_t *ldq, int D,
                                 const double *steps, int n_steps, int n_wide, float *const *C, const int64_t *ldc, raht_stream_t stream)
{
    const char *what = "raht_dequant_inv_mixed_batch";
    return guarded(what, [&]() -> int {
        RAHT_RET(mx_batch_check_args(what, n, plans, (const void *const *)Q, ldq, (const void *const *)C, ldc, D, steps, n_steps, n_wide));
        std::vector<MxIO> ios((size_t)n);
        for (int i = 0; i < n; ++i) { MxIO &io = ios[(size_t)i]; io.C_out = C[i]; io.ldc = ldc[i]; io.Q = const_cast<int32_t *>(Q[i]); io.ldq = ldq[i]; }
        return run_batch_mx<true>(what, n, plans, ios.data(), D, steps, n_steps, n_wide, (hipStream_t)stream);
    });
}

int raht_mixed_batch_stats(int n, raht_plan *const *plans, int D, int n_wide, int inverse, int *tile_launches, int *top_launches,
                           int *single_scene_calls)
{
    return guarded("raht_mixed_batch_stats", [&]() {
        return mixed_batch_stats_impl(n, plans, D, n_wide, inverse, tile_launches, top_launches, single_scene_calls); });
}

#ifdef RAHT_PHASE_CLOCKS
int raht_debug_read_phase_clocks_mx(unsigned long long *dst, int n_tiles)
{
    RAHT_HIP_CHECK(hipDeviceSynchronize());
    RAHT_HIP_CHECK(hipMemcpyFromSymbol(dst, HIP_SYMBOL(g_phase_clk_mx), sizeof(unsigned long long) * MX_CLK_SLOTS * (size_t)std::min(n_tiles, MX_CLK_TILES)));
    return MX_CLK_SLOTS;
}
#endif

int raht_plan_mixed_stats(raht_plan *plan, int D, int n_wide, int *tile_rows, int *n_stages, int64_t *rows_per_stage, int max_stages)
{
    return guarded("raht_plan_mixed_stats", [&]() -> int {
        if (!plan || !tile_rows || !n_stages || D < 1 || n_wide < 1 || n_wide > MX_MAX_WIDE) { set_error("raht_plan_mixed_stats: bad argument"); return RAHT_ERR_INVALID; }
        RAHT_RET(check_plan_device(plan, "raht_plan_mixed_stats"));
        *tile_rows = 0; *n_stages = 0;
        if (plan->row_map) return RAHT_OK;
        Schedule *sc = nullptr;
        MxGeom g;
        RAHT_RET(mx_setup(plan, D, n_wide, D, nullptr, &sc, g));
        if (!sc) return RAHT_OK;
        *tile_rows = g.R0;
        *n_stages = (int)sc->stages.size();
        for (int k = 0; k < *n_stages && k < max_stages && rows_per_stage; ++k) rows_per_stage[k] = sc->stages[(size_t)k].n_entries;
        return RAHT_OK;
    });
}

}
```

### raht-3dgs-codec_amd/ops.py

```python
import collections
import contextlib
import ctypes as C

import torch

from . import _lib
from ._lib import RahtError, check

_MAGIC = 0x52414854_504C414E
_plans = collections.OrderedDict()
_PLAN_CACHE = 16
_next_id = [1]


def _stream():
    return C.c_void_p(torch.cuda.current_stream().cuda_stream)


def _need_cuda(t, name):
    if not isinstance(t, torch.Tensor) or not t.is_cuda:
        raise RuntimeError(f"raht-3dgs-codec_amd: {name} must be a CUDA (HIP) tensor; this package has "
                           "no CPU path for the RAHT hot path")


# ... 283 lines not shown

    def prepare(self, D, dtype=torch.float32):
        es = 8 if dtype == torch.float64 else 4
        with torch.cuda.device(self.device):
            check(_lib.lib().raht_plan_prepare(self._h, es, int(D), _stream()))

    def set_row_map(self, row_map, n_matrix_rows):
        with torch.cuda.device(self.device):
            if row_map is None:
                check(_lib.lib().raht_plan_set_row_map(self._h, None, 0, _stream()))
                self.map_rows = None
                return
            m = row_map.to(device=self.device, dtype=torch.int64).contiguous()
            check(_lib.lib().raht_plan_set_row_map(self._h, C.c_void_p(m.data_ptr()), int(n_matrix_rows), _stream()))
        self.map_rows = int(n_matrix_rows)

    def set_concurrent_directions(self, on=True):
        with torch.cuda.device(self.device):
            check(_lib.lib().raht_plan_set_concurrent_directions(self._h, 1 if on else 0))

    def set_max_stages(self, max_stages):
        with torch.cuda.device(self.device):
            check(_lib.lib().raht_plan_set_max_stages(self._h, int(max_stages)))

    def _quant_to(self, name, src, steps, out_dtype, step_dtype, roots=None):
        D = src.shape[1]
        st = _step_array(steps, D, _STEP_CTYPE[step_dtype])
        dst = torch.empty((self.N, D), dtype=out_dtype, device=src.device)
        with self._with_roots(D, roots, step_dtype):
            self._quant(_fn(name, step_dtype), src, st, _p(dst), D)
        return dst

    def forward_quant(self, Cmat, steps, roots=None):
        X = _rows(Cmat, None, "C")
        return self._quant_to("raht_fwd_quant", X, steps, torch.int32, X.dtype, roots)

    def dequant_inverse(self, Q, steps, roots=None, dtype=torch.float32):
        dtype = torch.float64 if dtype == torch.float64 else torch.float32
        return self._quant_to("raht_dequant_inv", _qmat(Q), steps, dtype, dtype, roots)

    def forward_quant_multi(self, Cmat, steps):
        X = _rows(Cmat, torch.float32, "C")
        Qs, st, ptrs = self._multi_out(X, steps, C.c_float)
        self._quant(_lib.lib().raht_fwd_quant_multi, X, st, ptrs, X.shape[1])
        return Qs

    def _multi_out(self, X, steps, ctype):
        k = len(steps)
        Qs = [torch.empty((self.N, X.shape[1]), dtype=torch.int32, device=X.device) for _ in range(k)]
        return Qs, (ctype * k)(*[float(s) for s in steps]), (C.c_void_p * k)(*[q.data_ptr() for q in Qs])

    def dequant_inverse_sqdiff(self, Q, steps, C_ref, want_rec=True):
        Q, X, st, out, ssd = self._sqdiff_args(Q, steps, C_ref, want_rec, C.c_float)
        self._quant(_lib.lib().raht_dequant_inv_sqdiff, Q, st, _p(X), X.stride(0), _p(out), Q.shape[1], _p(ssd))
        return out, ssd

    def _sqdiff_args(self, Q, steps, C_ref, want_rec, ctype):
        _need_cuda(Q, "Q")
        _need_cuda(C_ref, "C_ref")
        Q = _qmat(Q)
        D = Q.shape[1]
        X = _rows(C_ref, torch.float32, "C_ref")
        st = _step_array(steps, D, ctype)
        out = torch.empty((self.N, D), dtype=torch.float32, device=Q.device) if want_rec else None
        return Q, X, st, out, torch.empty(D, dtype=torch.float64, device=Q.device)

    def forward_quant_mixed(self, Cmat, steps, n_wide=3, roots=None, roots_wide=None):
        X = _rows(Cmat, torch.float32, "C")
        D = X.shape[1]
        st = _step_array(steps, D, C.c_double)
        Q = torch.empty((self.N, D), dtype=torch.int32, device=X.device)
        with self._with_roots(D, roots, torch.float32, roots_wide, int(n_wide)):
            self._quant(_lib.lib().raht_fwd_quant_mixed, X, st, int(n_wide), _p(Q), D)
        return Q

    def dequant_inverse_mixed(self, Q, steps, n_wide=3, out=None, roots=None, roots_wide=None):
        Q = _qmat(Q)
        D = Q.shape[1]
        st = _step_array(steps, D, C.c_double)
        if out is None:
            out = torch.empty((self.N, D), dtype=torch.float32, device=Q.device)
        with self._with_roots(D, roots, torch.float32, roots_wide, int(n_wide)):
            self._quant(_lib.lib().raht_dequant_inv_mixed, Q, st, int(n_wide), _p(out), out.stride(0))
        return out

    def forward_quant_mixed_multi(self, Cmat, steps, n_wide=3, roots=None, roots_wide=None):
        X = _rows(Cmat, torch.float32, "C")
        D = X.shape[1]
        Qs, st, ptrs = self._multi_out(X, steps, C.c_double)
        with self._with_roots(D, roots, torch.float32, roots_wide, int(n_wide)):
            self._quant(_lib.lib().raht_fwd_quant_mixed_multi, X, st, int(n_wide), ptrs, D)
        return Qs

    def dequant_inverse_mixed_sqdiff(self, Q, steps, C_ref, n_wide=3, want_rec=True, roots=None, roots_wide=None):
        Q, X, st, out, ssd = self._sqdiff_args(Q, steps, C_ref, want_rec, C.c_double)
        D = Q.shape[1]
        with self._with_roots(D, roots, torch.float32, roots_wide, int(n_wide)):
            self._quant(_lib.lib().raht_dequant_inv_mixed_sqdiff, Q, st, int(n_wide), _p(X), X.stride(0), _p(out), D, _p(ssd))
        return out, ssd

    def rate_curve(self, Cmat, steps, n_wide=0, seg_len=2048):
        from .rlgr import SegmentedCoder
        _need_cuda(Cmat, "C")
        if self.map_rows is not None or self.n_roots != 1:
            raise ValueError("rate_curve: not available for row-mapped or truncated plans")
        n_wide = int(n_wide)
        if Cmat.dim() != 2 or Cmat.shape[0] != self.N or not 0 <= n_wide <= Cmat.shape[1]:
            raise ValueError(f"rate_curve: expected an ({self.N}, D) matrix and 0 <= n_wide <= D")
        D = int(Cmat.shape[1])
        rows = []
        for st in steps:
            r = step_list(st)
            if len(r) not in (1, D):
                raise ValueError("rate_curve: every step must be a scalar or have D entries")
            rows.append(r * D if len(r) == 1 else r)
        if not rows:
            raise ValueError("rate_curve: no steps")
        k = len(rows)
        scalar = all(len(set(r)) == 1 for r in rows)
        order = self.order_RAGFT
        parts = []
        with torch.cuda.device(self.device):
            if n_wide:
                Tw = self.forward(Cmat[:, :n_wide].to(torch.float64).contiguous(), want_w=False)
                Twq = torch.empty_like(Tw)
                rows_gather(Tw, order, Twq)
                parts.append((0, n_wide, Twq))
                del Tw
            if n_wide < D:
                T = self.forward(Cmat.to(torch.float32), want_w=False)
                Tq = torch.empty_like(T)
                rows_gather(T, order, Tq)
                parts.append((n_wide, D, Tq[:, n_wide:] if n_wide else Tq))
                del T
            payload = 0
            sse = torch.empty((k, D), dtype=torch.float64, device=self.device)
            G = 0
            for lo, hi, Tp in parts:
                st = [r[lo] for r in rows] if scalar else [r[lo:hi] for r in rows]
                nbytes, seg_bytes, e = SegmentedCoder.rate(Tp, st, seg_len, 1, True)
                Gp = seg_bytes.shape[1]
                payload = payload + (nbytes - SegmentedCoder.container_size(Gp, 0))
                G += Gp
                sse[:, lo:hi] = e
        return {"bytes": SegmentedCoder.container_size(G, payload), "sse": sse.cpu().numpy()}

    def mixed_stats(self, D=59, n_wide=3):
        tr, ns = C.c_int(0), C.c_int(0)
        rows = (C.c_int64 * 64)()
        with torch.cuda.device(self.device):
            check(_lib.lib().raht_plan_mixed_stats(self._h, int(D), int(n_wide), C.byref(tr), C.byref(ns), rows, 64))
        return {"tile_rows": tr.value, "rows_per_stage": [int(rows[i]) for i in range(ns.value)]}

    def quant_reorder(self, T, steps):
        T = _rows(T, None, "T")
        return self._quant_to("raht_quant_reorder", T, steps, torch.int32, T.dtype)

    def dequant_unreorder(self, Q, steps, dtype=torch.float32):
        dtype = torch.float64 if dtype == torch.float64 else torch.float32
        return self._quant_to("raht_dequant_unreorder", _qmat(Q), steps, dtype, dtype)


def _batch_arrays(plans, mats, dtype, name):
    n = len(plans)
    if n < 1 or len(mats) != n:
        raise ValueError("batch: one matrix per plan")
    D = int(mats[0].shape[1])
    ms = []
    for p, m in zip(plans, mats):
        _need_cuda(m, name)
        if m.dim() != 2 or m.shape[0] != p.N or m.shape[1] != D:
            raise ValueError(f"batch: expected ({p.N}, {D}) matrices, got {tuple(m.shape)}")
        if m.dtype != dtype:
            m = m.to(dtype)
        if m.stride(1) != 1 or m.stride(0) < D:
            m = m.contiguous()
        ms.append(m)
    hp = (C.c_void_p * n)(*[p._h for p in plans])
    mp = (C.c_void_p * n)(*[m.data_ptr() for m in ms])
    ld = (C.c_int64 * n)(*[m.stride(0) for m in ms])
    return n, D, ms, hp, mp, ld


def _batch_out(plans, D, dtype, device):
    outs = [torch.empty((p.N, D), dtype=dtype, device=device) for p in plans]
    return outs, (C.c_void_p * len(outs))(*[o.data_ptr() for o in outs]), (C.c_int64 * len(outs))(*[D] * len(outs))


@contextlib.contextmanager
def _batch_mixed_roots(plans, roots, roots_wide, D, n_wide):
    n = len(plans)
    roots = [None] * n if roots is None else list(roots)
    wide = [None] * n if roots_wide is None else list(roots_wide)
    if len(roots) != n or len(wide) != n:
        raise ValueError("batch: roots / roots_wide need one entry per plan (None allowed)")
    with contextlib.ExitStack() as stack:
        for p, r, w in zip(plans, roots, wide):
            stack.enter_context(p._with_roots(D, r, torch.float32, w, n_wide))
        yield


def _batch(fn, plans, mats, dtype, name, out_dtype, steps=None, ctype=None, n_wide=None, roots=None, roots_wide=None):
    n, D, ms, hp, mp, ld = _batch_arrays(plans, mats, dtype, name)
    mid = []
    if steps is not None:
        st = _step_array(steps, D, ctype)
        mid = [st, len(st)] if n_wide is None else [st, len(st), int(n_wide)]
    outs, op, old = _batch_out(plans, D, out_dtype, ms[0].device)
    with contextlib.nullcontext() if n_wide is None else _batch_mixed_roots(plans, roots, roots_wide, D, int(n_wide)):
        _call(fn, ms[0].device, n, hp, mp, ld, D, *mid, op, old)
    return outs


def forward_batch(plans, Cs):
    return _batch(_lib.lib().raht_fwd_batch, plans, Cs, torch.float32, "C", torch.float32)


def inverse_batch(plans, Ts):
    return _batch(_lib.lib().raht_inv_batch, plans, Ts, torch.float32, "T", torch.float32)


def forward_quant_batch(plans, Cs, steps):
    return _batch(_lib.lib().raht_fwd_quant_batch, plans, Cs, torch.float32, "C", torch.int32, steps, C.c_float)


def dequant_inverse_batch(plans, Qs, steps):
    return _batch(_lib.lib().raht_dequant_inv_batch, plans, Qs, torch.int32, "Q", torch.float32, steps, C.c_float)


def forward_quant_mixed_batch(plans, Cs, steps, n_wide=3, roots=None, roots_wide=None):
    return _batch(_lib.lib().raht_fwd_quant_mixed_batch, plans, Cs, torch.float32, "C", torch.int32, steps, C.c_double, n_wide, roots,
                  roots_wide)


def dequant_inverse_mixed_batch(plans, Qs, steps, n_wide=3, roots=None, roots_wide=None):
    return _batch(_lib.lib().raht_dequant_inv_mixed_batch, plans, Qs, torch.int32, "Q", torch.float32, steps, C.c_double, n_wide, roots,
                  roots_wide)


def mixed_batch_stats(plans, D, n_wide, inverse=False):
    n = len(plans)
    if n < 1:
        raise ValueError("batch: at least one plan")
    hp = (C.c_void_p * n)(*[p._h for p in plans])
    t, u, v = C.c_int(0), C.c_int(0), C.c_int(0)
    with torch.cuda.device(plans[0].device):
        check(_lib.lib().raht_mixed_batch_stats(n, hp, int(D), int(n_wide), 1 if inverse else 0, C.byref(t), C.byref(u), C.byref(v)))
    return {"tile_launches": t.value, "top_launches": u.value, "single_scene_calls": v.value}


def _quant_rows(X, steps, pos, Q, dtype):
    _need_cuda(X, "X")
    if X.shape[0] == 0:
        return Q
    if dtype == torch.float64 and X.dtype != dtype:
        raise ValueError("quant_rows_f64: X must be float64")
    X = _rows(X, dtype, "X")
    n, D = X.shape
    st = _step_array(steps, D, _STEP_CTYPE[dtype])
    pos = pos.to(torch.int64).contiguous()
    if Q.dtype != torch.int32 or Q.stride(1) != 1:
        raise ValueError("Q must be an int32 matrix with contiguous rows")
    _call(_fn("raht_quant_rows", dtype), X.device, _p(X), X.stride(0), n, D, st, len(st), _p(pos), _p(Q), Q.stride(0))
    return Q


def _dequant_rows(Q, steps, pos, out, dtype):
    _need_cuda(Q, "Q")
    if Q.dtype != torch.int32 or Q.stride(1) != 1:
        raise ValueError("Q must be an int32 matrix with contiguous rows")
    D = Q.shape[1]
    st = _step_array(steps, D, _STEP_CTYPE[dtype])
    pos = pos.to(torch.int64).contiguous()
    X = torch.empty((pos.shape[0], D), dtype=dtype, device=Q.device) if out is None else out
    if X.dtype != dtype or tuple(X.shape) != (pos.shape[0], D) or (X.shape[0] > 0 and (X.stride(1) != 1 or X.stride(0) < D)):
        raise ValueError(f"out must be a {'float64' if dtype == torch.float64 else 'float32'} (n, D) tensor with contiguous rows")
    _call(_fn("raht_dequant_rows", dtype), Q.device, _p(Q), Q.stride(0), _p(pos), pos.shape[0], D, st, len(st), _p(X), max(X.stride(0), D))
    return X


def quant_rows(X, steps, pos, Q):
    return _quant_rows(X, steps, pos, Q, torch.float32)


def dequant_rows(Q, steps, pos, out=None):
    return _dequant_rows(Q, steps, pos, out, torch.float32)


def quant_rows_f64(X, steps, pos, Q):
    return _quant_rows(X, steps, pos, Q, torch.float64)


def dequant_rows_f64(Q, steps, pos, out=None):
    return _dequant_rows(Q, steps, pos, out, torch.float64)


def sqdiff_columns(A, B):
    _need_cuda(A, "A")
    N, D = A.shape
    out = torch.empty(D, dtype=torch.float64, device=A.device)
    _call(_lib.lib().raht_sqdiff_columns, A.device, _p(A), A.stride(0), _p(B), B.stride(0), N, D, _VDT[A.dtype], _p(out))
    return out


def _rows_move(fn, src, pos, dst):
    _need_cuda(src, "src")
# ... 429 lines not shown
```

Baseline: 5019 M-Gaussians/s.

## Collapse upper inverse stages into per-tile walk programs at stage one

Builds, on the host and once per schedule, a per-tile "walk" program for stage 1 of the mixed inverse. Each program lists every butterfly from higher stages and the top stage that feeds the tile's survivors, plus the quantized positions to load. The inverse then runs a single walk-kernel launch that dequantizes and replays those ancestor butterflies in LDS. This replaces separate launches for stages 1..K-1 and their workspace round trips. The cost is redundant recomputation of shared upper-level butterflies across tiles, a host-side build with device-to-host copies on first use, and a fallback when a tile's ancestry exceeds R slots.

```diff
diff --git a/include/raht.h b/include/raht.h
--- a/include/raht.h
+++ b/include/raht.h
@@ -102,6 +102,7 @@
                                   raht_stream_t stream);
 int raht_plan_mixed_stats(raht_plan *plan, int D, int n_wide, int *tile_rows, int *n_stages, int64_t *rows_per_stage,
                           int max_stages);
+int raht_plan_mixed_walk_stage(raht_plan *plan, int D, int n_wide, int *walk_stage);
 
 int raht_fwd_batch(int n, raht_plan *const *plans, const float *const *C, const int64_t *ldc, int D,
                    float *const *T, const int64_t *ldt, raht_stream_t stream);
diff --git a/raht-3dgs-codec_amd/_lib.py b/raht-3dgs-codec_amd/_lib.py
--- a/raht-3dgs-codec_amd/_lib.py
+++ b/raht-3dgs-codec_amd/_lib.py
@@ -21,7 +21,7 @@
     "raht_quant_reorder", "raht_dequant_unreorder", "raht_voxelize", "raht_voxelize_all", "raht_voxelize_plan", "raht_morton", "raht_sort_keys",
     "raht_voxel_keys", "raht_sort_fallbacks", "raht_voxelize_residuals", "raht_plan_set_row_map", "raht_rows_gather", "raht_rows_scatter",
     "raht_plan_set_max_stages", "raht_plan_set_concurrent_directions", "raht_quant_reorder_f64", "raht_dequant_unreorder_f64", "raht_fwd_quant_f64", "raht_dequant_inv_f64",
-    "raht_fwd_quant_mixed", "raht_dequant_inv_mixed", "raht_dequant_inv_sqdiff", "raht_fwd_quant_multi", "raht_plan_mixed_stats",
+    "raht_fwd_quant_mixed", "raht_dequant_inv_mixed", "raht_dequant_inv_sqdiff", "raht_fwd_quant_multi", "raht_plan_mixed_stats", "raht_plan_mixed_walk_stage",
     "raht_fwd_quant_mixed_multi", "raht_dequant_inv_mixed_sqdiff",
     "raht_fwd_batch", "raht_inv_batch", "raht_fwd_quant_batch", "raht_dequant_inv_batch",
     "raht_fwd_quant_mixed_batch", "raht_dequant_inv_mixed_batch", "raht_mixed_batch_stats",
@@ -105,6 +105,7 @@
     L.raht_fwd_quant_mixed_multi.argtypes = [vp, vp, i64, i32, C.POINTER(dbl), i32, i32, C.POINTER(vp), i64, vp]
     L.raht_dequant_inv_mixed_sqdiff.argtypes = [vp, vp, i64, i32, C.POINTER(dbl), i32, i32, vp, i64, vp, i64, vp, vp]
     L.raht_plan_mixed_stats.argtypes = [vp, i32, i32, C.POINTER(i32), C.POINTER(i32), C.POINTER(i64), i32]
+    L.raht_plan_mixed_walk_stage.argtypes = [vp, i32, i32, C.POINTER(i32)]
     pp, pi64 = C.POINTER(vp), C.POINTER(i64)
     L.raht_fwd_batch.argtypes = [i32, pp, pp, pi64, i32, pp, pi64, vp]
     L.raht_inv_batch.argtypes = [i32, pp, pp, pi64, i32, pp, pi64, vp]
diff --git a/raht-3dgs-codec_amd/csrc/raht_common.h b/raht-3dgs-codec_amd/csrc/raht_common.h
--- a/raht-3dgs-codec_amd/csrc/raht_common.h
+++ b/raht-3dgs-codec_amd/csrc/raht_common.h
@@ -221,6 +221,10 @@
     bool ws_split = false;
     OwnedEvent ready;
     hipStream_t ready_on = nullptr;
+    DevBuf<uint32_t> walk;
+    uint32_t walk_stride = 0, walk_ab = 0;
+    int walk_stage = 0;
+    bool walk_tried = false;
 };
 static_assert(!std::is_copy_constructible<Stage>::value && !std::is_copy_constructible<Schedule>::value, "stages and schedules own device memory: moved, never copied");
 
@@ -277,6 +281,7 @@
 void pick_tail_geometry(const raht_plan *plan, int elem_size, int D, int stage0_rows, int *tail_rows, int *tail_chunk,
                         int *final_rows);
 int build_tile_programs(raht_plan *plan, Schedule *sc, hipStream_t s);
+int build_walk_programs(raht_plan *plan, Schedule *sc, int walk_stage, hipStream_t s);
 int ensure_workspace(Schedule *sc, size_t row_bytes, bool split = false);
 static inline void *stage_ws(const Stage &st, bool inverse) { return st.ws ? (void *)((char *)st.ws.get() + (inverse ? st.ws_inv_off : 0)) : nullptr; }
 void free_schedule(Schedule &sc);
diff --git a/raht-3dgs-codec_amd/csrc/schedule.hip b/raht-3dgs-codec_amd/csrc/schedule.hip
--- a/raht-3dgs-codec_amd/csrc/schedule.hip
+++ b/raht-3dgs-codec_amd/csrc/schedule.hip
@@ -86,6 +86,7 @@
 {
     if (!sc.stages.empty()) (void)hipDeviceSynchronize();
     sc.stages.clear();
+    sc.walk.reset(); sc.walk_stage = 0; sc.walk_tried = false;
     sc.ready = OwnedEvent();
 }
 
@@ -416,6 +417,169 @@
         RAHT_HIP_CHECK(hipEventRecord(sc->ready, s));
         sc->ready_on = s;
     }
+    return RAHT_OK;
+}
+
+namespace {
+struct WalkHostStage {
+    bool is_top = false;
+    int R = 0; int64_t n = 0; uint32_t stride = 0, ab = 0;
+    std::vector<uint32_t> prog, surv_off;
+    std::vector<uint32_t> pj, pos; std::vector<double> ab64; std::vector<uint32_t> lev; uint32_t n_merges = 0;
+};
+struct WalkBfly { uint32_t order, p, j; double a, b; };
+}
+
+int build_walk_programs(raht_plan *plan, Schedule *sc, int walk_stage, hipStream_t s)
+{
+    if (sc->walk_tried) return RAHT_OK;
+    const int K = (int)sc->stages.size();
+    const int w = walk_stage;
+    if (K < 3 || w < 1 || w > K - 2 || plan->N >= ((int64_t)1 << 30)) { sc->walk_tried = true; return RAHT_OK; }
+    std::vector<WalkHostStage> hs((size_t)K);
+    for (int k = w; k < K; ++k) {
+        const Stage &st = sc->stages[(size_t)k];
+        WalkHostStage &h = hs[(size_t)k];
+        h.is_top = st.is_top; h.n = st.n_entries;
+        if (st.is_top) {
+            if (k != K - 1 || !st.t_pj || !st.t_ab64 || !st.e_pos) { set_error("walk programs: missing top-stage arrays"); return RAHT_ERR_INVALID; }
+            h.n_merges = st.n_merges;
+            h.pj.resize(std::max<size_t>(st.n_merges, 1)); h.ab64.resize(2 * std::max<size_t>(st.n_merges, 1)); h.pos.resize((size_t)st.n_entries);
+            if (st.n_merges) {
+                RAHT_HIP_CHECK(hipMemcpyAsync(h.pj.data(), st.t_pj, sizeof(uint32_t) * st.n_merges, hipMemcpyDeviceToHost, s));
+                RAHT_HIP_CHECK(hipMemcpyAsync(h.ab64.data(), st.t_ab64, sizeof(double) * 2 * st.n_merges, hipMemcpyDeviceToHost, s));
+            }
+            RAHT_HIP_CHECK(hipMemcpyAsync(h.pos.data(), st.e_pos, sizeof(uint32_t) * (size_t)st.n_entries, hipMemcpyDeviceToHost, s));
+            if (st.t_nlev < 0 || st.t_nlev > 64 || (st.t_nlev && !st.t_lev)) { set_error("walk programs: missing top-stage levels"); return RAHT_ERR_INVALID; }
+            h.lev.resize(2 * (size_t)st.t_nlev);
+            if (st.t_nlev) RAHT_HIP_CHECK(hipMemcpyAsync(h.lev.data(), st.t_lev, sizeof(uint32_t) * h.lev.size(), hipMemcpyDeviceToHost, s));
+        } else {
+            if (!st.prog || st.prog_compact || (k < K - 1 && !st.surv_off)) { set_error("walk programs: missing tile programs"); return RAHT_ERR_INVALID; }
+            h.R = st.tile_rows; h.stride = st.prog_stride; h.ab = st.prog_ab;
+            h.prog.resize((size_t)st.prog_stride * (size_t)st.n_tiles);
+            RAHT_HIP_CHECK(hipMemcpyAsync(h.prog.data(), st.prog, sizeof(uint32_t) * h.prog.size(), hipMemcpyDeviceToHost, s));
+            if (st.surv_off) {
+                h.surv_off.resize((size_t)st.n_tiles + 1);
+                RAHT_HIP_CHECK(hipMemcpyAsync(h.surv_off.data(), st.surv_off, sizeof(uint32_t) * h.surv_off.size(), hipMemcpyDeviceToHost, s));
+            }
+        }
+    }
+    RAHT_HIP_CHECK(hipStreamSynchronize(s));
+    sc->walk_tried = true;
+
+    const WalkHostStage &hw = hs[(size_t)w];
+    const int R = hw.R;
+    const int64_t n_tiles = sc->stages[(size_t)w].n_tiles;
+    const uint32_t w_ab = (uint32_t)(4 + 2 * R + 3) & ~3u, w_stride = w_ab + 4 * (uint32_t)R;
+    std::vector<uint32_t> out((size_t)w_stride * (size_t)n_tiles, 0u);
+    std::vector<WalkBfly> bf;
+    std::vector<int> free_ids;
+    std::vector<std::pair<uint32_t, uint32_t>> want, next;
+    std::vector<int32_t> loc;
+    std::vector<uint8_t> wanted;
+    for (int64_t t = 0; t < n_tiles; ++t) {
+        uint32_t *o = out.data() + (size_t)t * w_stride;
+        uint32_t *o_slot = o + 4, *o_pj = o + 4 + R;
+        double *o_ab = (double *)(o + w_ab);
+        const uint32_t *pg = hw.prog.data() + (size_t)t * hw.stride;
+        const int nt = (int)std::min<int64_t>(R, hw.n - t * R);
+        const int n_merged = ((const uint16_t *)pg)[63];
+        const uint32_t *rec = pg + 32 + R;
+        const uint32_t sbase = hw.surv_off[(size_t)t], scnt = hw.surv_off[(size_t)t + 1] - sbase;
+        if ((int)scnt != nt - n_merged) { set_error("walk programs: survivor count of tile %lld", (long long)t); return RAHT_ERR_INVALID; }
+        std::vector<uint8_t> taken((size_t)R, 0);
+        want.clear(); bf.clear();
+        for (uint32_t q = 0; q < scnt; ++q) {
+            const uint32_t j = rec[n_merged + q];
+            if (j >= (uint32_t)R || taken[j]) { set_error("walk programs: survivor slots of tile %lld", (long long)t); return RAHT_ERR_INVALID; }
+            taken[j] = 1;
+            want.emplace_back(sbase + q, j);
+        }
+        free_ids.clear();
+        for (int j = R - 1; j >= 0; --j) if (!taken[(size_t)j]) free_ids.push_back(j);
+        bool fits = true;
+        auto new_slot = [&]() -> int { if (free_ids.empty()) { fits = false; return 0; } const int v = free_ids.back(); free_ids.pop_back(); return v; };
+        auto q_slot = [&](int slot, uint32_t qpos, bool root) { o_slot[slot] = 0x80000000u | (root ? 0x40000000u : 0u) | qpos; };
+        for (int k = w + 1; k < K && fits; ++k) {
+            const WalkHostStage &h = hs[(size_t)k];
+            next.clear();
+            if (h.is_top) {
+                loc.assign((size_t)h.n, -1); wanted.assign((size_t)h.n, 0);
+                for (auto &e : want) { if (e.first >= (uint64_t)h.n) { set_error("walk programs: top entry"); return RAHT_ERR_INVALID; } loc[e.first] = (int32_t)e.second; wanted[e.first] = 1; }
+                const int nlev = (int)h.lev.size() / 2;
+                for (int li = 0; li < nlev; ++li)
+                    if (h.lev[2 * (size_t)li + 1] > h.n_merges) { set_error("walk programs: top levels"); return RAHT_ERR_INVALID; }
+                for (int li = 0; li < nlev && fits; ++li)
+                    for (uint32_t m = h.lev[2 * (size_t)li]; m < h.lev[2 * (size_t)li + 1] && fits; ++m) {
+                        const uint32_t p = h.pj[m] & 0xffffu, j = h.pj[m] >> 16;
+                        if (p >= (uint64_t)h.n || j >= (uint64_t)h.n) { set_error("walk programs: top butterfly"); return RAHT_ERR_INVALID; }
+                        if (!wanted[p] && !wanted[j]) continue;
+                        if (loc[j] < 0) loc[j] = new_slot();
+                        if (loc[p] < 0) loc[p] = new_slot();
+                        if (!fits) break;
+                        bf.push_back({((uint32_t)k << 8) | (uint32_t)li, (uint32_t)loc[p], (uint32_t)loc[j], h.ab64[2 * (size_t)m], h.ab64[2 * (size_t)m + 1]});
+                        q_slot(loc[j], h.pos[j], false);
+                        wanted[p] = 1; wanted[j] = 0;
+                    }
+                for (int64_t e = 0; e < h.n && fits; ++e) if (wanted[(size_t)e]) q_slot(loc[(size_t)e], h.pos[(size_t)e], true);
+                want.clear();
+                continue;
+            }
+            for (size_t i0 = 0; i0 < want.size() && fits; ) {
+                const int64_t T = want[i0].first / h.R;
+                size_t i1 = i0;
+                while (i1 < want.size() && want[i1].first / h.R == T) ++i1;
+                if (want[i0].first >= (uint64_t)h.n) { set_error("walk programs: stage entry"); return RAHT_ERR_INVALID; }
+                const uint32_t *tp = h.prog.data() + (size_t)T * h.stride;
+                const uint16_t *end = (const uint16_t *)tp;
+                const uint32_t *rw = tp + 32, *trec = tp + 32 + h.R;
+                const double *tab = (const double *)(tp + h.ab);
+                const int tnt = (int)std::min<int64_t>(h.R, h.n - T * h.R);
+                const int tnm = end[63];
+                loc.assign((size_t)h.R, -1); wanted.assign((size_t)h.R, 0);
+                if (tnm > tnt || want[i1 - 1].first >= (uint64_t)h.n) { set_error("walk programs: stage tile"); return RAHT_ERR_INVALID; }
+                for (size_t i = i0; i < i1; ++i) { const int sl = (int)(want[i].first - T * h.R); loc[(size_t)sl] = (int32_t)want[i].second; wanted[(size_t)sl] = 1; }
+                int ht = 0;
+                for (int m = 0; m < tnm && fits; ++m) {
+                    while (ht < 63 && (int)end[ht] <= m) ++ht;
+                    const uint32_t p = trec[m] & 0xffffu, j = trec[m] >> 16;
+                    if (p >= (uint32_t)tnt || j >= (uint32_t)tnt) { set_error("walk programs: tile butterfly"); return RAHT_ERR_INVALID; }
+                    if (!wanted[p] && !wanted[j]) continue;
+                    if (loc[j] < 0) loc[j] = new_slot();
+                    if (loc[p] < 0) loc[p] = new_slot();
+                    if (!fits) break;
+                    bf.push_back({((uint32_t)k << 8) | (uint32_t)ht, (uint32_t)loc[p], (uint32_t)loc[j], tab[2 * m], tab[2 * m + 1]});
+                    q_slot(loc[j], rw[j] & 0x7fffffffu, false);
+                    wanted[p] = 1; wanted[j] = 0;
+                }
+                for (int q = 0; q < tnt - tnm && fits; ++q) {
+                    const uint32_t sl = trec[tnm + q];
+                    if (sl >= (uint32_t)tnt || !wanted[sl]) continue;
+                    wanted[sl] = 0;
+                    if (k == K - 1) q_slot(loc[sl], rw[sl] & 0x7fffffffu, true);
+                    else next.emplace_back(h.surv_off[(size_t)T] + (uint32_t)q, (uint32_t)loc[sl]);
+                }
+                for (int sl = 0; sl < tnt && fits; ++sl) if (wanted[(size_t)sl]) { set_error("walk programs: a wanted entry is neither merged nor a survivor"); return RAHT_ERR_INVALID; }
+                i0 = i1;
+            }
+            want.swap(next);
+        }
+        if (!fits || bf.size() > (size_t)R) return RAHT_OK;
+        std::stable_sort(bf.begin(), bf.end(), [](const WalkBfly &x, const WalkBfly &y) { return x.order > y.order; });
+        o[0] = (uint32_t)bf.size();
+        for (size_t i = 0; i < bf.size(); ++i) {
+            const bool first = i == 0 || bf[i].order != bf[i - 1].order;
+            o_pj[i] = bf[i].p | (first ? 0x8000u : 0u) | (bf[i].j << 16);
+            o_ab[2 * i] = bf[i].a; o_ab[2 * i + 1] = bf[i].b;
+        }
+        for (int j = 0; j < R; ++j) if ((o_slot[j] >> 31) && (o_slot[j] & 0x3fffffffu) >= (uint64_t)plan->N) { set_error("walk programs: Q position"); return RAHT_ERR_INVALID; }
+    }
+    RAHT_HIP_CHECK(sc->walk.alloc(out.size()));
+    RAHT_HIP_CHECK(hipMemcpyAsync(sc->walk, out.data(), sizeof(uint32_t) * out.size(), hipMemcpyHostToDevice, s));
+    sc->walk_stride = w_stride; sc->walk_ab = w_ab; sc->walk_stage = w;
+    if (!sc->ready) RAHT_HIP_CHECK(hipEventCreateWithFlags(&sc->ready.ev, hipEventDisableTiming));
+    RAHT_HIP_CHECK(hipEventRecord(sc->ready, s));
+    sc->ready_on = s;
     return RAHT_OK;
 }
 
diff --git a/raht-3dgs-codec_amd/csrc/transform_mx.hip b/raht-3dgs-codec_amd/csrc/transform_mx.hip
--- a/raht-3dgs-codec_amd/csrc/transform_mx.hip
+++ b/raht-3dgs-codec_amd/csrc/transform_mx.hip
@@ -28,6 +28,18 @@
     StepTable f;
     double w[MX_MAX_WIDE];
 };
+
+template <bool INV, typename T>
+__device__ __forceinline__ void mx_butterfly(const T a, const T b, const T x0, const T x1, T &lo, T &hi)
+{
+    if (!INV) {
+        lo = a * x0 + b * x1;
+        hi = a * x1 - b * x0;
+    } else {
+        lo = a * x0 - b * x1;
+        hi = b * x0 + a * x1;
+    }
+}
 
 static size_t tile_lds_bytes_mx(int R, int NF, int nwide)
 {
@@ -54,10 +66,16 @@
     int32_t *Q[MULTI_Q_MAX];
 };
 
-template <bool INV, bool IDENT, int SLOTS, bool ROOTS, bool MULTI = false, bool SQ = false>
+struct MxWalk {
+    const uint32_t *prog;
+    uint32_t stride, ab;
+};
+
+template <bool INV, bool IDENT, int SLOTS, bool ROOTS, bool MULTI = false, bool SQ = false, bool WALK = false>
 __device__ __forceinline__ void tile_body_mx(const TileArgs<float> &A, const MxPtrs &P, const StepTableMX &ST, const int64_t tile_id,
-                                             const MxMultiQ *MQ = nullptr)
-{
+                                             const MxMultiQ *MQ = nullptr, const MxWalk *WK = nullptr)
+{
+    static_assert(!WALK || (INV && !IDENT && !ROOTS && !MULTI && !SQ), "walk: a plain inverse stage >= 1");
     extern __shared__ __align__(16) unsigned char smem[];
     typedef RegChunk<float> V16;
     typedef RegChunk<double> W16;
@@ -131,6 +149,22 @@
             if (!P.prog_compact) m_ab[s] = ((const W16 *)(pg + P.prog_ab))[j];
         }
     }
+    uint32_t wk_n = 0, wk_q[SLOTS], wk_pj[SLOTS];
+    W16 wk_ab[SLOTS];
+    if constexpr (WALK) {
+        const uint32_t *wp = WK->prog + (uint64_t)tile_id * WK->stride;
+        wk_n = min(wp[0], (uint32_t)R);
+#pragma unroll
+        for (int s = 0; s < SLOTS; ++s) {
+            const int j = tid0 + s * nthreads;
+            wk_q[s] = 0; wk_pj[s] = 0; wk_ab[s].v[0] = 0.0; wk_ab[s].v[1] = 0.0;
+            if (j < R) {
+                wk_q[s] = wp[4 + j];
+                wk_pj[s] = wp[4 + R + j];
+                wk_ab[s] = ((const W16 *)(wp + WK->ab))[j];
+            }
+        }
+    }
     auto early_loads_landed = [&]() {
         asm volatile("" : "+v"(surv_raw));
         if constexpr (!MULTI) asm volatile("" : "+v"(tab_step[0]), "+v"(tab_step[1]), "+v"(tab_step[2]), "+v"(tab_step[3]));
@@ -227,6 +261,84 @@
         MX_STAMP(3);
         MX_STAMP(4);
     } else {
+        if constexpr (WALK) {
+#pragma unroll
+            for (int s = 0; s < SLOTS; ++s) {
+                const int j = tid0 + s * nthreads;
+                if (j < R) { sdst[j] = (int32_t)wk_q[s]; rec_pj[j] = wk_pj[s]; rec_ab[j] = wk_ab[s]; }
+            }
+            sync_lds();
+            load_caller_rows(R, [&](int jr, uint32_t go) -> const void * {
+                const uint32_t d = (uint32_t)sdst[jr];
+                return (d >> 31) ? (const void *)row_far((const int32_t *)A.Q, d & 0x3fffffffu, (uint32_t)A.ldq, go) : nullptr; });
+            wait_landed();
+            sync_lds();
+            use_steps();
+#pragma unroll
+            for (int s = 0; s < SLOTS; ++s) {
+                const int j = tid0 + s * nthreads;
+                if (j < R && (wk_q[s] >> 31)) {
+                    double *row = wd + __mul24(j, nwide);
+                    const I16 raw = *(const I16 *)(ftile + __mul24(j, Fp));
+#pragma unroll
+                    for (int i = 0; i < 4; ++i) if (i < nwide) row[i] = (double)raw.v[i] * ST.w[i];
+                }
+            }
+            if (c4 < NF) for (int it = wid; (it << lr) < R; it += nwv) {
+                const int jr = (it << lr) + g;
+                if (jr < R && ((uint32_t)sdst[jr] >> 30) == 3u) {
+                    V16 *pr = (V16 *)&ftile[__mul24(jr, Fp) + fl * 4];
+                    const I16 raw = *(const I16 *)pr;
+                    V16 x;
+#pragma unroll
+                    for (int i = 0; i < 4; ++i)
+                        x.v[i] = (head && i < nwide) ? __int_as_float(raw.v[i]) : (float)raw.v[i] * my_step[i];
+                    *pr = x;
+                }
+            }
+            sync_lds();
+            if (wid == 0) {
+                const uint32_t cf = (uint32_t)fl * 4u;
+                for (uint32_t k = 0; k < wk_n; ) {
+                    const uint32_t m = min(k + (uint32_t)g, wk_n - 1);
+                    const uint32_t pj = rec_pj[m];
+                    const W16 ab = rec_ab[m];
+                    const uint64_t stop = __ballot(g >= 1 && (k + (uint32_t)g >= wk_n || (pj & 0x8000u)));
+                    const uint32_t take = stop ? (uint32_t)(__ffsll((long long)stop) - 1) >> lg : 1u << lr;
+                    if ((uint32_t)g < take) {
+                        const uint32_t ip = __umul24(pj & 0x7fffu, (uint32_t)Fp) + cf, ij = __umul24(pj >> 16, (uint32_t)Fp) + cf;
+                        const V16 x0 = *(const V16 *)&ftile[ip];
+                        V16 x1 = *(const V16 *)&ftile[ij];
+#pragma unroll
+                        for (int i = 0; i < 4; ++i) x1.v[i] = (float)__float_as_int(x1.v[i]) * my_step[i];
+                        const float ca = (float)ab.v[0], cb = (float)ab.v[1];
+                        V16 lo, hi;
+#pragma unroll
+                        for (int i = 0; i < 4; ++i) mx_butterfly<true>(ca, cb, x0.v[i], x1.v[i], lo.v[i], hi.v[i]);
+                        *(V16 *)&ftile[ip] = lo; *(V16 *)&ftile[ij] = hi;
+                    }
+                    k += take;
+                }
+            } else if (wid == 1) {
+                const uint32_t gw = (uint32_t)lane >> lgw, cw = (uint32_t)min(lane & ((1 << lgw) - 1), nwide - 1);
+                for (uint32_t k = 0; k < wk_n; ) {
+                    const uint32_t m = min(k + gw, wk_n - 1);
+                    const uint32_t pj = rec_pj[m];
+                    const W16 ab = rec_ab[m];
+                    const uint64_t stop = __ballot(gw >= 1u && (k + gw >= wk_n || (pj & 0x8000u)));
+                    const uint32_t take = stop ? (uint32_t)(__ffsll((long long)stop) - 1) >> lgw : 64u >> lgw;
+                    if (gw < take) {
+                        const uint32_t ip = __umul24(pj & 0x7fffu, (uint32_t)nwide) + cw, ij = __umul24(pj >> 16, (uint32_t)nwide) + cw;
+                        const double d0 = wd[ip], d1 = wd[ij];
+                        double lo, hi;
+                        mx_butterfly<true>(ab.v[0], ab.v[1], d0, d1, lo, hi);
+                        wd[ip] = lo; wd[ij] = hi;
+                    }
+                    k += take;
+                }
+            }
+            __syncthreads();
+        }
         const uint32_t n_merged = (uint32_t)__builtin_amdgcn_readlane(end_v, 63);
         write_dst();
         write_survivors(n_merged);
@@ -239,7 +351,8 @@
         write_records(n_merged);
         const uint32_t surv_base = (uint32_t)__builtin_amdgcn_readlane((int)surv_raw, 0);
         const uint32_t surv_cnt = (uint32_t)__builtin_amdgcn_readlane((int)surv_raw, 1) - surv_base;
-        if (!A.last_stage) {
+        if constexpr (WALK) {
+        } else if (!A.last_stage) {
             if (c4 < NF) for (uint32_t it = wid; (it << lr) < surv_cnt; it += nwv) {
                 const uint32_t qc = min((it << lr) + g, surv_cnt - 1);
                 const V16 x = ld_chunk<float>(row_at((const float *)A.wsn + (int64_t)surv_base * Fp, qc, (uint32_t)Fp, (uint32_t)(fl * 4)));
@@ -330,15 +443,7 @@
                     const float ca = (float)ab[u].v[0], cb = (float)ab[u].v[1];
                     V16 lo, hi;
 #pragma unroll
-                    for (int i = 0; i < 4; ++i) {
-                        if (!INV) {
-                            lo.v[i] = ca * x0[u].v[i] + cb * x1[u].v[i];
-                            hi.v[i] = ca * x1[u].v[i] - cb * x0[u].v[i];
-                        } else {
-                            lo.v[i] = ca * x0[u].v[i] - cb * x1[u].v[i];
-                            hi.v[i] = cb * x0[u].v[i] + ca * x1[u].v[i];
-                        }
-                    }
+                    for (int i = 0; i < 4; ++i) mx_butterfly<INV>(ca, cb, x0[u].v[i], x1[u].v[i], lo.v[i], hi.v[i]);
                     if (u == 0 || mb + u * stride < cnt) { *(V16 *)&ftile[ip[u]] = lo; *(V16 *)&ftile[ij[u]] = hi; }
                 }
             };
@@ -354,13 +459,7 @@
                 const double d0 = wd[ip], d1 = wd[ij];
                 const double ca = ab.v[0], cb = ab.v[1];
                 double lo, hi;
-                if (!INV) {
-                    lo = ca * d0 + cb * d1;
-                    hi = ca * d1 - cb * d0;
-                } else {
-                    lo = ca * d0 - cb * d1;
-                    hi = cb * d0 + ca * d1;
-                }
+                mx_butterfly<INV>(ca, cb, d0, d1, lo, hi);
                 wd[ip] = lo; wd[ij] = hi;
             };
             if (cnt <= (1u << lr)) {
@@ -606,6 +705,11 @@
 __global__ __launch_bounds__(MX_THREADS, 6) void tile_kernel_mx_sq(const TileArgs<float> A, const MxPtrs P, const StepTableMX ST)
 {
     tile_body_mx<true, true, SLOTS, false, false, true>(A, P, ST, (int64_t)blockIdx.x);
+}
+template <int SLOTS>
+__global__ __launch_bounds__(MX_THREADS, 6) void tile_kernel_mx_walk(const TileArgs<float> A, const MxPtrs P, const StepTableMX ST, const MxWalk W)
+{
+    tile_body_mx<true, false, SLOTS, false, false, false, true>(A, P, ST, (int64_t)blockIdx.x, nullptr, &W);
 }
 
 struct TileBatchMX {
@@ -733,15 +837,7 @@
         const V16 x0 = tile[ip], x1 = tile[ij];
         V16 vlo, vhi;
 #pragma unroll
-        for (int i = 0; i < VN; ++i) {
-            if (!INV) {
-                vlo.v[i] = a * x0.v[i] + b * x1.v[i];
-                vhi.v[i] = a * x1.v[i] - b * x0.v[i];
-            } else {
-                vlo.v[i] = a * x0.v[i] - b * x1.v[i];
-                vhi.v[i] = b * x0.v[i] + a * x1.v[i];
-            }
-        }
+        for (int i = 0; i < VN; ++i) mx_butterfly<INV>(a, b, x0.v[i], x1.v[i], vlo.v[i], vhi.v[i]);
         tile[ip] = vlo; tile[ij] = vhi;
     };
     auto big_levels = [&]() {
@@ -1152,6 +1248,16 @@
     return RAHT_OK;
 }
 
+static int mx_walk_stage(int K)
+{
+#ifdef RAHT_WALK_LAST_TILE
+    return K - 2;
+#else
+    (void)K;
+    return 1;
+#endif
+}
+
 static int dequant_inv_mixed_impl(const raht_plan *cp, const int32_t *Q, int64_t ldq, int D, const double *steps, int n_steps, int n_wide,
                                   float *C, int64_t ldc, raht_stream_t stream)
 {
@@ -1181,7 +1287,21 @@
     MxIO io;
     io.C_out = C; io.ldc = ldc; io.Q = const_cast<int32_t *>(Q); io.ldq = ldq;
     const int K = (int)sc->stages.size();
-    for (int k = K - 1; k >= 0; --k) RAHT_RET((launch_stage_mx<true>(p, *sc, k, io, D, g, stp, s)));
+    int k_first = K - 1;
+    if (K >= 3 && !p->root_buf) {
+        RAHT_RET(build_walk_programs(p, sc, mx_walk_stage(K), s));
+        if (sc->walk_stage > 0) {
+            k_first = sc->walk_stage - 1;
+            MxStageLaunch L;
+            RAHT_RET((prepare_stage_mx<true>(p, *sc, sc->walk_stage, io, D, g, L)));
+            if (L.is_top || L.A.last_stage || L.A.root_buf) { set_error("raht_dequant_inv_mixed: walking stage %d is not an inner tile stage", sc->walk_stage); return RAHT_ERR_INVALID; }
+            const MxWalk W{sc->walk, sc->walk_stride, sc->walk_ab};
+            const dim3 grid(L.n_tiles), block(MX_THREADS);
+            if (L.A.R <= MX_THREADS) RAHT_RET((launch_lds<tile_kernel_mx_walk<1>>(grid, block, L.lds, TILE_LDS_LIMIT, s, L.A, L.P, stp, W)));
+            else RAHT_RET((launch_lds<tile_kernel_mx_walk<2>>(grid, block, L.lds, TILE_LDS_LIMIT, s, L.A, L.P, stp, W)));
+        }
+    }
+    for (int k = k_first; k >= 0; --k) RAHT_RET((launch_stage_mx<true>(p, *sc, k, io, D, g, stp, s)));
     return RAHT_OK;
 }
 
@@ -1519,4 +1639,21 @@
     });
 }
 
-}
+int raht_plan_mixed_walk_stage(raht_plan *plan, int D, int n_wide, int *walk_stage)
+{
+    return guarded("raht_plan_mixed_walk_stage", [&]() -> int {
+        if (!plan || !walk_stage || D < 1 || n_wide < 1 || n_wide > MX_MAX_WIDE) { set_error("raht_plan_mixed_walk_stage: bad argument"); return RAHT_ERR_INVALID; }
+        RAHT_RET(check_plan_device(plan, "raht_plan_mixed_walk_stage"));
+        *walk_stage = 0;
+        if (plan->row_map || plan->root_buf) return RAHT_OK;
+        Schedule *sc = nullptr;
+        MxGeom g;
+        RAHT_RET(mx_setup(plan, D, n_wide, D, nullptr, &sc, g));
+        if (!sc || sc->stages.size() < 3) return RAHT_OK;
+        RAHT_RET(build_walk_programs(plan, sc, mx_walk_stage((int)sc->stages.size()), nullptr));
+        *walk_stage = sc->walk_stage;
+        return RAHT_OK;
+    });
+}
+
+}
diff --git a/raht-3dgs-codec_amd/ops.py b/raht-3dgs-codec_amd/ops.py
--- a/raht-3dgs-codec_amd/ops.py
+++ b/raht-3dgs-codec_amd/ops.py
@@ -459,6 +459,12 @@
             check(_lib.lib().raht_plan_mixed_stats(self._h, int(D), int(n_wide), C.byref(tr), C.byref(ns), rows, 64))
         return {"tile_rows": tr.value, "rows_per_stage": [int(rows[i]) for i in range(ns.value)]}
 
+    def mixed_walk_stage(self, D=59, n_wide=3):
+        ws = C.c_int(0)
+        with torch.cuda.device(self.device):
+            check(_lib.lib().raht_plan_mixed_walk_stage(self._h, int(D), int(n_wide), C.byref(ws)))
+        return ws.value
+
     def quant_reorder(self, T, steps):
         T = _rows(T, None, "T")
         return self._quant_to("raht_quant_reorder", T, steps, torch.int32, T.dtype)
```

Result: no change. 5064 M-Gaussians/s, median of 4 (+0.9%).
